# ALIZE-Speaker-Recognition/LIA_RAL

Measured on AMD Instinct MI355X. Metric: Gframe-Gaussian evals/s (UBM EM pass: LLK + full-posterior statistics), higher is better.
Workload: dtype f64; 1 GPU; TrainWorld EM: 2048-Gaussian diag UBM, 60-dim float32 frames, 10000000 frames per GPU resident in HBM, 1 EM iteration per step; gaussians=2048, dim=60, frames_per_gpu=10000000, partitioning=frames sharded per rank, one RCCL all-reduce of 247810 doubles per step

## Files before the change

### lia_ral_amd/csrc/capi_ctx.hip

```cpp
#include <stdarg.h>
#include <stdlib.h>

#include "ctx.h"
#include "gmm_kernels.h"

static thread_local char g_err[512] = "";

static thread_local gmmiv_kopts g_kopts_val;
static thread_local const gmmiv_kopts *g_kopts_src = nullptr;
const gmmiv_kopts &gmmiv_kopts_cur() { return g_kopts_val; }
void gmmiv_kopts_bind(const gmmiv_kopts *ko) { g_kopts_val = ko ? *ko : gmmiv_kopts(); g_kopts_src = ko; }

void gmmiv_set_error(const char *fmt, ...)
{
    va_list ap;
    va_start(ap, fmt);
    vsnprintf(g_err, sizeof(g_err), fmt, ap);
    va_end(ap);
}

bool gmmiv_is_device_ptr(const void *p)
{
    if (!p) return false;
    hipPointerAttribute_t at;
    hipError_t e = hipPointerGetAttributes(&at, p);
    if (e != hipSuccess) {
        (void)hipGetLastError();
        return false;
    }
    return at.type == hipMemoryTypeDevice || at.type == hipMemoryTypeManaged;
}

extern "C" {

const char *gmmiv_last_error(void) { return g_err; }
const char *gmmiv_version(void) { return "gmmiv 0.1 (gfx950)"; }

int gmmiv_ctx_create(int device, void *stream, gmmiv_ctx **out)
{
    if (!out) { gmmiv_set_error("ctx_create: out == NULL"); return GMMIV_ERR_ARG; }
    int ndev = 0;
    hipError_t e = hipGetDeviceCount(&ndev);
    if (e != hipSuccess || ndev <= 0) {
        (void)hipGetLastError();
        gmmiv_set_error("ctx_create: no HIP device available (%s)", e == hipSuccess ? "count = 0" : hipGetErrorString(e));
        return GMMIV_ERR_HIP;
    }
    if (device < 0 || device >= ndev) { gmmiv_set_error("ctx_create: device %d out of range [0,%d)", device, ndev); return GMMIV_ERR_ARG; }
    GCHK(hipSetDevice(device));
    gmmiv_ctx *c = new gmmiv_ctx();
    c->device = device;
    if (stream == GMMIV_STREAM_DEFAULT || stream == (void *)hipStreamLegacy) { c->stream = nullptr; c->own_stream = false; }
    else if (stream) { c->stream = (hipStream_t)stream; c->own_stream = false; }
    else { GCHK(hipStreamCreateWithFlags(&c->stream, hipStreamNonBlocking)); c->own_stream = true; }
    hipDeviceProp_t prop;
    if (hipGetDeviceProperties(&prop, device) == hipSuccess) { c->n_cu = prop.multiProcessorCount; c->total_mem = prop.totalGlobalMem; }
    if (hipMalloc((void **)&c->d_zero_llk, 2 * sizeof(unsigned long long)) != hipSuccess || hipMemset(c->d_zero_llk, 0, 2 * sizeof(unsigned long long)) != hipSuccess) {
        (void)hipGetLastError();
        if (c->own_stream) (void)hipStreamDestroy(c->stream);
        delete c;
        gmmiv_set_error("ctx_create: hipMalloc of the context's device counters failed");
        return GMMIV_ERR_HIP;
    }
    c->d_screened = c->d_zero_llk + 1;
    *out = c;
    return GMMIV_OK;
}

void gmmiv_ctx_destroy(gmmiv_ctx *c)
{
    if (!c) return;
    (void)hipSetDevice(c->device);
    (void)hipStreamSynchronize(c->stream);
    for (gmmiv_comm *cm : std::vector<gmmiv_comm *>(c->comms)) gmmiv_comm_orphan(cm);
    for (int i = 0; i < WS_COUNT; ++i)
        if (c->ws[i]) (void)hipFree(c->ws[i]);
    for (int i = 0; i < gmmiv_ctx::NSLOT; ++i) {
        for (hipEvent_t e : c->ev0[i]) (void)hipEventDestroy(e);
        for (hipEvent_t e : c->ev1[i]) (void)hipEventDestroy(e);
    }
    if (c->d_zero_llk) (void)hipFree(c->d_zero_llk);
    if (c->own_stream) (void)hipStreamDestroy(c->stream);
    if (g_kopts_src == &c->ko) gmmiv_kopts_bind(nullptr);
    delete c;
}

int gmmiv_ctx_sync(gmmiv_ctx *c)
{
    if (!c) return GMMIV_ERR_ARG;
    GCHK(hipStreamSynchronize(c->stream));
    return GMMIV_OK;
}

void *gmmiv_ctx_stream(gmmiv_ctx *c) { return c ? (void *)c->stream : nullptr; }

long gmmiv_ctx_set_option(gmmiv_ctx *c, const char *key, long value)
{
    if (!c || !key) return -1;
    long *slot = nullptr;
    if (!strcmp(key, "glds")) slot = &c->use_glds;
    else if (!strcmp(key, "em_chunks")) slot = &c->em_chunks;
    else if (!strcmp(key, "timing")) slot = &c->timing;
    else if (!strcmp(key, "wg_waves")) slot = &c->wg_waves;
    else if (!strcmp(key, "dbg")) slot = &c->dbg;
    else if (!strcmp(key, "prune_log2")) slot = &c->prune_log2;
    else if (!strcmp(key, "stats_z")) slot = &c->stats_z;
    else if (!strcmp(key, "z_scratch_mb")) slot = &c->z_scratch_mb;
    else if (!strcmp(key, "models_scratch_mb")) slot = &c->models_scratch_mb;
    else if (!strcmp(key, "trials_scratch_mb")) slot = &c->trials_scratch_mb;
    else if (!strcmp(key, "trials_piece")) slot = &c->trials_piece;
    else if (!strcmp(key, "iv_trials_anchor")) slot = &c->iv_trials_anchor;
    else if (!strcmp(key, "iv_trials_piece")) slot = &c->iv_trials_piece;
    else if (!strcmp(key, "tv_batch")) slot = &c->tv_batch;
    else if (!strcmp(key, "tv_tett_direct")) slot = &c->tv_tett_direct;
    else if (!strcmp(key, "tv_stats_split")) slot = &c->tv_stats_split;
    else if (!strcmp(key, "topc_z")) slot = &c->topc_z;
    else if (!strcmp(key, "tv_mstep_solve")) slot = &c->tv_mstep_solve;
    else if (!strcmp(key, "tv_md_device")) slot = &c->tv_md_device;
    else if (!strcmp(key, "tv_acc_mb")) slot = &c->tv_acc_mb;
    else if (!strcmp(key, "topc_fused")) slot = &c->topc_fused;
    else if (!strcmp(key, "topc_fallbacks")) slot = &c->topc_fallbacks;
    else if (!strcmp(key, "topc_rank_direct")) slot = &c->topc_rank_direct;
    else if (!strcmp(key, "topc_rank2")) slot = &c->topc_rank2;
    else if (!strcmp(key, "topc_use_lanes")) slot = &c->topc_use_lanes;
    else if (!strcmp(key, "assume_finite")) slot = &c->assume_finite;
    int *ks = nullptr;
    if (!strcmp(key, "z_waves")) { const long prev = c->ko.z_waves; c->ko.z_waves = (value == 4 || value == 16) ? (int)value : 8; return prev; }
    if (!strcmp(key, "z_depth_em")) { const long prev = c->ko.z_depth_em; if (value == 2 || value == 4) c->ko.z_depth_em = (int)value; return prev; }
    if (!strcmp(key, "z_depth_tv")) { const long prev = c->ko.z_depth_tv; if (value == 2 || value == 4) c->ko.z_depth_tv = (int)value; return prev; }
    if (!strcmp(key, "z_tv4")) ks = &c->ko.z_tv4;
    else if (!strcmp(key, "gemm_remap")) ks = &c->ko.gemm_remap;
    else if (!strcmp(key, "gemm_clamp")) ks = &c->ko.gemm_clamp;
    else if (!strcmp(key, "gemm_narrow")) ks = &c->ko.gemm_narrow;
    else if (!strcmp(key, "gemm_nt80")) ks = &c->ko.gemm_nt80;
    else if (!strcmp(key, "chol_lds")) ks = &c->ko.chol_lds;
    else if (!strcmp(key, "chol_gemm")) ks = &c->ko.chol_gemm;
    else if (!strcmp(key, "chol_waves")) ks = &c->ko.chol_waves;
    else if (!strcmp(key, "short_calls")) ks = &c->ko.short_calls;
    else if (!strcmp(key, "chol_flow")) ks = &c->ko.chol_flow;
    if (ks) { const long prev = *ks; *ks = (int)value; return prev; }
    if (!strcmp(key, "zero_llk_frames") || !strcmp(key, "screened_frames")) {
        unsigned long long *ctr = key[0] == 'z' ? c->d_zero_llk : c->d_screened;
        unsigned long long prev = 0, nv = value > 0 ? (unsigned long long)value : 0;
        if (hipSetDevice(c->device) != hipSuccess || hipStreamSynchronize(c->stream) != hipSuccess ||
            hipMemcpy(&prev, ctr, sizeof prev, hipMemcpyDeviceToHost) != hipSuccess ||
            hipMemcpy(ctr, &nv, sizeof nv, hipMemcpyHostToDevice) != hipSuccess) { (void)hipGetLastError(); return -1; }
        return (long)prev;
    }
    if (!strcmp(key, "kopts_bound")) return g_kopts_src == &c->ko ? 1 : 0;
    if (!slot) return -1;
    long prev = *slot;
    *slot = value;
    return prev;
}

int gmmiv_ctx_set_hook(gmmiv_ctx *c, const char *point, gmmiv_hook_fn fn, void *user)
{
    if (!c || !point) return -1;
    gmmiv_ctx::Hook *h = !strcmp(point, "tv_a_ready") ? &c->hook_tv_a_ready : (!strcmp(point, "md_factored") ? &c->hook_md_factored : nullptr);
    if (!h) return -1;
    h->fn = fn;
    h->user = fn ? user : nullptr;
    return 0;
}
// ... 103 lines not shown
```

### lia_ral_amd/csrc/capi_feat.hip

```cpp
#include <math.h>
#include <stdlib.h>

#include <algorithm>

#include "ctx.h"
#include "gmm_kernels.h"
#include "tv_kernels.h"
#include "capi_gmm_util.h"

extern "C" {

int gmmiv_frame_moments(gmmiv_ctx *c, const void *x, int dt, int64_t T, int64_t ldx, int D, double *acc)
{
    if (!c || !acc || T < 0 || D <= 0) { gmmiv_set_error("frame_moments: bad argument"); return GMMIV_ERR_ARG; }
    GBIND(c);
    XView xv;
    int rc = xv.init(c, x, dt, T, ldx, D);
    if (rc) return rc;
    DevOut<double> o;
    if ((rc = o.init(c, WS_T0, acc, 2 * D + 1, true))) return rc;
    const int maxb = 2048;
    void *part;
    if ((rc = c->scratch(WS_PART, (size_t)maxb * 2 * D * sizeof(double), &part))) return rc;
    c->t_begin("k_frame_moments");
// ... 63 lines not shown
    c->t_end();
    if (!gmmiv_is_device_ptr(runs)) GCHK(hipStreamSynchronize(c->stream));
    return GMMIV_OK;
}

int gmmiv_segment_means(gmmiv_ctx *c, const double *v, int64_t ld, int nrows, const int64_t *seg_begin, int64_t nseg, double *out)
{
    if (!c || !v || !seg_begin || !out || nrows < 0 || nseg < 0 || ld < 0) { gmmiv_set_error("segment_means: bad argument"); return GMMIV_ERR_ARG; }
    if (!gmmiv_is_device_ptr(v)) { gmmiv_set_error("segment_means: v must be a device array"); return GMMIV_ERR_ARG; }
    if (gmmiv_is_device_ptr(seg_begin)) { gmmiv_set_error("segment_means: seg_begin must be a host array"); return GMMIV_ERR_ARG; }
    for (int64_t s = 0; s < nseg; ++s)
        if (seg_begin[s] < 0 || seg_begin[s + 1] < seg_begin[s]) { gmmiv_set_error("segment_means: seg_begin must be non-negative and non-decreasing"); return GMMIV_ERR_ARG; }
    if (nseg > 0 && nrows > 1 && seg_begin[nseg] > ld) { gmmiv_set_error("segment_means: the last segment ends after the row stride"); return GMMIV_ERR_ARG; }
    const int64_t npair = (int64_t)nrows * nseg;
    if (npair == 0) return GMMIV_OK;
    GBIND(c);
    const int64_t PIECE = 8192;
    std::vector<long> tab;
    std::vector<long> off(npair + 1, 0), len(npair, 0);
    for (int r = 0; r < nrows; ++r)
        for (int64_t s = 0; s < nseg; ++s) {
            const int64_t p = (int64_t)r * nseg + s;
            len[p] = (long)(seg_begin[s + 1] - seg_begin[s]);
            for (int64_t b = seg_begin[s]; b < seg_begin[s + 1]; b += PIECE) {
                tab.push_back(r); tab.push_back((long)b); tab.push_back((long)(b + PIECE < seg_begin[s + 1] ? b + PIECE : seg_begin[s + 1]));
            }
            off[p + 1] = (long)(tab.size() / 3);
        }
    const size_t nitem = tab.size() / 3;
    tab.insert(tab.end(), off.begin(), off.end());
    tab.insert(tab.end(), len.begin(), len.end());
    void *dtab, *part;
    int rc;
    if ((rc = c->scratch(WS_T8, tab.size() * sizeof(long), &dtab))) return rc;
    if ((rc = c->scratch(WS_T9, (nitem ? nitem : 1) * sizeof(double), &part))) return rc;
    DevOut<double> o;
    if ((rc = o.init(c, WS_T7, out, (size_t)npair, false))) return rc;
    GCHK(hipMemcpyAsync(dtab, tab.data(), tab.size() * sizeof(long), hipMemcpyHostToDevice, c->stream));
    const long *di = (const long *)dtab;
    GCHK(gmmk_segment_means(c->stream, v, (long)ld, di, (long)nitem, (double *)part, di + 3 * nitem, di + 3 * nitem + npair + 1, (long)npair, o.d));
    GCHK(hipStreamSynchronize(c->stream));
    return o.finish();
}

static int feat_check_dtype(const char *who, int xdt, int odt)
{
    if ((xdt != GMMIV_F32 && xdt != GMMIV_F64) || (odt != GMMIV_F32 && odt != GMMIV_F64)) { gmmiv_set_error("%s: x_dtype / out_dtype must be GMMIV_F32 or GMMIV_F64", who); return GMMIV_ERR_ARG; }
    return GMMIV_OK;
}
static int feat_check(const char *who, const void *x, int xdt, int64_t T, int64_t ldx, const void *out, int odt, int64_t ldo, int D)
{
    if (T < 0 || ldx < D || ldo < D) { gmmiv_set_error("%s: T < 0 or a row stride below vectSize %d", who, D); return GMMIV_ERR_ARG; }
    if (T == 0) return GMMIV_OK;
    if (!x || !out) { gmmiv_set_error("%s: x or out == NULL", who); return GMMIV_ERR_ARG; }
    const uintptr_t xb = (uintptr_t)x, xe = xb + ((size_t)(T - 1) * ldx + D) * gmmiv_esize(xdt);
    const uintptr_t ob = (uintptr_t)out, oe = ob + ((size_t)(T - 1) * ldo + D) * gmmiv_esize(odt);
    const bool in_place = x == out && xdt == odt && ldx == ldo;
    if (!in_place && xb < oe && ob < xe) { gmmiv_set_error("%s: out overlaps x (only out == x with the same dtype and stride is allowed)", who); return GMMIV_ERR_ARG; }
    return GMMIV_OK;
}

int gmmiv_feat_check_args(const char *who, const void *x, int xdt, int64_t T, int64_t ldx, const void *out, int odt, int64_t ldo, int D)
{
    const int rc = feat_check_dtype(who, xdt, odt);
    return rc ? rc : feat_check(who, x, xdt, T, ldx, out, odt, ldo, D);
}

int gmmiv_feat_compensate(gmmiv_ctx *c, const gmmiv_gmm *g, const void *x, int dt, int64_t T, int64_t ldx, const double *offset,
                          void *out, int odt, int64_t ldo)
{
    int rc = feat_check_dtype("feat_compensate", dt, odt);
    if (rc) return rc;
    if (!c || !g) { gmmiv_set_error("feat_compensate: NULL context or model"); return GMMIV_ERR_ARG; }
    if ((rc = check_model(c, g))) return rc;
    if (!offset) { gmmiv_set_error("feat_compensate: offset == NULL"); return GMMIV_ERR_ARG; }
    if ((rc = feat_check("feat_compensate", x, dt, T, ldx, out, odt, ldo, g->D))) return rc;
    if (T == 0) return GMMIV_OK;
    XView xv;
    if ((rc = xv.init(c, x, dt, T, ldx, g->D))) return rc;
    FeatOut o;
    if ((rc = o.init(c, out, odt, 0, T, ldo, g->D))) return rc;
    DevIn<double> i_off;
    if ((rc = i_off.init(c, WS_FEAT_M0, offset, (size_t)g->C * g->D))) return rc;
    if ((rc = count_unusable(c, xv, dt, T, g->D))) return rc;
    const int64_t Tcz = g->D <= 64 ? z_chunk_frames(c, g) : 0;
    if (Tcz > 0) {
        gmmk_zview z;
        double *lz;
        void *offp;
        if ((rc = gmmiv_z_reserve(c, g->nct, T < Tcz ? T : Tcz, true, &z, &lz))) return rc;
        if ((rc = c->scratch(WS_FEAT_OFF, gmmk_feat_offset_doubles(g->nct, g->D) * sizeof(double), &offp))) return rc;
        GCHK(gmmk_feat_pack_offset(c->stream, i_off.d, g->C, g->D, g->nct, (double *)offp));
        for (int64_t c0 = 0; c0 < T; c0 += Tcz) {
            const int64_t n = (T - c0) < Tcz ? (T - c0) : Tcz;
            if ((rc = llk_z_run(c, g, xv, dt, c0, n, lz, z, c0 == 0))) return rc;
            GCHK(count_dead(c, lz, n));
            c->t_begin("k_feat_comp", c0 == 0);
            GCHK(gmmk_feat_comp(c->stream, dt == GMMIV_F64, odt == GMMIV_F64, gmmiv_x_at(xv, dt, c0), xv.ldx, n, g->D, g->nct, z, (const double *)offp,
                                o.at(c0), o.ld));
            c->t_end();
        }
        return o.finish();
    }
    double *lse;
    if ((rc = run_lse(c, g, xv, dt, T, &lse))) return rc;
    int64_t per = (int64_t)(((size_t)512 << 20) / ((size_t)g->C * sizeof(double))) / 2 * 2;
    if (per < 64) per = 64;
    const int64_t firstg = T < per ? T : per;
    void *gam, *pm;
    if ((rc = c->scratch(WS_Z, (size_t)firstg * g->C * sizeof(double), &gam))) return rc;
    if ((rc = c->scratch(WS_INV, (size_t)firstg * g->D * sizeof(double), &pm))) return rc;
    for (int64_t b = 0; b < T; b += per) {
        const int64_t m = T - b < per ? T - b : per;
        c->t_begin("k_posteriors", b == 0);
        GCHK(gmmk_posteriors(c->stream, dt == GMMIV_F64, gmmiv_x_at(xv, dt, b), (long)m, xv.ldx, g->D, g->C, g->Cp64, g->meanT, g->ivT, g->lwc, lse + b,
                             (double *)gam));
        c->t_end();
        GCHK(tvk_dgemm(c->stream, false, false, (int)m, g->D, g->C, 1.0, (const double *)gam, g->C, 0, i_off.d, g->D, 0, 0.0, (double *)pm, g->D, 0, 1));
        c->t_begin("k_feat_sub", b == 0);
        GCHK(gmmk_feat_sub(c->stream, dt == GMMIV_F64, odt == GMMIV_F64, gmmiv_x_at(xv, dt, b), xv.ldx, (long)m, g->D, (const double *)pm, lse + b, o.at(b), o.ld));
        c->t_end();
    }
    return o.finish();
}

int gmmiv_feat_map(gmmiv_ctx *c, const gmmiv_gmm *cd, const double *cd_mean, const double *cd_cov, const double *ci_mean,
                   const double *ci_cov, const void *x, int dt, int64_t T, int64_t ldx, void *out, int odt, int64_t ldo, int32_t *best)
{
    int rc = feat_check_dtype("feat_map", dt, odt);
    if (rc) return rc;
    if (!c || !cd) { gmmiv_set_error("feat_map: NULL context or model"); return GMMIV_ERR_ARG; }
    if ((rc = check_model(c, cd))) return rc;
    if (!cd_mean || !cd_cov || !ci_mean || !ci_cov) { gmmiv_set_error("feat_map: a model table is NULL"); return GMMIV_ERR_ARG; }
    if ((rc = feat_check("feat_map", x, dt, T, ldx, out, odt, ldo, cd->D))) return rc;
    if (T == 0) return GMMIV_OK;
    XView xv;
    if ((rc = xv.init(c, x, dt, T, ldx, cd->D))) return rc;
    FeatOut o;
    if ((rc = o.init(c, out, odt, 0, T, ldo, cd->D))) return rc;
    const size_t CD = (size_t)cd->C * cd->D;
    DevIn<double> m0, v0, m1, v1;
    if ((rc = m0.init(c, WS_FEAT_M0, cd_mean, CD)) || (rc = v0.init(c, WS_FEAT_M1, cd_cov, CD)) || (rc = m1.init(c, WS_FEAT_M2, ci_mean, CD)) ||
        (rc = v1.init(c, WS_FEAT_M3, ci_cov, CD))) return rc;
    int32_t *bd = best;
    if (!gmmiv_is_device_ptr(best)) {
        void *p;
        if ((rc = c->scratch(WS_FEAT_IDX, (size_t)T * sizeof(int32_t), &p))) return rc;
        bd = (int32_t *)p;
    }
    GCHK(hipMemsetAsync(bd, 0, (size_t)T * sizeof(int32_t), c->stream));
    if ((rc = gmmiv_llk_determine_top(c, cd, xv.d, dt, T, xv.ldx, 1, GMMIV_TOP_COMPLETE, -INFINITY, INFINITY, bd, nullptr, nullptr, nullptr, nullptr,
                                      nullptr))) return rc;
    c->t_begin("k_feat_map");
    GCHK(gmmk_feat_map(c->stream, dt == GMMIV_F64, odt == GMMIV_F64, xv.d, xv.ldx, T, cd->D, cd->C, bd, m0.d, v0.d, m1.d, v1.d, o.d, o.ld));
    c->t_end();
    if (best && bd != best) GCHK(hipMemcpyAsync(best, bd, (size_t)T * sizeof(int32_t), hipMemcpyDeviceToHost, c->stream));
    if ((rc = o.finish())) return rc;
    if (best && bd != best) GCHK(hipStreamSynchronize(c->stream));
    return GMMIV_OK;
}

int gmmiv_scatter_runs(gmmiv_ctx *c, void *x, int dt, int64_t ldx, int D, const int64_t *runs, int64_t nrun, const void *in)
{
    if (!c || !x || !in || (!runs && nrun > 0) || nrun < 0 || D <= 0 || ldx < D) { gmmiv_set_error("scatter_runs: bad argument"); return GMMIV_ERR_ARG; }
    if (dt != GMMIV_F32 && dt != GMMIV_F64) { gmmiv_set_error("scatter_runs: feature dtype must be GMMIV_F32 or GMMIV_F64"); return GMMIV_ERR_ARG; }
    if (!gmmiv_is_device_ptr(x) || !gmmiv_is_device_ptr(in)) { gmmiv_set_error("scatter_runs: x and in must be device arrays"); return GMMIV_ERR_ARG; }
    if (nrun == 0) return GMMIV_OK;
    GBIND(c);
    DevIn<int64_t> i_runs;
    int rc = i_runs.init(c, WS_T0, runs, (size_t)nrun * 3);
    if (rc) return rc;
    c->t_begin("k_scatter_runs");
    GCHK(gmmk_scatter_runs(c->stream, dt == GMMIV_F64, x, ldx, D, (const long *)i_runs.d, nrun, in));
    c->t_end();
    if (!gmmiv_is_device_ptr(runs)) GCHK(hipStreamSynchronize(c->stream));
    return GMMIV_OK;
}

static int norm_check_runs(const char *who, const int64_t *runs, int64_t nrun, int64_t ngroups, int64_t *lo, int64_t *hi)
{
    int64_t prev = 0, a = INT64_MAX, b = 0;
    for (int64_t r = 0; r < nrun; ++r) {
        const int64_t first = runs[3 * r], len = runs[3 * r + 1], g = runs[3 * r + 2];
        if (first < 0 || len < 0) { gmmiv_set_error("%s: run %ld has a negative first frame or length", who, (long)r); return GMMIV_ERR_ARG; }
        if (g < prev || g >= ngroups) { gmmiv_set_error("%s: run %ld: group %ld is below its predecessor's or outside [0, %ld) (group ids must be non-decreasing)", who, (long)r, (long)g, (long)ngroups); return GMMIV_ERR_ARG; }
        prev = g;
        if (len > 0) { if (first < a) a = first; if (first + len > b) b = first + len; }
    }
// ... 216 lines not shown
```

### lia_ral_amd/csrc/capi_gmm.hip

```cpp
#include <math.h>
#include <stdlib.h>

#include "ctx.h"
#include "gmm_kernels.h"
#include "tv_kernels.h"
#include "capi_gmm_util.h"

namespace {
struct TopOut {
    int *idx;
    double *lk, *nlk, *nllk, *nw, *llk;
    int ctop;
    template <typename V> static V *from(V *p, size_t off) { return p ? p + off : nullptr; }
    TopOut at(int64_t c0) const { return TopOut{from(idx, (size_t)c0 * ctop), from(lk, (size_t)c0 * ctop), from(nlk, c0), from(nllk, c0), from(nw, c0), from(llk, c0), ctop}; }
};
}

int count_unusable(gmmiv_ctx *c, const XView &xv, int dt, int64_t T, int D)
{
    if (c->assume_finite || T <= 0) return GMMIV_OK;
    void *p;
    int rc;
    const size_t fbytes = ((size_t)T + 15) / 16 * 16;
    if ((rc = c->scratch(WS_GFLAG, fbytes + 16, &p))) return rc;
    unsigned char *flag = (unsigned char *)p;
    GCHK(hipMemsetAsync(flag, 0, fbytes + 16, c->stream));
    GCHK(gmmk_flag_frames(c->stream, dt == GMMIV_F64, xv.d, T, xv.ldx, D, flag, (int *)(flag + fbytes)));
    GCHK(gmmk_count_flags(c->stream, flag, (long)T, c->d_screened));
    return GMMIV_OK;
}

static int topc_big(gmmiv_ctx *c, const gmmiv_gmm *g, const XView &xv, int dt, int64_t T, int complete, double lo, double hi, const TopOut &o)
{
    const int ctop = o.ctop;
    if (T <= 0) return GMMIV_OK;
    int64_t per = (int64_t)(((size_t)1 << 30) / ((size_t)g->Cp64 * sizeof(double))) / 4 * 4;
    if (per < 4) per = 4;
    if (per > T) per = (T + 3) / 4 * 4;
    void *zs;
    int rc = c->scratch(WS_Z, gmmk_topc_big_scratch_doubles((long)per, g->Cp64) * sizeof(double), &zs);
    if (rc) return rc;
    for (int64_t c0 = 0; c0 < T; c0 += per) {
        const int64_t n = T - c0 < per ? T - c0 : per;
        c->t_begin("k_topc_determine", c0 == 0);
        const TopOut oc = o.at(c0);
        int krc = gmmk_topc_determine_big(c->stream, dt == GMMIV_F64, gmmiv_x_at(xv, dt, c0), (long)n, xv.ldx, g->D, g->C, g->Cp64, g->meanT, g->ivT, g->lwc,
                                          g->w, ctop, complete, lo, hi, oc.idx, oc.lk, oc.nlk, oc.nllk, oc.nw, oc.llk, (double *)zs);
        c->t_end();
        if (krc == -1) { gmmiv_set_error("vectSize %d exceeds the generic kernels' bound", g->D); return GMMIV_ERR_UNSUPPORTED; }
        if (krc == -2) { gmmiv_set_error("topDistribsCount %d outside 1 .. mixtureDistribCount %d", ctop, g->C); return GMMIV_ERR_ARG; }
        GCHK(krc);
    }
    return GMMIV_OK;
}

int run_lse(gmmiv_ctx *c, const gmmiv_gmm *g, const XView &xv, int dt, int64_t T, double **lse_out)
{
    void *lse;
    int rc = c->scratch(WS_LSE, (size_t)(T > 0 ? T : 1) * sizeof(double), &lse);
    if (rc) return rc;
    if (g->KS == GMMK_KS_GENERIC) {
        if ((rc = topc_big(c, g, xv, dt, T, 1, -INFINITY, INFINITY, TopOut{nullptr, nullptr, nullptr, nullptr, nullptr, (double *)lse, 1}))) return rc;
        GCHK(count_dead(c, (const double *)lse, T));
        *lse_out = (double *)lse;
        return GMMIV_OK;
    }
    c->t_begin("k_llk_mfma");
    GCHK(gmmk_llk(c->stream, g->KS, dt == GMMIV_F64, xv.d, T, xv.ldx, g->D, g->Pt, g->nct, (double *)lse, (int)(c->use_glds | (c->dbg << 8)), (int)c->wg_waves));
    c->t_end();
    GCHK(count_dead(c, (const double *)lse, T));
    *lse_out = (double *)lse;
    return GMMIV_OK;
}

int generic_gamma_gemm(gmmiv_ctx *c, const gmmiv_gmm *g, const XView &xv, int dt, int64_t t0, int64_t n, const double *lse, bool sq, int NC,
                       double *S)
{
    int rc;
    int64_t per = (int64_t)(((size_t)512 << 20) / ((size_t)g->C * sizeof(double)));
    if (per < 64) per = 64;
    per = per / 2 * 2;
    void *gam, *xa;
    const int64_t first = n < per ? n : per;
    if ((rc = c->scratch(WS_Z, (size_t)(first > 0 ? first : 1) * g->C * sizeof(double), &gam))) return rc;
    if ((rc = c->scratch(WS_INV, (size_t)(first > 0 ? first : 1) * NC * sizeof(double), &xa))) return rc;
    if (n <= 0) { GCHK(hipMemsetAsync(S, 0, (size_t)g->C * NC * sizeof(double), c->stream)); return GMMIV_OK; }
    for (int64_t b = 0; b < n; b += per) {
        const int64_t m = n - b < per ? n - b : per;
        c->t_begin("k_posteriors", b == 0);
        GCHK(gmmk_posteriors(c->stream, dt == GMMIV_F64, gmmiv_x_at(xv, dt, t0 + b), (long)m, xv.ldx, g->D, g->C, g->Cp64, g->meanT, g->ivT, g->lwc, lse + t0 + b,
                             (double *)gam));
        c->t_end();
        GCHK(gmmk_build_xa(c->stream, dt == GMMIV_F64, gmmiv_x_at(xv, dt, t0 + b), xv.ldx, g->D, (long)m, sq ? 1 : 0, NC, (double *)xa));
        GCHK(tvk_dgemm(c->stream, true, false, g->C, NC, (int)m, 1.0, (const double *)gam, g->C, 0, (const double *)xa, NC, 0, b == 0 ? 0.0 : 1.0, S, NC, 0, 1));
    }
    return GMMIV_OK;
}

static size_t fused_frame_bytes() { return (size_t)gmmk_topc_cap() * 16; }

static int64_t fused_chunk_frames(const gmmiv_ctx *c)
{
    size_t budget = (size_t)(c->z_scratch_mb > 0 ? c->z_scratch_mb : 0) << 20;
    if (c->total_mem && budget > c->total_mem / 4) budget = c->total_mem / 4;
    const int64_t Tf = (int64_t)(budget / fused_frame_bytes() / 1.2) / 256 * 256;
    return Tf >= 256 ? Tf : 0;
}

static int top_fused(gmmiv_ctx *c, const gmmiv_gmm *g, const XView &xv, int dt, int64_t T, int complete, double min_llk, double max_llk,
                     const TopOut &o, int64_t Tf, bool *done)
{
    int rc;
    const int ctop = o.ctop;
    const int64_t nalloc = T < Tf ? (T + 255) / 256 * 256 : Tf;
    const int stats = getenv("GMMIV_TOPC_STATS") != nullptr;
    void *cand, *cnt, *th, *sl, *flg, *redo;
    if ((rc = c->scratch(WS_Z, (size_t)nalloc * fused_frame_bytes(), &cand))) return rc;
    if ((rc = c->scratch(WS_EIT, (size_t)nalloc * sizeof(int), &cnt))) return rc;
    if ((rc = c->scratch(WS_INV, (size_t)nalloc * (sizeof(double) + sizeof(int)), &sl))) return rc;
    if ((rc = c->scratch(WS_LSE, (size_t)nalloc * sizeof(double), &th))) return rc;
    if ((rc = c->scratch(WS_FLAGS, 64, &flg))) return rc;
    int *efin = (int *)((double *)sl + nalloc);
    if ((rc = c->scratch(WS_SEG, (size_t)nalloc * 2 * sizeof(long), &redo))) return rc;
    int krc = 0;
    bool whole = false;
    for (int64_t c0 = 0; c0 < T; c0 += Tf) {
        const int64_t n = (T - c0) < Tf ? (T - c0) : Tf;
        const TopOut oc = o.at(c0);
        GCHK(hipMemsetAsync(flg, 0, 64, c->stream));
        c->t_begin("k_llk_mfma", c0 == 0);
        krc = gmmk_llk_topc(c->stream, g->KS, dt == GMMIV_F64, gmmiv_x_at(xv, dt, c0), n, xv.ldx, g->D, g->Pt, g->nct, (int)c->use_glds,
                            ctop, (double *)cand, (int *)cnt, (double *)th, (double *)sl, efin);
        c->t_end();
        if (krc) break;
        c->t_begin("k_topc_rank", c0 == 0);
        krc = gmmk_topc_rank(c->stream, dt == GMMIV_F64, gmmiv_x_at(xv, dt, c0), n, xv.ldx, g->D, g->C, (const double *)cand, (const int *)cnt,
                             (const double *)th, (const double *)sl, efin, g->mean, g->iv, g->lwc, g->w, ctop, complete,
                             min_llk, max_llk, oc.idx, oc.lk, oc.nlk, oc.nllk, oc.nw, oc.llk, (int *)flg, (long *)redo,
                             stats | (c->topc_rank_direct ? 2 : 0) | (c->topc_rank2 ? 0 : 4), (long *)redo + nalloc);
        c->t_end();
        if (krc) break;
        int hf[16] = {0};
        GCHK(hipMemcpyAsync(hf, flg, 64, hipMemcpyDeviceToHost, c->stream));
        GCHK(hipStreamSynchronize(c->stream));
        if (stats)
            fprintf(stderr, "topc fused: %ld frames, redone %d | overflow %d, survivors > 64: %d, < ctop: %d, margin %d | list max %d mean %.1f | survivors max %d mean %.1f\n",
                    (long)n, hf[0], hf[1], hf[2], hf[3], hf[4], hf[5], (double)*(unsigned long long *)&hf[6] / (double)n, hf[8],
                    (double)*(unsigned long long *)&hf[10] / (double)n);
        const int64_t nr = hf[0];
        c->topc_fallbacks += nr;
        if (nr == 0) continue;
        if (nr > n / 8 + 64) { whole = true; break; }
        void *gx, *t_idx, *t_d;
        if ((rc = c->scratch(WS_PART, (size_t)nr * g->D * gmmiv_esize(dt), &gx))) return rc;
        if ((rc = c->scratch(WS_T6, (size_t)nr * ctop * sizeof(int), &t_idx))) return rc;
        if ((rc = c->scratch(WS_T7, (size_t)nr * (ctop + 4) * sizeof(double), &t_d))) return rc;
        double *t_lk = (double *)t_d, *t_nlk = t_lk + (size_t)nr * ctop, *t_nllk = t_nlk + nr, *t_nw = t_nllk + nr, *t_llk = t_nw + nr;
        GCHK(gmmk_gather_frames(c->stream, dt == GMMIV_F64, gmmiv_x_at(xv, dt, c0), xv.ldx, g->D, (const long *)redo, nr, gx));
        c->t_begin("k_topc_determine", c0 == 0);
        GCHK(gmmk_topc_determine(c->stream, dt == GMMIV_F64, gx, nr, g->D, g->D, g->C, g->Cp64, g->meanT, g->ivT, g->lwc, g->w, ctop,
                                 complete, min_llk, max_llk, (int *)t_idx, t_lk, t_nlk, t_nllk, t_nw, t_llk));
        c->t_end();
        GCHK(gmmk_topc_scatter(c->stream, nr, ctop, (const long *)redo, (const int *)t_idx, t_lk, t_nlk, t_nllk, t_nw, t_llk, oc.idx, oc.lk, oc.nlk,
                               oc.nllk, oc.nw, oc.llk));
    }
    if (krc > 0) GCHK(krc);
    *done = krc == 0 && !whole;
    return GMMIV_OK;
}

static int top_from_z(gmmiv_ctx *c, const gmmiv_gmm *g, const XView &xv, int dt, int64_t T, int complete, double min_llk, double max_llk,
                      const TopOut &o, int64_t Tc, bool *done)
{
    int rc;
    gmmk_zview z;
    double *lse;
    void *flg;
    if ((rc = gmmiv_z_reserve(c, g->nct, T < Tc ? T : Tc, true, &z, &lse))) return rc;
    if ((rc = c->scratch(WS_FLAGS, 64, &flg))) return rc;
    GCHK(hipMemsetAsync(flg, 0, sizeof(int), c->stream));
    for (int64_t c0 = 0; c0 < T; c0 += Tc) {
        const int64_t n = (T - c0) < Tc ? (T - c0) : Tc;
        const TopOut oc = o.at(c0);
        if ((rc = llk_z_run(c, g, xv, dt, c0, n, lse, z, c0 == 0))) return rc;
        c->t_begin("k_topc_from_z", c0 == 0);
        GCHK(gmmk_topc_from_z(c->stream, dt == GMMIV_F64, gmmiv_x_at(xv, dt, c0), n, xv.ldx, g->D, g->C, g->nct, z, g->mean, g->iv, g->lwc, g->w,
                              o.ctop, complete, min_llk, max_llk, oc.idx, oc.lk, oc.nlk, oc.nllk, oc.nw, oc.llk, (int *)flg));
        c->t_end();
    }
    int hflag = 0;
    GCHK(hipMemcpyAsync(&hflag, flg, sizeof(int), hipMemcpyDeviceToHost, c->stream));
    GCHK(hipStreamSynchronize(c->stream));
    *done = hflag == 0;
    return GMMIV_OK;
}

static int top_direct(gmmiv_ctx *c, const gmmiv_gmm *g, const XView &xv, int dt, int64_t T, int complete, double min_llk, double max_llk,
                      const TopOut &o)
{
    if (o.ctop > 64 || !gmmk_topc_frames_per_block(g->Cp64, g->D)) return topc_big(c, g, xv, dt, T, complete, min_llk, max_llk, o);
    c->t_begin("k_topc_determine");
    GCHK(gmmk_topc_determine(c->stream, dt == GMMIV_F64, xv.d, T, xv.ldx, g->D, g->C, g->Cp64, g->meanT, g->ivT, g->lwc,
                             g->w, o.ctop, complete, min_llk, max_llk, o.idx, o.lk, o.nlk, o.nllk, o.nw, o.llk));
    c->t_end();
    return GMMIV_OK;
}

extern "C" {

int gmmiv_llk(gmmiv_ctx *c, const gmmiv_gmm *g, const void *x, int dt, int64_t T, int64_t ldx, double min_llk,
              double max_llk, double *llk_out, double *sums)
{
    int rc = check_model(c, g);
    if (rc) return rc;
    if (T < 0) { gmmiv_set_error("llk: T < 0"); return GMMIV_ERR_ARG; }
    XView xv;
    if ((rc = xv.init(c, x, dt, T, ldx, g->D))) return rc;
    if ((rc = count_unusable(c, xv, dt, T, g->D))) return rc;
    double *lse;
    if ((rc = run_lse(c, g, xv, dt, T, &lse))) return rc;
    DevOut<double> o_llk, o_sum;
    if ((rc = o_llk.init(c, WS_T0, llk_out, (size_t)T, false))) return rc;
    if ((rc = o_sum.init(c, WS_T1, sums, 2, true))) return rc;
    void *part;
    if ((rc = c->scratch(WS_SMALL, 3 * 256 * sizeof(double), &part))) return rc;
    GCHK(gmmk_llk_finalize(c->stream, lse, T, min_llk, max_llk, o_llk.d, (double *)part, 1.0, 0.0,
                           sums ? o_sum.d : nullptr, nullptr));
    if (sums) GCHK(gmmk_add_scalar(c->stream, o_sum.d + 1, (double)T));
    if ((rc = o_llk.finish())) return rc;
    return o_sum.finish();
}

int gmmiv_llk_determine_top(gmmiv_ctx *c, const gmmiv_gmm *g, const void *x, int dt, int64_t T, int64_t ldx, int ctop,
                            int mode, double min_llk, double max_llk, int32_t *idx, double *lk, double *nontop_lk,
                            double *nontop_llk, double *nontop_w, double *llk_out)
{
    int rc = check_model(c, g);
    if (rc) return rc;
    if (T < 0 || !idx || ctop <= 0) { gmmiv_set_error("determine_top: bad argument"); return GMMIV_ERR_ARG; }
    if (ctop > g->C) { gmmiv_set_error("determine_top: topDistribsCount %d exceeds mixtureDistribCount %d (clamp it at the call site)", ctop, g->C); return GMMIV_ERR_ARG; }
    XView xv;
    if ((rc = xv.init(c, x, dt, T, ldx, g->D))) return rc;
    if ((rc = count_unusable(c, xv, dt, T, g->D))) return rc;
    DevOut<int32_t> o_idx;
    DevOut<double> o_lk, o_nlk, o_nllk, o_nw, o_llk;
    if ((rc = o_idx.init(c, WS_T0, idx, (size_t)T * ctop, false))) return rc;
    if ((rc = o_lk.init(c, WS_T1, lk, (size_t)T * ctop, false))) return rc;
    if ((rc = o_nlk.init(c, WS_T2, nontop_lk, (size_t)T, false))) return rc;
    if ((rc = o_nllk.init(c, WS_T3, nontop_llk, (size_t)T, false))) return rc;
    if ((rc = o_nw.init(c, WS_T4, nontop_w, (size_t)T, false))) return rc;
    if ((rc = o_llk.init(c, WS_T5, llk_out, (size_t)T, false))) return rc;
    const TopOut o{o_idx.d, o_lk.d, o_nlk.d, o_nllk.d, o_nw.d, o_llk.d, ctop};
    const int complete = mode == GMMIV_TOP_COMPLETE;
    bool done = false;
    const int64_t Tf = (c->topc_fused && T > 0 && ctop <= 16 && g->C <= 2048 && g->D <= 64 && g->KS <= 15 && c->wg_waves == 8) ? fused_chunk_frames(c) : 0;
    if (Tf > 0 && (rc = top_fused(c, g, xv, dt, T, complete, min_llk, max_llk, o, Tf, &done))) return rc;
    const int64_t Tc = (!done && c->topc_z) ? z_chunk_frames(c, g) : 0;
    if (Tc > 0 && T > 0 && ctop + 4 <= 64 && gmmk_topc_z_lds(g->nct, g->D) && (rc = top_from_z(c, g, xv, dt, T, complete, min_llk, max_llk, o, Tc, &done))) return rc;
    if (!done && (rc = top_direct(c, g, xv, dt, T, complete, min_llk, max_llk, o))) return rc;
    if ((rc = o_idx.finish())) return rc;
    if ((rc = o_lk.finish())) return rc;
    if ((rc = o_nlk.finish())) return rc;
    if ((rc = o_nllk.finish())) return rc;
    if ((rc = o_nw.finish())) return rc;
    return o_llk.finish();
}

int gmmiv_topgauss_compute(gmmiv_ctx *c, const gmmiv_gmm *g, const void *x, int dt, int64_t T, int64_t ldx, int cap, double top_gauss,
                           int mode, double min_llk, double max_llk, int32_t *idx, int32_t *count, double *snsw, double *snsl,
                           double *llk_out, int64_t *n_capped)
{
    int rc = check_model(c, g);
    if (rc) return rc;
    if (T < 0 || !idx || !count || !snsw || !snsl || cap <= 0 || !(top_gauss > 0.0)) { gmmiv_set_error("topgauss_compute: bad argument"); return GMMIV_ERR_ARG; }
    if (n_capped && gmmiv_is_device_ptr(n_capped)) { gmmiv_set_error("topgauss_compute: n_capped must be a host variable"); return GMMIV_ERR_ARG; }
    const int fixed = top_gauss >= 1.0 ? (int)top_gauss : 0;
    if (fixed > cap) { gmmiv_set_error("topgauss_compute: topGauss %d exceeds the list length %d", fixed, cap); return GMMIV_ERR_ARG; }
    if (n_capped) *n_capped = 0;
    if (T == 0) return GMMIV_OK;
    void *p;
    const bool idx_dev = gmmiv_is_device_ptr(idx);
    int32_t *d_idx = idx;
    if (!idx_dev) { if ((rc = c->scratch(WS_LP, (size_t)T * cap * sizeof(int32_t), &p))) return rc; d_idx = (int32_t *)p; }
    if ((rc = c->scratch(WS_AUX, (size_t)T * cap * sizeof(double), &p))) return rc;
    double *d_lk = (double *)p;
    const bool llk_dev = llk_out && gmmiv_is_device_ptr(llk_out);
    double *d_llk = llk_out;
    if (!llk_dev) { if ((rc = c->scratch(WS_SLAB, (size_t)T * sizeof(double), &p))) return rc; d_llk = (double *)p; }
    if ((rc = gmmiv_llk_determine_top(c, g, x, dt, T, ldx, cap, mode, min_llk, max_llk, d_idx, d_lk, nullptr, nullptr, nullptr, d_llk))) return rc;
    DevOut<int32_t> o_cnt;
    DevOut<double> o_w, o_l;
    if ((rc = o_cnt.init(c, WS_T0, count, (size_t)T, false))) return rc;
    if ((rc = o_w.init(c, WS_T1, snsw, (size_t)T, false))) return rc;
    if ((rc = o_l.init(c, WS_T2, snsl, (size_t)T, false))) return rc;
    if ((rc = c->scratch(WS_SMALL, 3 * 256 * sizeof(double), &p))) return rc;
    unsigned long long *d_cap = (unsigned long long *)p;
    GCHK(hipMemsetAsync(d_cap, 0, sizeof(unsigned long long), c->stream));
    GCHK(gmmk_topgauss_select(c->stream, T, cap, top_gauss, fixed, g->w, d_idx, d_lk, d_llk, o_cnt.d, o_w.d, o_l.d, d_cap));
    if (!idx_dev) GCHK(hipMemcpyAsync(idx, d_idx, (size_t)T * cap * sizeof(int32_t), hipMemcpyDeviceToHost, c->stream));
    if (llk_out && !llk_dev) GCHK(hipMemcpyAsync(llk_out, d_llk, (size_t)T * sizeof(double), hipMemcpyDeviceToHost, c->stream));
    if (n_capped) {
        unsigned long long h = 0;
        GCHK(hipMemcpyAsync(&h, d_cap, sizeof(h), hipMemcpyDeviceToHost, c->stream));
// ... 25 lines not shown
    if ((rc = o_llk.init(c, WS_T2, llk_out, (size_t)T, false))) return rc;
    if ((rc = count_unusable(c, xv, dt, T, g->D))) return rc;
    c->t_begin("k_topc_use");
    int krc = ctop > 64 ? gmmk_topc_use_big(c->stream, dt == GMMIV_F64, xv.d, T, xv.ldx, g->D, g->mean, g->iv, g->lwc, g->C, ctop, i_idx.d, i_n.d,
                                            mode == GMMIV_TOP_COMPLETE, min_llk, max_llk, o_llk.d)
              : c->topc_z ? gmmk_topc_use16(c->stream, dt == GMMIV_F64, xv.d, T, xv.ldx, g->D, g->mean, g->iv, g->lwc, g->C, ctop, i_idx.d, i_n.d,
                                          mode == GMMIV_TOP_COMPLETE, min_llk, max_llk, o_llk.d, (int)c->topc_use_lanes)
                        : -1;
    if (krc == -1 && ctop <= 64)
        krc = gmmk_topc_use(c->stream, dt == GMMIV_F64, xv.d, T, xv.ldx, g->D, g->mean, g->iv, g->lwc, g->C, ctop, i_idx.d, i_n.d,
                            mode == GMMIV_TOP_COMPLETE, min_llk, max_llk, o_llk.d);
    GCHK(krc);
    c->t_end();
    return o_llk.finish();
}

int gmmiv_llk_use_top_multi(gmmiv_ctx *c, int n_clients, const gmmiv_gmm *const *clients, const void *x, int dt, int64_t T, int64_t ldx,
                            int ctop, const int32_t *idx, const double *nontop_llk, int mode, double min_llk, double max_llk,
                            double *llk_out)
{
    if (!c) { gmmiv_set_error("use_top_multi: null context"); return GMMIV_ERR_ARG; }
    if (n_clients < 0 || (n_clients > 0 && !clients)) { gmmiv_set_error("use_top_multi: bad client list"); return GMMIV_ERR_ARG; }
    if (n_clients == 0) return GMMIV_OK;
    int rc;
    for (int i = 0; i < n_clients; ++i) {
        if ((rc = check_model(c, clients[i]))) return rc;
        if (clients[i]->D != clients[0]->D) { gmmiv_set_error("use_top_multi: client %d has %d dimensions, client 0 has %d", i, clients[i]->D, clients[0]->D); return GMMIV_ERR_ARG; }
        if (ctop > clients[i]->C) { gmmiv_set_error("use_top_multi: topDistribsCount %d exceeds mixtureDistribCount %d of client %d", ctop, clients[i]->C, i); return GMMIV_ERR_ARG; }
    }
    if (T < 0 || !idx || !llk_out || ctop <= 0) { gmmiv_set_error("use_top_multi: bad argument"); return GMMIV_ERR_ARG; }
    if (mode == GMMIV_TOP_COMPLETE && !nontop_llk) { gmmiv_set_error("use_top_multi: COMPLETE mode needs nontop_llk"); return GMMIV_ERR_ARG; }
    const gmmiv_gmm *g0 = clients[0];
    {
        const size_t cap = (size_t)1 << 30, row = (size_t)(T > 0 ? T : 1) * sizeof(double);
        if (n_clients > 1 && !gmmiv_is_device_ptr(llk_out) && (size_t)n_clients * row > cap) {
            const int per = (int)(cap / row > 0 ? cap / row : 1);
            for (int i0 = 0; i0 < n_clients; i0 += per) {
                const int n = n_clients - i0 < per ? n_clients - i0 : per;
                if ((rc = gmmiv_llk_use_top_multi(c, n, clients + i0, x, dt, T, ldx, ctop, idx, nontop_llk, mode, min_llk, max_llk, llk_out + (size_t)i0 * T))) return rc;
            }
            return GMMIV_OK;
        }
    }
    const bool batched = c->topc_z && c->topc_use_lanes == 4 && ctop <= 16 && g0->D % 2 == 0 && n_clients <= 65535 && T > 0;
    if (!batched) {
        for (int i = 0; i < n_clients; ++i)
            if ((rc = gmmiv_llk_use_top(c, clients[i], x, dt, T, ldx, ctop, idx, nontop_llk, mode, min_llk, max_llk, llk_out + (size_t)i * T))) return rc;
        return GMMIV_OK;
    }
    GBIND(c);
    XView xv;
    if ((rc = xv.init(c, x, dt, T, ldx, g0->D))) return rc;
    if ((rc = count_unusable(c, xv, dt, T, g0->D))) return rc;
    DevIn<int32_t> i_idx;
    DevIn<double> i_n;
    DevOut<double> o_llk;
    if ((rc = i_idx.init(c, WS_T0, idx, (size_t)T * ctop))) return rc;
    if ((rc = i_n.init(c, WS_T1, nontop_llk, (size_t)T))) return rc;
    if ((rc = o_llk.init(c, WS_T2, llk_out, (size_t)T * n_clients, false))) return rc;
    struct Rec { const double *mean, *iv, *lwc; long C; };
    std::vector<Rec> recs((size_t)n_clients);
    for (int i = 0; i < n_clients; ++i) recs[i] = Rec{clients[i]->mean, clients[i]->iv, clients[i]->lwc, (long)clients[i]->C};
    void *drec;
    if ((rc = c->scratch(WS_T3, recs.size() * sizeof(Rec), &drec))) return rc;
    GCHK(hipMemcpyAsync(drec, recs.data(), recs.size() * sizeof(Rec), hipMemcpyHostToDevice, c->stream));
    GCHK(hipStreamSynchronize(c->stream));
    c->t_begin("k_topc_use");
    GCHK(gmmk_topc_use4_multi(c->stream, dt == GMMIV_F64, xv.d, T, xv.ldx, g0->D, drec, n_clients, ctop, i_idx.d, i_n.d, mode == GMMIV_TOP_COMPLETE,
                              min_llk, max_llk, o_llk.d));
    c->t_end();
    return o_llk.finish();
}

int gmmiv_occ(gmmiv_ctx *c, const gmmiv_gmm *g, const void *x, int dt, int64_t T, int64_t ldx, double *gamma)
{
    int rc = check_model(c, g);
    if (rc) return rc;
    if (T < 0 || !gamma) { gmmiv_set_error("occ: bad argument"); return GMMIV_ERR_ARG; }
    if (T > 0x7fffffff) { gmmiv_set_error("occ: too many frames in one call"); return GMMIV_ERR_UNSUPPORTED; }
    XView xv;
    if ((rc = xv.init(c, x, dt, T, ldx, g->D))) return rc;
    DevOut<double> o;
    if ((rc = o.init(c, WS_T0, gamma, (size_t)T * g->C, false))) return rc;
    if ((rc = count_unusable(c, xv, dt, T, g->D))) return rc;
    const int64_t Tcz = c->topc_z ? z_chunk_frames(c, g) : 0;
    if (Tcz > 0 && T > 0) {
        gmmk_zview z;
        double *lz;
        if ((rc = gmmiv_z_reserve(c, g->nct, T < Tcz ? T : Tcz, true, &z, &lz))) return rc;
        for (int64_t c0 = 0; c0 < T; c0 += Tcz) {
            const int64_t n = (T - c0) < Tcz ? (T - c0) : Tcz;
            if ((rc = llk_z_run(c, g, xv, dt, c0, n, lz, z, c0 == 0))) return rc;
            GCHK(count_dead(c, lz, n));
            c->t_begin("k_post_from_z", c0 == 0);
            GCHK(gmmk_post_from_z(c->stream, n, g->C, g->nct, z, o.d + (size_t)c0 * g->C));
            c->t_end();
        }
        return o.finish();
    }
    double *lse;
    if ((rc = run_lse(c, g, xv, dt, T, &lse))) return rc;
    c->t_begin("k_posteriors");
    GCHK(gmmk_posteriors(c->stream, dt == GMMIV_F64, xv.d, T, xv.ldx, g->D, g->C, g->Cp64, g->meanT, g->ivT, g->lwc, lse, o.d));
    c->t_end();
    return o.finish();
}

size_t gmmiv_em_acc_len(int C, int D) { return (size_t)C * (1 + 2 * (size_t)D) + 2; }

static int make_chunks(gmmiv_ctx *c, int64_t T, int nseg, long **dev)
{
    const int64_t per = ((T + nseg - 1) / nseg + 63) / 64 * 64;
    void *buf;
    int rc = c->scratch(WS_SEG, (nseg + 1) * sizeof(long), &buf);
    if (rc) return rc;
    GCHK(gmmk_fill_chunks(c->stream, (long *)buf, nseg, (long)per, (long)T));
    *dev = (long *)buf;
    return GMMIV_OK;
}

static int em_stats_z(gmmiv_ctx *c, const gmmiv_gmm *g, const XView &xv, int dt, int64_t T, int64_t Tc, double weight,
                      double *lse, int *nseg_out, void **part_out)
{
    int rc;
    const int ngrp = gmmk_stats_z_groups(g->nct);
    int nseg = c->em_chunks > 0 ? (int)c->em_chunks : (c->n_cu * gmmk_stats_z_wg_per_cu() + ngrp - 1) / ngrp;
    nseg = (nseg + 7) / 8 * 8;
    const int64_t first = T < Tc ? T : Tc;
    const int64_t cap = (first + 255) / 256;
    if (nseg > cap) nseg = (int)((cap + 7) / 8 * 8);
    const int64_t nchunk = (T + Tc - 1) / Tc;
    const int64_t lastn = T - (nchunk - 1) * Tc;
    void *seg, *part;
    if ((rc = c->scratch(WS_SEG, 2 * (size_t)(nseg + 1) * sizeof(long), &seg))) return rc;
    auto fill = [&](long *dst, int64_t n) {
        const int64_t per = ((n + nseg - 1) / nseg + 63) / 64 * 64;
        return gmmk_fill_chunks(c->stream, dst, nseg, (long)per, (long)n);
    };
    GCHK(fill((long *)seg, first));
    GCHK(fill((long *)seg + nseg + 1, lastn));
    gmmk_zview z;
    if ((rc = gmmiv_z_reserve(c, g->nct, first, !(c->dbg & 64), &z, nullptr))) return rc;
    const int RL = gmmk_rl_for_ks(g->KS);
    const size_t Cp = (size_t)g->nct * 16;
    if ((rc = c->scratch(WS_PART, (size_t)nseg * Cp * 2 * RL * sizeof(double), &part))) return rc;
    for (int64_t k = 0; k < nchunk; ++k) {
        const int64_t c0 = k * Tc, n = (k == nchunk - 1) ? lastn : Tc;
        if ((rc = llk_z_run(c, g, xv, dt, c0, n, lse + c0, z, k == 0))) return rc;
        GCHK(count_dead(c, lse + c0, n));
        c->t_begin("k_stats_z", k == 0);
        GCHK(gmmk_stats_z(c->stream, g->KS, 1, dt == GMMIV_F64, gmmiv_x_at(xv, dt, c0), xv.ldx, g->D, g->C, g->nct, z, weight,
                          (const long *)seg + (k == nchunk - 1 ? nseg + 1 : 0), nseg, (double *)part, nullptr, 0, k > 0, c->prune_thr()));
        c->t_end();
    }
    *nseg_out = nseg;
    *part_out = part;
    return GMMIV_OK;
}

int gmmiv_em_accumulate(gmmiv_ctx *c, const gmmiv_gmm *g, const void *x, int dt, int64_t T, int64_t ldx, double weight,
                        double *acc)
{
    int rc = check_model(c, g);
    if (rc) return rc;
    if (T < 0 || !acc || !(weight > 0.0)) { gmmiv_set_error("em_accumulate: bad argument (T >= 0, weight > 0, acc != NULL)"); return GMMIV_ERR_ARG; }
    const size_t nacc = gmmiv_em_acc_len(g->C, g->D);
    DevOut<double> o;
    if ((rc = o.init(c, WS_T0, acc, nacc, true))) return rc;
    if (T == 0) return o.finish();
    XView xv;
    if ((rc = xv.init(c, x, dt, T, ldx, g->D))) return rc;
    if ((rc = count_unusable(c, xv, dt, T, g->D))) return rc;
    const int64_t Tc = z_chunk_frames(c, g);
    if (Tc > 0) {
        void *lsew, *small, *part;
        int nseg = 0;
        if ((rc = c->scratch(WS_LSE, (size_t)T * sizeof(double), &lsew))) return rc;
        if ((rc = c->scratch(WS_SMALL, 3 * 256 * sizeof(double), &small))) return rc;
        if ((rc = em_stats_z(c, g, xv, dt, T, Tc, weight, (double *)lsew, &nseg, &part))) return rc;
        GCHK(gmmk_llk_finalize(c->stream, (const double *)lsew, T, -INFINITY, INFINITY, nullptr, (double *)small, 0.0, weight, nullptr,
                               o.d + nacc - 2, weight, o.d + nacc - 1));
        GCHK(gmmk_em_reduce(c->stream, (const double *)part, nseg, g->C, g->nct * 16, g->D, g->KS, o.d));
        return o.finish();
    }
    double *lse;
    if ((rc = run_lse(c, g, xv, dt, T, &lse))) return rc;
    void *small;
    if ((rc = c->scratch(WS_SMALL, 3 * 256 * sizeof(double), &small))) return rc;
    GCHK(gmmk_llk_finalize(c->stream, lse, T, -INFINITY, INFINITY, nullptr, (double *)small, 0.0, weight, nullptr,
                           o.d + nacc - 2, weight, o.d + nacc - 1));
    if (g->KS == GMMK_KS_GENERIC) {
        const int NC = 2 * g->D + 2;
        void *S;
        if ((rc = c->scratch(WS_PART, (size_t)g->C * NC * sizeof(double), &S))) return rc;
        if ((rc = generic_gamma_gemm(c, g, xv, dt, 0, T, lse, true, NC, (double *)S))) return rc;
        GCHK(gmmk_scatter_em(c->stream, g->C, g->D, NC, (const double *)S, weight, o.d));
        return o.finish();
    }
    const int nw = c->wg_waves == 8 ? 8 : 4;
    const int ngrp = (g->nct + nw - 1) / nw;
    int nseg = c->em_chunks > 0 ? (int)c->em_chunks : ((nw == 8 ? 2 : 4) * c->n_cu + ngrp - 1) / ngrp;
    nseg = (nseg + 7) / 8 * 8;
    const int64_t cap = (T + 4095) / 4096;
    if (nseg > cap) nseg = (int)cap;
    if (nseg < 1) nseg = 1;
    long *seg;
    if ((rc = make_chunks(c, T, nseg, &seg))) return rc;
    const int RL = gmmk_rl_for_ks(g->KS);
    const size_t Cp = (size_t)g->nct * 16;
    void *part;
    if ((rc = c->scratch(WS_PART, (size_t)nseg * Cp * 2 * RL * sizeof(double), &part))) return rc;
    c->t_begin("k_stats_mfma");
    GCHK(gmmk_stats(c->stream, g->KS, 1, dt == GMMIV_F64, xv.d, xv.ldx, g->D, g->C, g->Pt, g->nct, lse, -log(weight), seg,
                    nseg, (double *)part, nullptr, 0, (int)c->wg_waves, c->prune_arg()));
    c->t_end();
    GCHK(gmmk_em_reduce(c->stream, (const double *)part, nseg, g->C, (int)Cp, g->D, g->KS, o.d));
    return o.finish();
}

int gmmiv_em_get(gmmiv_ctx *c, int C, int D, const double *acc, const double *prev_mean, const double *prev_cov,
                 double *w, double *mean, double *cov)
{
    if (!c || !acc || !prev_mean || !prev_cov || !w || !mean || !cov || C <= 0 || D <= 0) { gmmiv_set_error("em_get: bad argument"); return GMMIV_ERR_ARG; }
    GBIND(c);
    const size_t CD = (size_t)C * D;
    DevIn<double> i_acc, i_pm, i_pc;
    DevOut<double> o_w, o_m, o_c;
    int rc;
    if ((rc = i_acc.init(c, WS_T0, acc, gmmiv_em_acc_len(C, D)))) return rc;
    if ((rc = i_pm.init(c, WS_T1, prev_mean, CD))) return rc;
    if ((rc = i_pc.init(c, WS_T2, prev_cov, CD))) return rc;
    if ((rc = o_w.init(c, WS_T3, w, C, false))) return rc;
    if ((rc = o_m.init(c, WS_T4, mean, CD, false))) return rc;
    if ((rc = o_c.init(c, WS_T5, cov, CD, false))) return rc;
    GCHK(gmmk_em_get(c->stream, C, D, i_acc.d, i_pm.d, i_pc.d, o_w.d, o_m.d, o_c.d));
    if ((rc = o_w.finish())) return rc;
    if ((rc = o_m.finish())) return rc;
    return o_c.finish();
}

int gmmiv_variance_control(gmmiv_ctx *c, int C, int D, double *cov, double flooring, double ceiling,
                           const double *cov_signal, int64_t *counts)
{
    if (!c || C <= 0 || D <= 0 || !cov || !cov_signal) { gmmiv_set_error("variance_control: bad argument"); return GMMIV_ERR_ARG; }
    if (counts && gmmiv_is_device_ptr(counts)) { gmmiv_set_error("variance_control: counts must be a host array"); return GMMIV_ERR_ARG; }
    GBIND(c);
    DevOut<double> o;
    DevIn<double> i_cs;
    int rc;
    if ((rc = o.init(c, WS_T0, cov, (size_t)C * D, true))) return rc;
    if ((rc = i_cs.init(c, WS_T1, cov_signal, D))) return rc;
    unsigned long long *dc = nullptr;
    if (counts) {
        void *p;
        if ((rc = c->scratch(WS_SMALL, 3 * 256 * sizeof(double), &p))) return rc;
        dc = (unsigned long long *)p;
        GCHK(hipMemsetAsync(dc, 0, 2 * sizeof(unsigned long long), c->stream));
    }
    GCHK(gmmk_variance_control(c->stream, C, D, o.d, flooring, ceiling, i_cs.d, dc));
    if (counts) {
        unsigned long long h[2];
        GCHK(hipMemcpyAsync(h, dc, sizeof(h), hipMemcpyDeviceToHost, c->stream));
        GCHK(hipStreamSynchronize(c->stream));
        counts[0] = (int64_t)h[0];
        counts[1] = (int64_t)h[1];
    }
    return o.finish();
}

static bool plan_utt_chunks(const int64_t *utt_begin, int64_t U, int64_t Tcz, std::vector<int64_t> &cu, std::vector<long> &rel, int64_t *maxn)
{
    cu.assign(1, 0);
    const int64_t Ttot = utt_begin[U] - utt_begin[0], nch = (Ttot + Tcz - 1) / Tcz;
    const int64_t target = nch > 0 ? (Ttot + nch - 1) / nch : Tcz;
    for (int64_t u = 0; u < U;) {
        int64_t v = u;
        while (v < U && utt_begin[v + 1] - utt_begin[u] <= Tcz && (v == u || utt_begin[v] - utt_begin[u] < target)) ++v;
        if (v < U && v - u > 64) v = u + (v - u) / 64 * 64;
        if (v == u) return false;
        if (utt_begin[v] - utt_begin[u] > *maxn) *maxn = utt_begin[v] - utt_begin[u];
        cu.push_back(v);
        u = v;
    }
    for (size_t k = 0; k + 1 < cu.size(); ++k)
        for (int64_t u = cu[k]; u <= cu[k + 1]; ++u) rel.push_back((long)(utt_begin[u] - utt_begin[cu[k]]));
    return true;
}

static bool plan_utt_pieces(const int64_t *utt_begin, int64_t U, std::vector<long> &pb, std::vector<int> &rbh)
{
    rbh.assign((size_t)U + 1, 0);
    const int64_t per_utt = 32 / U > 1 ? 32 / U : 1;
    for (int64_t u = 0; u < U; ++u) {
        const int64_t b = utt_begin[u] - utt_begin[0], e = utt_begin[u + 1] - utt_begin[0], len = e - b;
        int64_t S = (len + 255) / 256;
        S = S < 1 ? 1 : (S > per_utt ? per_utt : S);
        const int64_t per = ((len + S - 1) / S + 63) / 64 * 64;
        int64_t pos = b;
        int cntp = 0;
        do { pb.push_back((long)pos); pos = per > 0 && pos + per < e ? pos + per : e; ++cntp; } while (pos < e);
        rbh[u + 1] = rbh[u] + cntp;
    }
    pb.push_back((long)(utt_begin[U] - utt_begin[0]));
    return rbh[U] > U;
}

int gmmiv_tv_stats(gmmiv_ctx *c, const gmmiv_gmm *g, const void *x, int dt, int64_t T, int64_t ldx,
                   const int64_t *utt_begin, int64_t U, double *N, double *F)
{
    int rc = check_model(c, g);
    if (rc) return rc;
    if (T < 0 || U < 0 || !utt_begin || !N || !F) { gmmiv_set_error("tv_stats: bad argument"); return GMMIV_ERR_ARG; }
    if (gmmiv_is_device_ptr(utt_begin)) { gmmiv_set_error("tv_stats: utt_begin must be a host array"); return GMMIV_ERR_ARG; }
    if (U == 0) return GMMIV_OK;
    if (utt_begin[0] < 0 || utt_begin[U] > T) { gmmiv_set_error("tv_stats: utt_begin out of range"); return GMMIV_ERR_ARG; }
    for (int64_t u = 0; u < U; ++u)
        if (utt_begin[u + 1] < utt_begin[u]) { gmmiv_set_error("tv_stats: utt_begin must be non-decreasing"); return GMMIV_ERR_ARG; }
    if (U > 0x7fffffff / 64) { gmmiv_set_error("tv_stats: too many utterances in one call"); return GMMIV_ERR_UNSUPPORTED; }
    XView xv;
    if ((rc = xv.init(c, x, dt, T, ldx, g->D))) return rc;
    if ((rc = count_unusable(c, xv, dt, T, g->D))) return rc;
    std::vector<long> h(utt_begin, utt_begin + U + 1);
    void *seg;
    if ((rc = c->scratch(WS_SEG, (U + 1) * sizeof(long), &seg))) return rc;
    GCHK(hipMemcpyAsync(seg, h.data(), (U + 1) * sizeof(long), hipMemcpyHostToDevice, c->stream));
    GCHK(hipStreamSynchronize(c->stream));
    const size_t SV = (size_t)g->C * g->D;
    DevOut<double> o_n, o_f;
    if ((rc = o_n.init(c, WS_T0, N, (size_t)U * g->C, false))) return rc;
    if ((rc = o_f.init(c, WS_T1, F, (size_t)U * SV, false))) return rc;
    const int64_t Tcz = z_chunk_frames(c, g);
    std::vector<int64_t> cu;
    std::vector<long> rel;
    int64_t maxn = 0;
    if (Tcz > 0 && plan_utt_chunks(utt_begin, U, Tcz, cu, rel, &maxn)) {
        if ((rc = c->scratch(WS_SEG, rel.size() * sizeof(long), &seg))) return rc;
        GCHK(hipMemcpyAsync(seg, rel.data(), rel.size() * sizeof(long), hipMemcpyHostToDevice, c->stream));
        GCHK(hipStreamSynchronize(c->stream));
        gmmk_zview z;
        double *lsew;
        if ((rc = gmmiv_z_reserve(c, g->nct, maxn, true, &z, &lsew))) return rc;
        std::vector<long> pb;
        std::vector<int> rbh;
        const bool split = cu.size() == 2 && U <= 16 && c->tv_stats_split && plan_utt_pieces(utt_begin, U, pb, rbh);
        const int np = split ? rbh[U] : 0;
        void *pseg = nullptr, *prb = nullptr, *tn = o_n.d, *tf = o_f.d;
        if (split) {
            if ((rc = c->scratch(WS_SEG, pb.size() * sizeof(long), &pseg))) return rc;
            if ((rc = c->scratch(WS_SMALL, rbh.size() * sizeof(int) + 64, &prb))) return rc;
            if ((rc = c->scratch(WS_T2, (size_t)np * g->C * sizeof(double), &tn))) return rc;
            if ((rc = c->scratch(WS_T3, (size_t)np * SV * sizeof(double), &tf))) return rc;
            GCHK(hipMemcpyAsync(pseg, pb.data(), pb.size() * sizeof(long), hipMemcpyHostToDevice, c->stream));
            GCHK(hipMemcpyAsync(prb, rbh.data(), rbh.size() * sizeof(int), hipMemcpyHostToDevice, c->stream));
            GCHK(hipStreamSynchronize(c->stream));
        }
        for (size_t k = 0; k + 1 < cu.size(); ++k) {
            const int64_t u0 = cu[k], u1 = cu[k + 1], c0 = utt_begin[u0], n = utt_begin[u1] - c0;
            if ((rc = llk_z_run(c, g, xv, dt, c0, n, lsew, z, k == 0))) return rc;
            GCHK(count_dead(c, lsew, n));
            c->t_begin("k_stats_z", k == 0);
            GCHK(gmmk_stats_z(c->stream, g->KS, 0, dt == GMMIV_F64, gmmiv_x_at(xv, dt, c0), xv.ldx, g->D, g->C, g->nct, z, 1.0,
                              split ? (const long *)pseg : (const long *)seg + u0 + k, split ? np : (int)(u1 - u0), (double *)tn + (size_t)u0 * g->C,
                              (double *)tf + (size_t)u0 * SV, 1, 0, c->prune_thr()));
            if (split) {
                GCHK(gmmk_rows_sum_groups(c->stream, g->C, (int)U, (const int *)prb, (const double *)tn, o_n.d));
                GCHK(gmmk_rows_sum_groups(c->stream, (long)SV, (int)U, (const int *)prb, (const double *)tf, o_f.d));
            }
            c->t_end();
        }
        if ((rc = o_n.finish())) return rc;
        return o_f.finish();
    }
    double *lse;
    if ((rc = run_lse(c, g, xv, dt, T, &lse))) return rc;
    if (g->KS == GMMK_KS_GENERIC) {
        const int NC = g->D + 2 - (g->D & 1);
        void *S;
        if ((rc = c->scratch(WS_PART, (size_t)g->C * NC * sizeof(double), &S))) return rc;
        for (int64_t u = 0; u < U; ++u) {
            if ((rc = generic_gamma_gemm(c, g, xv, dt, utt_begin[u], utt_begin[u + 1] - utt_begin[u], lse, false, NC, (double *)S))) return rc;
            GCHK(gmmk_scatter_nf(c->stream, g->C, g->D, NC, (const double *)S, o_n.d + (size_t)u * g->C, o_f.d + (size_t)u * SV));
        }
        if ((rc = o_n.finish())) return rc;
        return o_f.finish();
    }
    c->t_begin("k_stats_mfma");
    GCHK(gmmk_stats(c->stream, g->KS, 0, dt == GMMIV_F64, xv.d, xv.ldx, g->D, g->C, g->Pt, g->nct, lse, 0.0,
                    (const long *)seg, (int)U, o_n.d, o_f.d, 1, (int)c->wg_waves, c->prune_arg()));
    c->t_end();
    if ((rc = o_n.finish())) return rc;
    return o_f.finish();
}

int gmmiv_tv_stats_lines(gmmiv_ctx *c, const gmmiv_gmm *g, const void *x, int dt, int64_t T, int64_t ldx, const int64_t *file_begin,
                         int64_t nfiles, int64_t nlines, const int64_t *line_off, const int64_t *line_files, double *N, double *F)
{
    int rc = check_model(c, g);
    if (rc) return rc;
    if (nfiles < 0 || nlines < 0 || !file_begin || !line_off || (!line_files && nlines && line_off[nlines]) || !N || !F) { gmmiv_set_error("tv_stats_lines: bad argument"); return GMMIV_ERR_ARG; }
    if (gmmiv_is_device_ptr(line_off) || gmmiv_is_device_ptr(line_files)) { gmmiv_set_error("tv_stats_lines: the line map must be host arrays"); return GMMIV_ERR_ARG; }
    if (nlines == 0) return GMMIV_OK;
    if (line_off[0] != 0) { gmmiv_set_error("tv_stats_lines: line_off must start at 0"); return GMMIV_ERR_ARG; }
    for (int64_t l = 0; l < nlines; ++l)
        if (line_off[l + 1] < line_off[l]) { gmmiv_set_error("tv_stats_lines: line_off must be non-decreasing"); return GMMIV_ERR_ARG; }
    const int64_t npairs = line_off[nlines];
    for (int64_t p = 0; p < npairs; ++p)
        if (line_files[p] < 0 || line_files[p] >= nfiles) { gmmiv_set_error("tv_stats_lines: file index %lld out of range", (long long)line_files[p]); return GMMIV_ERR_ARG; }
    const size_t SV = (size_t)g->C * g->D;
    void *pn, *pf, *pm;
    if ((rc = c->scratch(WS_T6, (size_t)(nfiles ? nfiles : 1) * g->C * sizeof(double), &pn))) return rc;
    if ((rc = c->scratch(WS_T7, (size_t)(nfiles ? nfiles : 1) * SV * sizeof(double), &pf))) return rc;
    if ((rc = gmmiv_tv_stats(c, g, x, dt, T, ldx, file_begin, nfiles, (double *)pn, (double *)pf))) return rc;
    if ((rc = c->scratch(WS_T8, (size_t)(nlines + 1 + npairs + 1) * sizeof(long), &pm))) return rc;
    std::vector<long> h((size_t)nlines + 1 + npairs);
    for (int64_t l = 0; l <= nlines; ++l) h[l] = (long)line_off[l];
    for (int64_t p = 0; p < npairs; ++p) h[nlines + 1 + p] = (long)line_files[p];
    GCHK(hipMemcpyAsync(pm, h.data(), h.size() * sizeof(long), hipMemcpyHostToDevice, c->stream));
    DevOut<double> o_n, o_f;
    if ((rc = o_n.init(c, WS_T4, N, (size_t)nlines * g->C, false))) return rc;
    if ((rc = o_f.init(c, WS_T5, F, (size_t)nlines * SV, false))) return rc;
    const long *off = (const long *)pm, *rows = off + nlines + 1;
    GCHK(tvk_merge_rows(c->stream, (long)nlines, g->C, off, rows, (const double *)pn, o_n.d));
    GCHK(tvk_merge_rows(c->stream, (long)nlines, (long)SV, off, rows, (const double *)pf, o_f.d));
    GCHK(hipStreamSynchronize(c->stream));
    if ((rc = o_n.finish())) return rc;
    return o_f.finish();
}

}
```

### lia_ral_amd/csrc/capi_gmm_util.h

```cpp
#pragma once
#include "ctx.h"
#include "gmm_kernels.h"

static inline int check_model(gmmiv_ctx *c, const gmmiv_gmm *g)
{
    if (!c || !g) { gmmiv_set_error("NULL context or model"); return GMMIV_ERR_ARG; }
    if (g->ctx != c) { gmmiv_set_error("model belongs to a different context"); return GMMIV_ERR_ARG; }
    GBIND(c);
    return GMMIV_OK;
}

static inline size_t gmmiv_esize(int dt) { return dt == GMMIV_F64 ? 8 : 4; }

struct XView {
    const void *d = nullptr;
    int64_t ldx = 0;
    int init(gmmiv_ctx *c, const void *x, int dt, int64_t T, int64_t ld, int D)
    {
        if (dt != GMMIV_F32 && dt != GMMIV_F64) { gmmiv_set_error("feature dtype must be GMMIV_F32 or GMMIV_F64"); return GMMIV_ERR_ARG; }
        if (ld < D) { gmmiv_set_error("ldx (%ld) < D (%d)", (long)ld, D); return GMMIV_ERR_ARG; }
        if (T == 0) { d = x; ldx = ld; return GMMIV_OK; }
        if (!x) { gmmiv_set_error("x == NULL"); return GMMIV_ERR_ARG; }
        if (gmmiv_is_device_ptr(x)) { d = x; ldx = ld; return GMMIV_OK; }
        void *buf;
        int rc = c->scratch(WS_X, (size_t)T * D * gmmiv_esize(dt), &buf);
        if (rc) return rc;
        GCHK(hipMemcpy2DAsync(buf, D * gmmiv_esize(dt), x, ld * gmmiv_esize(dt), D * gmmiv_esize(dt), T, hipMemcpyHostToDevice, c->stream));
        d = buf; ldx = D;
        return GMMIV_OK;
    }
};

static inline const void *gmmiv_x_at(const XView &xv, int dt, int64_t frame) { return (const char *)xv.d + (size_t)frame * xv.ldx * gmmiv_esize(dt); }

struct FeatOut {
    void *d = nullptr, *host = nullptr;
    int64_t ld = 0, hld = 0, F0 = 0, F1 = 0;
    int D = 0, dt = 0;
    gmmiv_ctx *c = nullptr;
    int init(gmmiv_ctx *ctx, void *out, int odt, int64_t F0_, int64_t F1_, int64_t ldo, int D_)
    {
        c = ctx; F0 = F0_; F1 = F1_; D = D_; dt = odt;
        if (F1 == F0 || gmmiv_is_device_ptr(out)) { d = out; ld = ldo; return GMMIV_OK; }
        void *stage;
        int rc = c->scratch(WS_FEAT_OUT, (size_t)(F1 - F0) * D * gmmiv_esize(odt), &stage);
        if (rc) return rc;
        host = out; hld = ldo; ld = D;
        d = (char *)stage - (ptrdiff_t)F0 * ld * (ptrdiff_t)gmmiv_esize(dt);
        return GMMIV_OK;
    }
    void *at(int64_t frame) const { return (char *)d + (ptrdiff_t)frame * ld * (ptrdiff_t)gmmiv_esize(dt); }
    int finish()
    {
        if (host) {
            GCHK(hipMemcpy2DAsync((char *)host + (size_t)F0 * hld * gmmiv_esize(dt), hld * gmmiv_esize(dt), at(F0), D * gmmiv_esize(dt), D * gmmiv_esize(dt),
                                  (size_t)(F1 - F0), hipMemcpyDeviceToHost, c->stream));
            GCHK(hipStreamSynchronize(c->stream));
        }
        return GMMIV_OK;
    }
};

static inline long gmmiv_z_tile_blocks(int64_t n, bool pad)
{
    long nfb = 16 * ((n + 255) / 256);
    if (pad && (nfb / 2) % 2 == 0) nfb += 2;
    return nfb;
}

static inline int gmmiv_z_reserve(gmmiv_ctx *c, int nct, int64_t frames, bool pad, gmmk_zview *z, double **lse)
{
    const size_t n = (size_t)(frames > 0 ? frames : 1);
    void *zb, *eit, *inv, *l;
    int rc;
    z->nfb = gmmiv_z_tile_blocks(frames, pad);
    if ((rc = c->scratch(WS_Z, (size_t)nct * z->nfb * 2048, &zb))) return rc;
    if ((rc = c->scratch(WS_EIT, (size_t)(nct / 2) * z->nfb * 16 * sizeof(int), &eit))) return rc;
    if ((rc = c->scratch(WS_INV, n * (sizeof(double) + sizeof(int)), &inv))) return rc;
    if (lse && (rc = c->scratch(WS_LSE, n * sizeof(double), &l))) return rc;
    z->zbuf = (double *)zb; z->eit = (int *)eit; z->inv = (double *)inv;
    z->efin = (int *)(z->inv + n);
    if (lse) *lse = (double *)l;
    return GMMIV_OK;
}

static inline int64_t gmmiv_z_budget_frames(const gmmiv_ctx *c, int nct, size_t extra)
{
    size_t budget = (size_t)(c->z_scratch_mb > 0 ? c->z_scratch_mb : 0) << 20;
    if (c->total_mem && budget > c->total_mem / 4) budget = c->total_mem / 4;
    const size_t per_frame = (size_t)nct * 16 * sizeof(double) + (size_t)nct * 2 + extra;
    return (int64_t)(budget / per_frame / 1.2);
}

static inline int64_t z_chunk_frames(gmmiv_ctx *c, const gmmiv_gmm *g)
{
    if (!c->stats_z || g->KS > 15 || c->wg_waves != 8) return 0;
    int64_t tc = gmmiv_z_budget_frames(c, g->nct, 16);
    const int64_t round = (int64_t)c->n_cu * 2 * 256;
    tc = tc >= round ? tc / round * round : tc / 64 * 64;
    return tc >= 4096 ? tc : 0;
}

static inline int llk_z_run(gmmiv_ctx *c, const gmmiv_gmm *g, const XView &xv, int dt, int64_t c0, int64_t n, double *lse, const gmmk_zview &z, bool first)
{
    c->t_begin("k_llk_mfma", first);
    GCHK(gmmk_llk_z(c->stream, g->KS, dt == GMMIV_F64, gmmiv_x_at(xv, dt, c0), n, xv.ldx, g->D, g->Pt, g->nct, lse,
                    (int)(c->use_glds | ((c->dbg & 15) << 8)), z));
    c->t_end();
    return GMMIV_OK;
}

static inline int count_dead(gmmiv_ctx *c, const double *lse, int64_t n) { return gmmk_count_dead(c->stream, lse, (long)n, c->d_zero_llk); }

#pragma GCC visibility push(hidden)
int count_unusable(gmmiv_ctx *c, const XView &xv, int dt, int64_t T, int D);
int run_lse(gmmiv_ctx *c, const gmmiv_gmm *g, const XView &xv, int dt, int64_t T, double **lse_out);
int generic_gamma_gemm(gmmiv_ctx *c, const gmmiv_gmm *g, const XView &xv, int dt, int64_t t0, int64_t n, const double *lse, bool sq, int NC,
                       double *S);
extern "C" int gmmiv_feat_check_args(const char *who, const void *x, int xdt, int64_t T, int64_t ldx, const void *out, int odt, int64_t ldo, int D);
#pragma GCC visibility pop
```

### lia_ral_amd/csrc/capi_models.hip

```cpp
#include <math.h>
#include <stdlib.h>

#include <vector>

#include "capi_gmm_util.h"
#include "gmm_kernels.h"

#define MODEL_TILE_FRAMES 256

extern "C" {

int64_t gmmiv_plan_model_tiles(const int64_t *seg_begin, const int32_t *seg_model, int64_t nseg, int tile_frames, gmmiv_model_tile *tiles,
                               int64_t cap)
{
    if (!seg_begin || !seg_model || nseg < 0 || tile_frames <= 0 || tile_frames % 32 || seg_begin[0] < 0) return -1;
    int64_t first_ne = -1, last_ne = -1;
    for (int64_t s = 0; s < nseg; ++s) {
        if (seg_begin[s + 1] < seg_begin[s]) return -1;
        if (seg_begin[s + 1] > seg_begin[s]) { if (first_ne < 0) first_ne = s; last_ne = s; }
    }
    int64_t n = 0;
    for (int64_t s = 0; s < nseg; ++s) {
        const int64_t b = seg_begin[s], e = seg_begin[s + 1];
        if (e <= b) continue;
// ... 236 lines not shown
            const int64_t nf = gmmiv_plan_feat_tiles(seg_begin + s0, seg_model + s0, s1 - s0, p.feat_blocks, nullptr, 0);
            p.ftiles.resize(ck.ftile_off + (size_t)nf);
            gmmiv_plan_feat_tiles(seg_begin + s0, seg_model + s0, s1 - s0, p.feat_blocks, p.ftiles.data() + ck.ftile_off, nf);
            for (size_t i = ck.ftile_off; i < p.ftiles.size(); ++i) {
                gmmiv_feat_tile &t = p.ftiles[i];
                t.block -= ck.base / 16; t.lo -= ck.base; t.hi -= ck.base;
                t.model = slot[t.model];
            }
            ck.nftiles = (size_t)nf;
        }
        for (size_t i = ck.id_off; i < p.ids.size(); ++i) slot[p.ids[i]] = -1;
        const int64_t span = seg_begin[s1] - ck.base;
        if (span > p.max_span) p.max_span = span;
        if ((int)ck.nids > p.max_models) p.max_models = (int)ck.nids;
        p.chunks.push_back(ck);
        s0 = s1;
    }
    return true;
}

static int upload_plan(gmmiv_ctx *c, ModelPlan &p)
{
    void *dt, *di, *ds;
    int rc;
    if ((rc = c->scratch(WS_MB_TILES, p.tiles.size() * sizeof(gmmiv_model_tile), &dt))) return rc;
    if ((rc = c->scratch(WS_MB_IDS, p.ids.size() * sizeof(int), &di))) return rc;
    if ((rc = c->scratch(WS_MB_SEG, p.segrel.size() * sizeof(long), &ds))) return rc;
    if (!p.tiles.empty()) GCHK(hipMemcpyAsync(dt, p.tiles.data(), p.tiles.size() * sizeof(gmmiv_model_tile), hipMemcpyHostToDevice, c->stream));
    if (!p.ids.empty()) GCHK(hipMemcpyAsync(di, p.ids.data(), p.ids.size() * sizeof(int), hipMemcpyHostToDevice, c->stream));
    GCHK(hipMemcpyAsync(ds, p.segrel.data(), p.segrel.size() * sizeof(long), hipMemcpyHostToDevice, c->stream));
    if (!p.ftiles.empty()) {
        void *df;
        if ((rc = c->scratch(WS_MB_FTILES, p.ftiles.size() * sizeof(gmmiv_feat_tile), &df))) return rc;
        GCHK(hipMemcpyAsync(df, p.ftiles.data(), p.ftiles.size() * sizeof(gmmiv_feat_tile), hipMemcpyHostToDevice, c->stream));
        p.d_ftiles = (const gmmiv_feat_tile *)df;
    }
    GCHK(hipStreamSynchronize(c->stream));
    p.d_tiles = (const gmmiv_model_tile *)dt; p.d_ids = (const int *)di; p.d_seg = (const long *)ds;
    return GMMIV_OK;
}

static int models_per_chunk(const gmmiv_ctx *c, const gmmiv_gmm_batch *b)
{
    const size_t budget = (size_t)(c->models_scratch_mb > 0 ? c->models_scratch_mb : 0) << 20;
    const size_t n = budget / (b->packed_doubles() * sizeof(double));
    return n < 1 ? 1 : (n > 0x7fff ? 0x7fff : (int)n);
}

static int64_t models_chunk_frames(const gmmiv_ctx *c, const gmmiv_gmm_batch *b)
{
    if (!c->stats_z || b->KS > 15) return 0;
    return gmmiv_z_budget_frames(c, b->nct, 24) / 256 * 256;
}

static int pack_chunk(gmmiv_ctx *c, const gmmiv_gmm_batch *b, const ModelPlan &p, const ModelChunk &ck, double *pt, bool first)
{
    c->t_begin("k_gmm_pack", first);
    GCHK(gmmk_pack_models(c->stream, (int)ck.nids, p.d_ids + ck.id_off, b->C, b->Cpa, b->D, b->KS, b->nct, b->mean, b->sm, b->iv, b->si, b->a, pt));
    c->t_end();
    return GMMIV_OK;
}

static int reserve_packed(gmmiv_ctx *c, const gmmiv_gmm_batch *b, const ModelPlan &p, double **pt)
{
    void *q;
    const int rc = c->scratch(WS_MB_PT, (size_t)(p.max_models ? p.max_models : 1) * b->packed_doubles() * sizeof(double), &q);
    *pt = (double *)q;
    return rc;
}

static int llk_chunk(gmmiv_ctx *c, const gmmiv_gmm_batch *b, const XView &xv, int dt, const int64_t *seg_begin, const ModelPlan &p, const ModelChunk &ck,
                     double *pt, double *lse, const gmmk_zview *z, bool first)
{
    const int64_t f0 = seg_begin[ck.s0], n = seg_begin[ck.s1] - f0;
    int rc;
    XView sub;
    sub.d = gmmiv_x_at(xv, dt, f0); sub.ldx = xv.ldx;
    if ((rc = count_unusable(c, sub, dt, n, b->D))) return rc;
    if ((rc = pack_chunk(c, b, p, ck, pt, first))) return rc;
    const void *xb = gmmiv_x_at(xv, dt, ck.base);
    c->t_begin("k_llk_mfma", first);
    if (z)
        GCHK(gmmk_llk_z_models(c->stream, b->KS, dt == GMMIV_F64, xb, xv.ldx, b->D, pt, (long)b->packed_doubles(), b->nct, p.d_tiles + ck.tile_off,
                               (long)ck.ntiles, lse, (int)(c->use_glds & 1), *z));
    else
        GCHK(gmmk_llk_models(c->stream, b->KS, dt == GMMIV_F64, xb, xv.ldx, b->D, pt, (long)b->packed_doubles(), b->nct, p.d_tiles + ck.tile_off,
                             (long)ck.ntiles, lse, (int)(c->use_glds & 1)));
    c->t_end();
    GCHK(gmmk_count_dead(c->stream, lse + (f0 - ck.base), (long)n, c->d_zero_llk));
    return GMMIV_OK;
}

struct OneModel {
    gmmiv_gmm *g = nullptr;
    int cur = -1;
    ~OneModel() { if (g) gmmiv_gmm_destroy(g); }
    int set(gmmiv_ctx *c, const gmmiv_gmm_batch *b, int m)
    {
        if (m == cur) return GMMIV_OK;
        const double *w = b->w + (size_t)m * b->sw, *mean = b->mean + (size_t)m * b->sm, *iv = b->iv + (size_t)m * b->si;
        const int rc = g ? gmmiv_gmm_set(g, w, mean, iv) : gmmiv_gmm_create(c, b->C, b->D, w, mean, iv, &g);
        if (!rc) cur = m;
        return rc;
    }
};

static int walk_segment(gmmiv_ctx *c, const gmmiv_gmm_batch *b, OneModel &om, int m, const XView &xv, int dt, int64_t f0, int64_t n, XView *sub,
                        double **lse, long **sb)
{
    int rc;
    if ((rc = om.set(c, b, m))) return rc;
    sub->d = gmmiv_x_at(xv, dt, f0); sub->ldx = xv.ldx;
    if ((rc = count_unusable(c, *sub, dt, n, b->D))) return rc;
    if ((rc = run_lse(c, om.g, *sub, dt, n, lse))) return rc;
    void *p;
    if ((rc = c->scratch(WS_MB_SEG, 2 * sizeof(long), &p))) return rc;
    GCHK(gmmk_fill_chunks(c->stream, (long *)p, 1, (long)n, (long)n));
    *sb = (long *)p;
    return GMMIV_OK;
}

int gmmiv_llk_models(gmmiv_ctx *c, const gmmiv_gmm_batch *b, const void *x, int dt, int64_t T, int64_t ldx, const int64_t *seg_begin,
                     const int32_t *seg_model, int64_t nseg, double min_llk, double max_llk, double *llk, double *seg_sum)
{
    int rc = check_batch(c, b, "llk_models");
    if (rc) return rc;
    if ((rc = check_segments(b, "llk_models", T, seg_begin, seg_model, nseg))) return rc;
    if (nseg == 0) return GMMIV_OK;
    XView xv;
    if ((rc = xv.init(c, x, dt, T, ldx, b->D))) return rc;
    DevOut<double> o_llk, o_sum;
    if ((rc = o_llk.init(c, WS_T0, llk, (size_t)T, true))) return rc;
    if ((rc = o_sum.init(c, WS_T1, seg_sum, (size_t)nseg, false))) return rc;
    ModelPlan p;
    if (b->KS <= 15 && plan_chunks(b, seg_begin, seg_model, nseg, (int64_t)1 << 24, models_per_chunk(c, b), p)) {
        if ((rc = upload_plan(c, p))) return rc;
        double *pt;
        void *lse;
        if ((rc = reserve_packed(c, b, p, &pt))) return rc;
        if ((rc = c->scratch(WS_LSE, (size_t)(p.max_span > 0 ? p.max_span : 1) * sizeof(double), &lse))) return rc;
        bool first = true;
        for (size_t k = 0; k < p.chunks.size(); ++k) {
            const ModelChunk &ck = p.chunks[k];
            if (seg_begin[ck.s1] > seg_begin[ck.s0]) {
                if ((rc = llk_chunk(c, b, xv, dt, seg_begin, p, ck, pt, (double *)lse, nullptr, first))) return rc;
                first = false;
            }
            GCHK(gmmk_llk_seg_finalize(c->stream, (const double *)lse, p.d_seg + ck.seg_off, (long)(ck.s1 - ck.s0), min_llk, max_llk,
                                       llk ? o_llk.d + ck.base : nullptr, seg_sum ? o_sum.d + ck.s0 : nullptr, nullptr));
        }
        if ((rc = o_llk.finish())) return rc;
        return o_sum.finish();
    }
    OneModel om;
    if (seg_sum) GCHK(hipMemsetAsync(o_sum.d, 0, (size_t)nseg * sizeof(double), c->stream));
    for (int64_t s = 0; s < nseg; ++s) {
        const int64_t f0 = seg_begin[s], n = seg_begin[s + 1] - f0;
        if (n <= 0) continue;
        XView sub;
        double *lse;
        long *sb;
        if ((rc = walk_segment(c, b, om, seg_model[s], xv, dt, f0, n, &sub, &lse, &sb))) return rc;
        GCHK(gmmk_llk_seg_finalize(c->stream, lse, sb, 1, min_llk, max_llk, llk ? o_llk.d + f0 : nullptr, seg_sum ? o_sum.d + s : nullptr, nullptr));
    }
    if ((rc = o_llk.finish())) return rc;
    return o_sum.finish();
}

static int stats_models(gmmiv_ctx *c, const gmmiv_gmm_batch *b, const void *x, int dt, int64_t T, int64_t ldx, const int64_t *seg_begin,
                        const int32_t *seg_model, int64_t nseg, double *N, double *F, double *S, double *seg_llk, bool second, const char *who)
{
    int rc = check_batch(c, b, who);
    if (rc) return rc;
    if ((rc = check_segments(b, who, T, seg_begin, seg_model, nseg))) return rc;
    if (!N || !F || (second && !S)) { gmmiv_set_error("%s: %s are required", who, second ? "N, F and S" : "N and F"); return GMMIV_ERR_ARG; }
    if (nseg == 0) return GMMIV_OK;
    XView xv;
    if ((rc = xv.init(c, x, dt, T, ldx, b->D))) return rc;
    const size_t SV = (size_t)b->C * b->D;
    DevOut<double> o_n, o_f, o_s, o_l;
    if ((rc = o_n.init(c, WS_T0, N, (size_t)nseg * b->C, false))) return rc;
    if ((rc = o_f.init(c, WS_T1, F, (size_t)nseg * SV, false))) return rc;
    if (second && (rc = o_s.init(c, WS_T5, S, (size_t)nseg * SV, false))) return rc;
    if ((rc = o_l.init(c, WS_T4, seg_llk, 2 * (size_t)nseg, false))) return rc;
    auto finish = [&]() { int r = o_n.finish(); if (!r) r = o_f.finish(); if (!r && second) r = o_s.finish(); if (!r) r = o_l.finish(); return r; };
    ModelPlan p;
    const int64_t Tc = models_chunk_frames(c, b);
    if (Tc > 0 && plan_chunks(b, seg_begin, seg_model, nseg, Tc, models_per_chunk(c, b), p)) {
        if ((rc = upload_plan(c, p))) return rc;
        gmmk_zview z;
        double *pt, *lse;
        if ((rc = reserve_packed(c, b, p, &pt))) return rc;
        if ((rc = gmmiv_z_reserve(c, b->nct, p.max_span, true, &z, &lse))) return rc;
        bool first = true;
        for (size_t k = 0; k < p.chunks.size(); ++k) {
            const ModelChunk &ck = p.chunks[k];
            const void *xb = gmmiv_x_at(xv, dt, ck.base);
// ... 237 lines not shown
```

### lia_ral_amd/csrc/ctx.h

```cpp
#pragma once
#include <hip/hip_runtime.h>
#include <stdint.h>
#include <stdio.h>
#include <string.h>
#include <stdlib.h>
#include <time.h>

#include <map>
#include <string>
#include <vector>

#include "../../include/gmmiv.h"

void gmmiv_set_error(const char *fmt, ...);

#include "kopts.h"

#define GBIND(c)                                                                                    \
    do {                                                                                            \
        GCHK(hipSetDevice((c)->device));                                                            \
        gmmiv_kopts_bind(&(c)->ko);                                                                 \
    } while (0)

#define GCHK(expr)                                                                                  \
    do {                                                                                            \
        hipError_t _e = (hipError_t)(expr);                                                         \
        if (_e != hipSuccess) {                                                                     \
            gmmiv_set_error("%s:%d: %s -> %s", __FILE__, __LINE__, #expr, hipGetErrorString(_e));   \
            return GMMIV_ERR_HIP;                                                                   \
        }                                                                                           \
    } while (0)

enum { WS_X = 0, WS_LSE, WS_PART, WS_SEG, WS_SMALL, WS_T0, WS_T1, WS_T2, WS_T3, WS_T4, WS_T5, WS_T6, WS_T7, WS_T8,
       WS_T9, WS_TIV, WS_LP, WS_AUX, WS_SLAB, WS_SLOTS, WS_FLAGS, WS_Z, WS_EIT, WS_INV,
       WS_GFLAG, WS_NORM, WS_FEAT_OFF, WS_FEAT_OUT, WS_FEAT_IDX, WS_FEAT_M0, WS_FEAT_M1, WS_FEAT_M2, WS_FEAT_M3,
       WS_NORM_OFF, WS_NORM_STATE, WS_NORM_DECAY,
       WS_MB_PT, WS_MB_TILES, WS_MB_IDS, WS_MB_SEG, WS_MB_OFF, WS_MB_FTILES, WS_MB_OFFSRC,
       WS_TR_IDX, WS_TR_NLLK, WS_TR_LLKW, WS_TR_TILES, WS_TR_TAB, WS_TR_PART, WS_TR_ROW,
       WS_IVT_M, WS_IVT_S, WS_IVT_OUT, WS_IVT_A, WS_IVT_B, WS_IVT_Y, WS_IVT_Q, WS_IVT_MAT, WS_IVT_TAB,
       WS_COUNT };

struct gmmiv_ctx {
    int device = 0;
    hipStream_t stream = nullptr;
    bool own_stream = false;
    void *ws[WS_COUNT] = {};
    size_t ws_size[WS_COUNT] = {};
    long use_glds = 1;
    long em_chunks = 0;
    long timing = 0;
    long dbg = 0;
    long prune_log2 = 0;
    double prune_arg() const { return prune_log2 > 0 ? -(double)prune_log2 * 0.6931471805599453 : -__builtin_inf(); }
    double prune_thr() const { return prune_log2 > 0 ? __builtin_ldexp(1.0, -(int)prune_log2) : 0.0; }
    long wg_waves = 8;
    long stats_z = 1;
    long topc_use_lanes = 4;
    long topc_rank2 = 1;
    long topc_rank_direct = 0;
    long topc_fused = 1;
    long assume_finite = 0;
    unsigned long long *d_zero_llk = nullptr, *d_screened = nullptr;
    long topc_fallbacks = 0;
    long topc_z = 1;
    long tv_acc_mb = 8192;
    long tv_md_device = 1;
    long tv_mstep_solve = 1;
    long tv_stats_split = 1;
    long tv_tett_direct = 1;
    long tv_batch = 1024;
    gmmiv_kopts ko;
    struct Hook { gmmiv_hook_fn fn = nullptr; void *user = nullptr; void call() const { if (fn) fn(user); } };
    Hook hook_tv_a_ready, hook_md_factored;
    long z_scratch_mb = 16384;
    long models_scratch_mb = 2048;
    long trials_scratch_mb = 2048;
    long trials_piece = 0;
    long iv_trials_anchor = 0;
    long iv_trials_piece = 0;
    int n_cu = 256;
    std::vector<double> plda_ftjf;
    struct PldaK { std::vector<double> K; double alpha; };
    std::map<long, PldaK> plda_k;
    std::vector<struct gmmiv_comm *> comms;
    size_t total_mem = 0;
    enum { NSLOT = 6 };
    std::vector<hipEvent_t> ev0[NSLOT], ev1[NSLOT];
    const char *ev_name[NSLOT] = {};
    int ev_used[NSLOT] = {};
    int ev_cur = -1, ev_last = -1;

    int scratch(int slot, size_t bytes, void **out)
    {
        if (bytes == 0) bytes = 8;
        if (ws_size[slot] < bytes) {
            if (ws[slot]) {
                GCHK(hipStreamSynchronize(stream));
                GCHK(hipFree(ws[slot]));
                ws[slot] = nullptr;
                ws_size[slot] = 0;
            }
            size_t want = bytes + bytes / 8;
            static const bool trace = [] { const char *e = getenv("GMMIV_TRACE_ALLOC"); return e && *e && *e != '0'; }();
            timespec t0, t1;
            if (trace) clock_gettime(CLOCK_MONOTONIC, &t0);
            hipError_t me = hipMalloc(&ws[slot], want);
            if (trace) {
                clock_gettime(CLOCK_MONOTONIC, &t1);
                fprintf(stderr, "[gmmiv] workspace %d: hipMalloc of %.1f MiB took %.2f ms\n", slot, want / 1048576.0,
                        (t1.tv_sec - t0.tv_sec) * 1e3 + (t1.tv_nsec - t0.tv_nsec) * 1e-6);
            }
            if (me != hipSuccess) {
                (void)hipGetLastError();
                ws[slot] = nullptr;
                gmmiv_set_error("device workspace %d: hipMalloc of %zu MiB failed (%s); lower the \"z_scratch_mb\" / \"tv_batch\" options or free device memory",
                                slot, want >> 20, hipGetErrorString(me));
                return GMMIV_ERR_HIP;
            }
            ws_size[slot] = want;
        }
        *out = ws[slot];
        return GMMIV_OK;
    }
    void t_begin(const char *name, bool first = true)
    {
        if (!timing) return;
        int s = -1;
        for (int i = 0; i < NSLOT; ++i)
            if (ev_name[i] && !strcmp(ev_name[i], name)) { s = i; break; }
        if (s < 0)
            for (int i = 0; i < NSLOT; ++i)
                if (!ev_name[i]) { s = i; break; }
        if (s < 0) s = NSLOT - 1;
        if (ev_name[s] == nullptr || strcmp(ev_name[s], name) != 0 || first) ev_used[s] = 0;
        ev_name[s] = name;
        if ((int)ev0[s].size() <= ev_used[s]) {
            hipEvent_t a = nullptr, b = nullptr;
            (void)hipEventCreate(&a); (void)hipEventCreate(&b);
            ev0[s].push_back(a); ev1[s].push_back(b);
        }
        ev_cur = s;
        (void)hipEventRecord(ev0[s][ev_used[s]], stream);
    }
    void t_end()
    {
// ... 85 lines not shown
```

### lia_ral_amd/csrc/devutil.h

```cpp
#pragma once
#include <hip/hip_runtime.h>
#include <stdint.h>

typedef double d4 __attribute__((ext_vector_type(4)));

#define MFMA_F64(a, b, c) __builtin_amdgcn_mfma_f64_16x16x4f64((a), (b), (c), 0, 0, 0)

#define GMMIV_NEG_BIG (-1.0e300)
#define GMMIV_ZERO_LLK (-745.1332191019412)
#define GMMIV_PAD_LOGIT (-1.0e9)

__device__ __forceinline__ double gexp(double x)
{
    x = fmax(x, -750.0);
    const double n = __builtin_rint(x * 1.4426950408889634074);
    double r = __builtin_fma(n, -6.93147180369123816490e-01, x);
    r = __builtin_fma(n, -1.90821492927058770002e-10, r);
    double p = 1.6059043836821613e-10;
    p = __builtin_fma(p, r, 2.08767569878681e-09);
    p = __builtin_fma(p, r, 2.505210838544172e-08);
    p = __builtin_fma(p, r, 2.755731922398589e-07);
    p = __builtin_fma(p, r, 2.7557319223985893e-06);
    p = __builtin_fma(p, r, 2.48015873015873e-05);
    p = __builtin_fma(p, r, 1.984126984126984e-04);
    p = __builtin_fma(p, r, 1.388888888888889e-03);
    p = __builtin_fma(p, r, 8.333333333333333e-03);
    p = __builtin_fma(p, r, 4.1666666666666664e-02);
    p = __builtin_fma(p, r, 1.6666666666666666e-01);
    p = __builtin_fma(p, r, 0.5);
    p = __builtin_fma(p, r, 1.0);
    p = __builtin_fma(p, r, 1.0);
    return __builtin_ldexp(p, (int)n);
}

__device__ __forceinline__ void gexp_table_init(double *tab, int tid)
{
    if (tid < 32) tab[tid] = exp2((double)tid * 0.03125);
}
__device__ __forceinline__ double gexp_t(double x, const double *tab)
{
    x = fmax(x, -750.0);
    const double k = __builtin_rint(x * 46.16624130844683);
    double r = __builtin_fma(k, -0.021660849219188094, x);
    r = __builtin_fma(k, -1.733101967801894e-10, r);
    const int ki = (int)k;
    const double tj = tab[ki & 31];
    double p = 1.984126984126984e-04;
    p = __builtin_fma(p, r, 1.388888888888889e-03);
    p = __builtin_fma(p, r, 8.333333333333333e-03);
    p = __builtin_fma(p, r, 4.1666666666666664e-02);
    p = __builtin_fma(p, r, 1.6666666666666666e-01);
    p = __builtin_fma(p, r, 0.5);
    p = __builtin_fma(p, r, 1.0);
    p = p * r;
    return __builtin_ldexp(__builtin_fma(tj, p, tj), ki >> 5);
}

__device__ __forceinline__ double gexp_scaled(double x, int E, const double *tab)
{
    x = fmax(x, -4.0e7);
    const double k = __builtin_rint(x * 46.16624130844683);
    double r = __builtin_fma(k, -0.021660849219188094, x);
    r = __builtin_fma(k, -1.733101967801894e-10, r);
    const int ki = (int)k;
    const double tj = tab[ki & 31];
    double p = 1.984126984126984e-04;
    p = __builtin_fma(p, r, 1.388888888888889e-03);
    p = __builtin_fma(p, r, 8.333333333333333e-03);
    p = __builtin_fma(p, r, 4.1666666666666664e-02);
    p = __builtin_fma(p, r, 1.6666666666666666e-01);
    p = __builtin_fma(p, r, 0.5);
    p = __builtin_fma(p, r, 1.0);
    p = p * r;
    int n = (ki >> 5) - E;
    n = n < -2000 ? -2000 : n;
    return __builtin_ldexp(__builtin_fma(tj, p, tj), n);
}
#ifndef GEXP_TAB_BITS
#define GEXP_TAB_BITS 11
#endif
#define GEXP_TAB_N (1 << GEXP_TAB_BITS)
#if GEXP_TAB_BITS == 11
#define GEXP_TAB_SCALE 2954.639443740597
#define GEXP_TAB_HI 0.00033845076904981397
#define GEXP_TAB_LO 2.7079718246904592e-12
#define GEXP_TAB_LN2N 0.00033845077175778578
#elif GEXP_TAB_BITS == 6
#define GEXP_TAB_SCALE 92.33248261689366
#define GEXP_TAB_HI 0.010830424609594047
#define GEXP_TAB_LO 8.66550983900947e-11
#define GEXP_TAB_LN2N 0.010830424696249145
#else
#error "GEXP_TAB_BITS must be 6 or 11"
#endif
__device__ __forceinline__ void gexp_tab_init(double *tab, int tid, int nthreads)
{
    for (int j = tid; j < GEXP_TAB_N; j += nthreads) tab[j] = exp2((double)j * (1.0 / GEXP_TAB_N));
}
__device__ __forceinline__ double gexp_tab_poly(double r)
{
#if GEXP_TAB_BITS == 11
    double p = 1.6666666666666666e-01;
#else
    double p = 8.333333333333333e-03;
    p = __builtin_fma(p, r, 4.1666666666666664e-02);
    p = __builtin_fma(p, r, 1.6666666666666666e-01);
#endif
    p = __builtin_fma(p, r, 0.5);
    p = __builtin_fma(p, r, 1.0);
    return p * r;
}
__device__ __forceinline__ void gexp_tab_reduce(double x, int &ki, double &r)
{
    const double k = __builtin_rint(x * GEXP_TAB_SCALE);
#ifdef GEXP_TAB_TWO_STEP
    r = __builtin_fma(k, -GEXP_TAB_HI, x);
    r = __builtin_fma(k, -GEXP_TAB_LO, r);
#else
    r = __builtin_fma(k, -GEXP_TAB_LN2N, x);
#endif
    ki = (int)k;
}
__device__ __forceinline__ double gexp_tab_finish(int ki, double r, int E, const double *tab)
{
    const double tj = tab[ki & (GEXP_TAB_N - 1)];
    return __builtin_ldexp(__builtin_fma(tj, gexp_tab_poly(r), tj), (ki >> GEXP_TAB_BITS) - E);
}
__device__ __forceinline__ double gexp_tab_scaled(double x, int E, const double *tab)
{
    int ki;
    double r;
    gexp_tab_reduce(x, ki, r);
    return gexp_tab_finish(ki, r, E, tab);
}
__device__ __forceinline__ int gexp_tab_exponent(double x)
{
    return ((int)__builtin_rint(x * GEXP_TAB_SCALE)) >> GEXP_TAB_BITS;
}
__device__ __forceinline__ int gexp_exponent(double x)
{
    x = fmax(x, -4.0e7);
    return ((int)__builtin_rint(x * 46.16624130844683)) >> 5;
}

template <int CTRL> __device__ __forceinline__ int dpp_i32(int v) { return __builtin_amdgcn_update_dpp(0, v, CTRL, 0xf, 0xf, false); }
__device__ __forceinline__ int row_max_i32(int v)
{
    int o;
    o = dpp_i32<0x128>(v); v = o > v ? o : v;
    o = dpp_i32<0x124>(v); v = o > v ? o : v;
    o = dpp_i32<0x122>(v); v = o > v ? o : v;
    o = dpp_i32<0x121>(v); v = o > v ? o : v;
    return v;
}

__device__ __forceinline__ int row_min_i32(int v)
{
    int o;
    o = dpp_i32<0x128>(v); v = o < v ? o : v;
    o = dpp_i32<0x124>(v); v = o < v ? o : v;
    o = dpp_i32<0x122>(v); v = o < v ? o : v;
    o = dpp_i32<0x121>(v); v = o < v ? o : v;
    return v;
}

__device__ __forceinline__ void wave_argmax_f64(double &v, int &c)
{
#define GMMIV_ARGMAX_STEP(CTRL)                                                                    \
    {                                                                                              \
        const int ohi = dpp_i32<CTRL>(__double2hiint(v)), olo = dpp_i32<CTRL>(__double2loint(v)); \
        const int oc = dpp_i32<CTRL>(c);                                                           \
        const double ov = __hiloint2double(ohi, olo);                                              \
        if (ov > v || (ov == v && oc < c)) { v = ov; c = oc; }                                     \
    }
    GMMIV_ARGMAX_STEP(0x128)
    GMMIV_ARGMAX_STEP(0x124)
    GMMIV_ARGMAX_STEP(0x122)
    GMMIV_ARGMAX_STEP(0x121)
#undef GMMIV_ARGMAX_STEP
    const double v0 = __hiloint2double(__builtin_amdgcn_readlane(__double2hiint(v), 0), __builtin_amdgcn_readlane(__double2loint(v), 0));
// ... 11 lines not shown
}

__device__ __forceinline__ double dpp_f64_0x128(double v) { return __hiloint2double(dpp_i32<0x128>(__double2hiint(v)), dpp_i32<0x128>(__double2loint(v))); }
__device__ __forceinline__ double dpp_f64_0x124(double v) { return __hiloint2double(dpp_i32<0x124>(__double2hiint(v)), dpp_i32<0x124>(__double2loint(v))); }
__device__ __forceinline__ double dpp_f64_0x122(double v) { return __hiloint2double(dpp_i32<0x122>(__double2hiint(v)), dpp_i32<0x122>(__double2loint(v))); }
__device__ __forceinline__ double dpp_f64_0x121(double v) { return __hiloint2double(dpp_i32<0x121>(__double2hiint(v)), dpp_i32<0x121>(__double2loint(v))); }
__device__ __forceinline__ double readlane_f64u(double v, int l)
{
    return __hiloint2double(__builtin_amdgcn_readlane(__double2hiint(v), l), __builtin_amdgcn_readlane(__double2loint(v), l));
}
__device__ __forceinline__ double wave_sum_f64_dpp(double v)
{
    v += dpp_f64_0x128(v); v += dpp_f64_0x124(v); v += dpp_f64_0x122(v); v += dpp_f64_0x121(v);
    return (readlane_f64u(v, 0) + readlane_f64u(v, 16)) + (readlane_f64u(v, 32) + readlane_f64u(v, 48));
}
__device__ __forceinline__ double half_sum_f64_dpp(double v, bool hi)
{
    v += dpp_f64_0x128(v); v += dpp_f64_0x124(v); v += dpp_f64_0x122(v); v += dpp_f64_0x121(v);
    const double a = readlane_f64u(v, 0) + readlane_f64u(v, 16), b = readlane_f64u(v, 32) + readlane_f64u(v, 48);
    return hi ? b : a;
}
__device__ __forceinline__ double half_max_f64_dpp(double v, bool hi)
{
    v = fmax(v, dpp_f64_0x128(v)); v = fmax(v, dpp_f64_0x124(v)); v = fmax(v, dpp_f64_0x122(v)); v = fmax(v, dpp_f64_0x121(v));
    const double a = fmax(readlane_f64u(v, 0), readlane_f64u(v, 16)), b = fmax(readlane_f64u(v, 32), readlane_f64u(v, 48));
    return hi ? b : a;
}
__device__ __forceinline__ double half_min_f64_dpp(double v, bool hi)
{
    v = fmin(v, dpp_f64_0x128(v)); v = fmin(v, dpp_f64_0x124(v)); v = fmin(v, dpp_f64_0x122(v)); v = fmin(v, dpp_f64_0x121(v));
    const double a = fmin(readlane_f64u(v, 0), readlane_f64u(v, 16)), b = fmin(readlane_f64u(v, 32), readlane_f64u(v, 48));
    return hi ? b : a;
}
__device__ __forceinline__ double wave_max_f64_dpp(double v)
{
    v = fmax(v, dpp_f64_0x128(v)); v = fmax(v, dpp_f64_0x124(v)); v = fmax(v, dpp_f64_0x122(v)); v = fmax(v, dpp_f64_0x121(v));
    return fmax(fmax(readlane_f64u(v, 0), readlane_f64u(v, 16)), fmax(readlane_f64u(v, 32), readlane_f64u(v, 48)));
}
__device__ __forceinline__ double wave_min_f64_dpp(double v)
{
    v = fmin(v, dpp_f64_0x128(v)); v = fmin(v, dpp_f64_0x124(v)); v = fmin(v, dpp_f64_0x122(v)); v = fmin(v, dpp_f64_0x121(v));
    return fmin(fmin(readlane_f64u(v, 0), readlane_f64u(v, 16)), fmin(readlane_f64u(v, 32), readlane_f64u(v, 48)));
}

__device__ __forceinline__ double shfl_xor_f64(double v, int mask)
{
    int lo = __double2loint(v), hi = __double2hiint(v);
    lo = __shfl_xor(lo, mask, 64);
    hi = __shfl_xor(hi, mask, 64);
    return __hiloint2double(hi, lo);
}

__device__ __forceinline__ double wave_sum_f64(double v)
{
#pragma unroll
    for (int o = 32; o > 0; o >>= 1) v += shfl_xor_f64(v, o);
    return v;
}
__device__ __forceinline__ double wave_max_f64(double v)
{
#pragma unroll
    for (int o = 32; o > 0; o >>= 1) v = fmax(v, shfl_xor_f64(v, o));
    return v;
}

__device__ __forceinline__ int xswz(int t) { return ((t << 1) ^ ((t & 1) << 4)) & 31; }

__device__ __forceinline__ int xrot(int t) { return ((t & 1) << 4) + (((t >> 1) & 7) << 1); }

__device__ __forceinline__ int eit_slot(int t) { return (t & ~15) | ((t & 3) << 2) | ((t >> 2) & 3); }

__device__ __forceinline__ int div_by_magic(unsigned e, unsigned magic) { return magic ? (int)__umulhi(e, magic) : (int)e; }
static inline unsigned gmmiv_div_magic(int D) { return D == 1 ? 0u : (unsigned)((1ULL << 32) / (unsigned)D + 1); }

#define GMMIV_UNUSABLE_BOUND 1e18
#define GMMIV_UNUSABLE_READ_AS 1e10
#ifndef GMMIV_FEAT_SANE_OFF
__device__ __forceinline__ float feat_sane(float v) { return __builtin_fabsf(v) <= (float)GMMIV_UNUSABLE_BOUND ? v : (float)GMMIV_UNUSABLE_READ_AS; }
__device__ __forceinline__ double feat_sane(double v) { return __builtin_fabs(v) <= GMMIV_UNUSABLE_BOUND ? v : GMMIV_UNUSABLE_READ_AS; }
#else
__device__ __forceinline__ float feat_sane(float v) { return v; }
__device__ __forceinline__ double feat_sane(double v) { return v; }
#endif
template <typename T> struct feat_load;
template <> struct feat_load<float> {
    static __device__ __forceinline__ double get(const void *p, long i) { return (double)feat_sane(((const float *)p)[i]); }
    static __device__ __forceinline__ double raw(const void *p, long i) { return (double)((const float *)p)[i]; }
};
template <> struct feat_load<double> {
    static __device__ __forceinline__ double get(const void *p, long i) { return feat_sane(((const double *)p)[i]); }
    static __device__ __forceinline__ double raw(const void *p, long i) { return ((const double *)p)[i]; }
};
```

### lia_ral_amd/csrc/gmm_kernels.h

```cpp
#pragma once
#include <hip/hip_runtime.h>

#include "kopts.h"
#include "../../include/gmmiv.h"

#define GMMK_KS_GENERIC 99
#define GMMK_MAX_DIM 4096
int gmmk_ks_for_dim(int D);
int gmmk_rl_for_ks(int KS);
int gmmk_pack_model(hipStream_t st, int C, int D, int KS, int nct, int Cp64, const double *w, const double *mean,
                    const double *iv, double *a, double *lwc, double *Pt, double *meanT, double *ivT);
int gmmk_llk(hipStream_t st, int KS, int x_f64, const void *x, long T, long ldx, int D, const double *Pt, int nct,
             double *lse, int use_glds, int wg_waves);
int gmmk_llk_finalize(hipStream_t st, const double *lse, long T, double lo, double hi, double *llk_out,
                      double *partial , double scale_c, double scale_r, double *dst_clamped,
                      double *dst_raw, double scale_n = 0.0, double *dst_count = nullptr);
int gmmk_add_scalar(hipStream_t st, double *dst, double v);
int gmmk_count_dead(hipStream_t st, const double *lse, long T, unsigned long long *cnt);
int gmmk_rows_sum_groups(hipStream_t st, long n, int ngroups, const int *rb, const double *src, double *dst);
int gmmk_stats(hipStream_t st, int KS, int sq, int x_f64, const void *x, long ldx, int D, int C, const double *Pt,
               int nct, const double *lse, double lse_shift, const long *seg_begin, int nseg, double *out0,
               double *out1, int mode, int wg_waves, double prune_arg);
int gmmk_em_reduce(hipStream_t st, const double *part, int nseg, int C, int Cp, int D, int KS, double *acc);
int gmmk_em_get(hipStream_t st, int C, int D, const double *acc, const double *prev_mean, const double *prev_cov,
                double *w, double *mean, double *cov);
int gmmk_topc_frames_per_block(int Cp64, int D);
int gmmk_topc_determine(hipStream_t st, int x_f64, const void *x, long T, long ldx, int D, int C, int Cp,
                        const double *meanT, const double *ivT, const double *lwc, const double *w, int ctop,
                        int complete, double lo, double hi, int *idx, double *lk, double *nlk, double *nllk,
                        double *nw, double *llk);
int gmmk_build_xa(hipStream_t st, int x_f64, const void *x, long ldx, int D, long n, int sq, int NC, double *Xa);
int gmmk_scatter_em(hipStream_t st, int C, int D, int NC, const double *S, double scale, double *acc);
int gmmk_scatter_nf(hipStream_t st, int C, int D, int NC, const double *S, double *Nrow, double *Frow);
size_t gmmk_topc_big_scratch_doubles(long T, int Cp);
int gmmk_topc_determine_big(hipStream_t st, int x_f64, const void *x, long T, long ldx, int D, int C, int Cp,
                            const double *meanT, const double *ivT, const double *lwc, const double *w, int ctop,
                            int complete, double lo, double hi, int *idx, double *lk, double *nlk, double *nllk,
                            double *nw, double *llk, double *zs);
int gmmk_topc_use_big(hipStream_t st, int x_f64, const void *x, long T, long ldx, int D, const double *mean,
                      const double *iv, const double *lwc, int C, int ctop, const int *idx, const double *nllk, int complete,
                      double lo, double hi, double *llk);
int gmmk_topc_use(hipStream_t st, int x_f64, const void *x, long T, long ldx, int D, const double *mean,
                  const double *iv, const double *lwc, int C, int ctop, const int *idx, const double *nllk, int complete,
                  double lo, double hi, double *llk);
int gmmk_frame_moments(hipStream_t st, int x_f64, const void *x, long T, long ldx, int D, double *partial,
                       int max_blocks, double *acc);
int gmmk_variance_control(hipStream_t st, int C, int D, double *cov, double flooring, double ceiling,
                          const double *cov_signal, unsigned long long *counts);
int gmmk_reciprocal(hipStream_t st, long n, const double *in, double *out);
int gmmk_gather_frames(hipStream_t st, int x_f64, const void *x, long ldx, int D, const long *idx, long n, void *out);
int gmmk_segment_means(hipStream_t st, const double *v, long ld, const long *item, long nitem, double *part, const long *pair_off,
                       const long *pair_len, long npair, double *out);
int gmmk_topgauss_select(hipStream_t st, long T, int cap, double mass, int fixed_count, const double *w, int *idx, const double *lk,
                         const double *llk, int *count, double *snsw, double *snsl, unsigned long long *capped);
int gmmk_flag_frames(hipStream_t st, int x_f64, const void *x, long T, long ldx, int D, unsigned char *flag, int *any);
int gmmk_fill_chunks(hipStream_t st, long *dst, int nseg, long per, long n);
int gmmk_count_flags(hipStream_t st, const unsigned char *flag, long T, unsigned long long *cnt);
int gmmk_gather_runs(hipStream_t st, int x_f64, const void *x, long ldx, int D, const long *runs, long nrun, void *out);

struct gmmk_zview {
    double *zbuf;
    long nfb;
    int *eit;
    double *inv;
    int *efin;
};
int gmmk_llk_z(hipStream_t st, int KS, int x_f64, const void *x, long T, long ldx, int D, const double *Pt, int nct,
               double *lse, int use_glds, const gmmk_zview &z);
int gmmk_llk_models(hipStream_t st, int KS, int x_f64, const void *x, long ldx, int D, const double *Pt, long pt_stride, int nct,
                    const gmmiv_model_tile *tiles, long ntiles, double *lse, int use_glds);
int gmmk_llk_z_models(hipStream_t st, int KS, int x_f64, const void *x, long ldx, int D, const double *Pt, long pt_stride, int nct,
                      const gmmiv_model_tile *tiles, long ntiles, double *lse, int use_glds, const gmmk_zview &z);
int gmmk_const_models(hipStream_t st, int G, int C, int Cp, int D, const double *w, long sw, const double *mean, long sm, const double *iv,
                      long si, double *a, double *lwc);
int gmmk_pack_models(hipStream_t st, int n, const int *ids, int C, int Cp, int D, int KS, int nct, const double *mean, long sm,
                     const double *iv, long si, const double *a, double *Pt);
int gmmk_llk_seg_finalize(hipStream_t st, const double *lse, const long *sb, long nseg, double lo, double hi, double *llk_out, double *seg_sum,
                          double *seg_llk);
int gmmk_map_adapt_models(hipStream_t st, int G, int C, int D, const double *N, const double *F, const double *count, long count_stride,
                          const double *w0, const double *mean0, const double *cur, long cur_stride, int method, int mean_adapt,
                          int weight_adapt, double mean_reg, double weight_reg, double mean_alpha, double *mean_out, double *w_out);
int gmmk_map_adapt_models_full(hipStream_t st, int G, int C, int D, const double *N, const double *F, const double *S, const double *count,
                               long count_stride, const double *w0, const double *mean0, const double *cov0, const double *cur_mean,
                               long cur_mean_stride, const double *cur_cov, long cur_cov_stride, int method, int mean_adapt, int var_adapt,
                               int weight_adapt, double mean_reg, double var_reg, double weight_reg, double mean_alpha, double *mean_out,
                               double *cov_out, double *w_out, int *status);
int gmmk_normalize_models(hipStream_t st, int G, int C, int D, const double *w, long w_stride, double *mean, double *cov, int nb_it,
                          int mean_only);
int gmmk_acc_to_rows(hipStream_t st, int C, int D, const double *acc, double *Nrow, double *Frow, double *Srow);
int gmmk_topc_cap(void);
int gmmk_llk_topc(hipStream_t st, int KS, int x_f64, const void *x, long T, long ldx, int D, const double *Pt, int nct, int use_glds,
                  int ctop, double *cand, int *cnt, double *theta, double *slow, int *efin);
int gmmk_topc_rank(hipStream_t st, int x_f64, const void *x, long n, long ldx, int D, int C, const double *cand, const int *cnt,
                   const double *theta, const double *slow, const int *efin, const double *mean, const double *iv, const double *lwc,
                   const double *w, int ctop, int complete, double lo, double hi, int *idx, double *lk, double *nlk, double *nllk,
                   double *nw, double *llk, int *flag, long *redo, int stats, long *wide);
int gmmk_topc_scatter(hipStream_t st, long n, int ctop, const long *redo, const int *sidx, const double *slk, const double *snlk,
                      const double *snllk, const double *snw, const double *sllk, int *idx, double *lk, double *nlk, double *nllk, double *nw,
                      double *llk);
int gmmk_posteriors(hipStream_t st, int x_f64, const void *x, long T, long ldx, int D, int C, int Cp, const double *meanT,
                    const double *ivT, const double *lwc, const double *lse, double *gamma);
int gmmk_stats_z_groups(int nct);
int gmmk_stats_z_wg_per_cu(void);
int gmmk_stats_z(hipStream_t st, int KS, int sq, int x_f64, const void *x, long ldx, int D, int C, int nct, const gmmk_zview &z,
                 double scale, const long *seg_begin, int nseg, double *out0, double *out1, int mode, int accum, double prune_thr);
int gmmk_stats_z_rows(hipStream_t st, int KS, int x_f64, const void *x, long ldx, int D, int C, int nct, const gmmk_zview &z,
                      const long *seg_begin, int nseg, double *N, double *F, double *X2, double prune_thr);
size_t gmmk_topc_z_lds(int nct, int D);
int gmmk_topc_from_z(hipStream_t st, int x_f64, const void *x, long n, long ldx, int D, int C, int nct, const gmmk_zview &z,
                     const double *mean, const double *iv, const double *lwc, const double *w, int ctop, int complete, double lo, double hi,
                     int *idx, double *lk, double *nlk, double *nllk, double *nw, double *llk, int *flag);
int gmmk_topc_use16(hipStream_t st, int x_f64, const void *x, long T, long ldx, int D, const double *mean, const double *iv,
                    const double *lwc, int C, int ctop, const int *idx, const double *nllk, int complete, double lo, double hi, double *llk, int four);
int gmmk_topc_use4_multi(hipStream_t st, int x_f64, const void *x, long T, long ldx, int D, const void *clients, int n_clients, int ctop,
                         const int *idx, const double *nllk, int complete, double lo, double hi, double *llk);
int gmmk_post_from_z(hipStream_t st, long n, int C, int nct, const gmmk_zview &z, double *gamma);

size_t gmmk_feat_offset_doubles(int nct, int D);
int gmmk_feat_pack_offset(hipStream_t st, const double *off, int C, int D, int nct, double *offP);
int gmmk_feat_comp(hipStream_t st, int x_f64, int o_f64, const void *x, long ldx, long n, int D, int nct, const gmmk_zview &z,
                   const double *offP, void *out, long ldo);
int gmmk_feat_pack_offsets(hipStream_t st, int n, const int *ids, const double *off, long stride, int C, int D, int nct, double *offP);
int gmmk_feat_blocks_per_tile(void);
int gmmk_feat_comp_models(hipStream_t st, int x_f64, int o_f64, const void *x, long ldx, long n, int D, int nct, const gmmk_zview &z,
                          const double *offP, long off_stride, const gmmiv_feat_tile *tiles, long ntiles, void *out, long ldo);
int gmmk_feat_sub(hipStream_t st, int x_f64, int o_f64, const void *x, long ldx, long n, int D, const double *P, const double *lse, void *out,
                  long ldo);
int gmmk_feat_map(hipStream_t st, int x_f64, int o_f64, const void *x, long ldx, long T, int D, int C, const int *best, const double *cd_mean,
                  const double *cd_cov, const double *ci_mean, const double *ci_cov, void *out, long ldo);
int gmmk_scatter_runs(hipStream_t st, int x_f64, void *x, long ldx, int D, const long *runs, long nrun, const void *in);

int gmmk_moments_groups(hipStream_t st, int x_f64, const void *x, long ldx, int D, const long *runs, long nrun, long ngroups, double *partial,
                        double *acc);
int gmmk_moments_stats(hipStream_t st, long ngroups, int D, const double *acc, double *mean, double *sd);
int gmmk_feat_norm_apply(hipStream_t st, int x_f64, int o_f64, const void *x, long ldx, int D, const long *runs, long nrun, long ngroups,
                         const double *mean, const double *sd, void *out, long ldo);
size_t gmmk_online_units(long nfiles, long frames);
long gmmk_online_chunk(void);
int gmmk_feat_norm_online(hipStream_t st, int n_cu, int x_f64, int o_f64, const void *x, long ldx, int D, const long *file_begin, long nfiles,
                          long W, long L, long max_units, long *chunk_off, double *state, double *decay, void *out, long ldo);
long gmmk_energy_stage_frames(int x_f64);
int gmmk_energy_em(hipStream_t st, int x_f64, const void *x, long ldx, const long *runs, long nrun, long nfiles, const long *order, long max_frames,
                   int C, int nb_it, double flooring, double ceiling, double alpha, double *model, double *threshold, int *status);
int gmmk_energy_select(hipStream_t st, int x_f64, const void *x, long ldx, const long *runs, long nrun, long nfiles, const double *threshold,
                       long *n_above, long *seg_count, const long *seg_off, long *seg_begin, long *seg_len);
```

### lia_ral_amd/csrc/gmm_kernels.hip

```cpp
#include <atomic>
#include "devutil.h"
#include "lds_attr.h"
#include "gmm_kernels.h"

typedef double d2v __attribute__((ext_vector_type(2)));

__device__ __forceinline__ void gmm_const_one(int c, int C, int D, const double *__restrict__ w, const double *__restrict__ mean,
                                              const double *__restrict__ iv, double *__restrict__ a, double *__restrict__ logwcst)
{
    if (c >= C) { a[c] = GMMIV_NEG_BIG; logwcst[c] = GMMIV_NEG_BIG; return; }
    double sl = 0.0, sm = 0.0;
    for (int d = 0; d < D; ++d) {
        double v = iv[(size_t)c * D + d], m = mean[(size_t)c * D + d];
        sl += log(v);
        sm += m * m * v;
    }
    double lw = (w[c] > 0.0) ? log(w[c]) : GMMIV_NEG_BIG;
    double lc = lw - 0.5 * D * 1.8378770664093454836 + 0.5 * sl;
    lc = fmax(lc, GMMIV_NEG_BIG);
    logwcst[c] = lc;
    a[c] = fmax(lc - 0.5 * sm, GMMIV_NEG_BIG);
}
__global__ void k_gmm_const(int C, int Cp, int D, const double *__restrict__ w,
                            const double *__restrict__ mean, const double *__restrict__ iv,
                            double *__restrict__ a, double *__restrict__ logwcst)
{
    int c = blockIdx.x * blockDim.x + threadIdx.x;
    if (c >= Cp) return;
    gmm_const_one(c, C, D, w, mean, iv, a, logwcst);
}
__global__ void k_gmm_const_batch(int C, int Cp, int D, const double *__restrict__ w, long sw, const double *__restrict__ mean, long sm,
                                  const double *__restrict__ iv, long si, double *__restrict__ a, double *__restrict__ logwcst)
{
    const int c = blockIdx.x * blockDim.x + threadIdx.x;
    const size_t g = blockIdx.y;
    if (c >= Cp) return;
    gmm_const_one(c, C, D, w + g * sw, mean + g * sm, iv + g * si, a + g * Cp, logwcst + g * Cp);
}

__device__ __forceinline__ double gmm_pack_one(long e, int C, int D, int KS, const double *__restrict__ mean,
                                               const double *__restrict__ iv, const double *__restrict__ a)
{
    const int NR = 2 * KS + 2;
    int lane = e & 63;
    int row = (e >> 6) % NR;
    int ct = (e >> 6) / NR;
    int j = lane & 15, q = lane >> 4;
    int c = ct * 16 + j;
    double v = 0.0;
    if (row < 2 * KS) {
        int s = row < KS ? row : row - KS;
        int k = 4 * s + q;
        if (c < C && k < D) {
            double ivv = iv[(size_t)c * D + k];
            v = row < KS ? mean[(size_t)c * D + k] * ivv : -0.5 * ivv;
        }
    } else if (row == 2 * KS) {
        v = c < C ? fmax(a[c], GMMIV_PAD_LOGIT) : GMMIV_PAD_LOGIT;
    } else {
        v = q == 0 ? (c < C ? fmax(a[c], GMMIV_PAD_LOGIT) : GMMIV_PAD_LOGIT) : (q == 1 ? -1.0 : 0.0);
    }
    return v;
}
__global__ void k_gmm_pack(int C, int D, int KS, int nct, const double *__restrict__ mean,
                           const double *__restrict__ iv, const double *__restrict__ a,
                           double *__restrict__ Pt)
{
    long e = (long)blockIdx.x * blockDim.x + threadIdx.x;
    long total = (long)nct * (2 * KS + 2) * 64;
    if (e >= total) return;
    Pt[e] = gmm_pack_one(e, C, D, KS, mean, iv, a);
}
__global__ void k_gmm_pack_batch(int C, int Cp, int D, int KS, int nct, const int *__restrict__ ids, const double *__restrict__ mean, long sm,
                                 const double *__restrict__ iv, long si, const double *__restrict__ a, double *__restrict__ Pt)
{
    long e = (long)blockIdx.x * blockDim.x + threadIdx.x;
    long total = (long)nct * (2 * KS + 2) * 64;
    if (e >= total) return;
    const size_t g = (size_t)ids[blockIdx.y];
    Pt[(size_t)blockIdx.y * total + e] = gmm_pack_one(e, C, D, KS, mean + g * sm, iv + g * si, a + g * Cp);
}

__global__ void k_gmm_transpose(int C, int Cp, int D, const double *__restrict__ mean,
                                const double *__restrict__ iv, double *__restrict__ meanT,
                                double *__restrict__ ivT)
{
    long e = (long)blockIdx.x * blockDim.x + threadIdx.x;
    if (e >= (long)D * Cp) return;
    int c = e % Cp, d = e / Cp;
    meanT[e] = c < C ? mean[(size_t)c * D + d] : 0.0;
    ivT[e] = c < C ? iv[(size_t)c * D + d] : 0.0;
}

#define TOPC_CAP 256
#define GMMIV_MIN_FRAME_EXP (-1076)
#ifndef K1_ABL
#define K1_ABL 0
#endif
#ifndef K1_PLAIN_SHARED
#define K1_PLAIN_SHARED 1
#endif
template <int KS, typename XT, int NW, int MODE, bool MM = false>
__global__ __launch_bounds__(NW * 64, 2) void k_llk_mfma(const void *__restrict__ x, long T, long ldx, int D,
                                                  const double *__restrict__ Pt, int nct,
                                                  double *__restrict__ lse_out, int use_glds, int dbg,
                                                  double *__restrict__ zbuf, long nfb, int *__restrict__ eit,
                                                  double *__restrict__ inv_out, int *__restrict__ efin_out,
                                                  const gmmiv_model_tile *__restrict__ tiles, long pt_stride)
{
    constexpr bool WZ = MODE == 1, TC = MODE == 2;
    static_assert(!MM || (MODE != 2 && NW == 8), "a model per segment: plain and stored-likelihood modes, 8 waves");
    constexpr int NR = 2 * KS + 2;
    constexpr int GT = 2;
    constexpr int TILE_D = GT * NR * 64;
    constexpr int PIECES = TILE_D * 8 / 1024;
    extern __shared__ __attribute__((aligned(16))) char smem[];
    double *buf0 = (double *)smem;
    double *buf1 = buf0 + TILE_D;
    double *etab = buf1 + TILE_D;
    int *ccnt = (int *)(etab + GEXP_TAB_N);

    const int tid = threadIdx.x, lane = tid & 63, wave = tid >> 6;
    const int i16 = lane & 15, q = lane >> 4;
    long tb0 = (long)blockIdx.x * (NW * 32);
    long wlo = 0, whi = 0, olo = 0, ohi = 0;
    if constexpr (MM) {
        const gmmiv_model_tile me = tiles[blockIdx.x];
        tb0 = me.first; wlo = me.lo; whi = me.hi; olo = me.lo - me.pad_lo; ohi = me.hi + me.pad_hi;
        Pt += (size_t)me.model * pt_stride;
    }
    const long tb = tb0 + wave * 32;
    gexp_tab_init(etab, tid, NW * 64);
    if (TC) ccnt[tid >> 1] = 0;

    constexpr int NA = TC ? KS : 2 * KS;
    double A[2][NA];
#pragma unroll
    for (int h = 0; h < 2; ++h) {
        const long t = tb + h * 16 + i16;
#pragma unroll
        for (int s = 0; s < KS; ++s) {
            const int k = 4 * s + q;
            double v = 0.0;
            if ((MM ? (t >= wlo && t < whi) : t < T) && k < D) v = feat_load<XT>::get(x, t * ldx + k);
            A[h][s] = v;
            if (!TC) A[h][NA - KS + s] = v * v;
        }
    }

    const int ntiles = nct / GT;
    auto stage = [&](double *dst, int tile) {
        const char *src = (const char *)(Pt + (size_t)tile * TILE_D);
        if (use_glds) {
            if (PIECES % NW == 0) {
#pragma unroll
                for (int j = 0; j < PIECES / NW; ++j) {
                    const int p = wave + NW * j;
                    __builtin_amdgcn_global_load_lds(
                        (const __attribute__((address_space(1))) void *)(src + p * 1024 + lane * 16),
                        (__attribute__((address_space(3))) void *)((char *)dst + p * 1024), 16, 0, 0);
                }
            } else {
                for (int p = wave; p < PIECES; p += NW)
                    __builtin_amdgcn_global_load_lds(
                        (const __attribute__((address_space(1))) void *)(src + p * 1024 + lane * 16),
                        (__attribute__((address_space(3))) void *)((char *)dst + p * 1024), 16, 0, 0);
            }
        } else {
            for (int p = wave; p < PIECES; p += NW) {
                uint4 v = *(const uint4 *)(src + p * 1024 + lane * 16);
                *(uint4 *)((char *)dst + p * 1024 + lane * 16) = v;
            }
        }
    };

    double sacc[2][4];
    int E[2][4], nref[2][4];
#pragma unroll
    for (int h = 0; h < 2; ++h)
#pragma unroll
        for (int r = 0; r < 4; ++r) { sacc[h][r] = 0.0; E[h][r] = -(1 << 30); nref[h][r] = -(1 << 30); }

    const bool late = NW == 8 && ((wave >> 1) & 1);
    float thf[2][4], lmaxf[2][4];
#pragma unroll
    for (int h = 0; h < 2; ++h)
#pragma unroll
        for (int r = 0; r < 4; ++r) { thf[h][r] = -__builtin_inff(); lmaxf[h][r] = -__builtin_inff(); }
    d4 acc[GT][2];
    auto mfma_phase = [&](const double *cur) __attribute__((always_inline)) {
    double zv = 0.0;
    if (TC) asm volatile("" : "+v"(zv));
#pragma unroll
    for (int g = 0; g < GT; ++g) {
        const double a = cur[(g * NR + 2 * KS) * 64 + lane];
        acc[g][0] = (d4){a, a, a, a};
        acc[g][1] = acc[g][0];
    }
#pragma unroll
    for (int s = 0; s < 2 * KS; ++s) {
        const double b0 = cur[(0 * NR + s) * 64 + lane];
        const double b1 = cur[(1 * NR + s) * 64 + lane];
        double a0, a1;
        if (TC && s >= KS && !(K1_ABL & 256)) { a0 = __builtin_fma(A[0][s - KS], A[0][s - KS], zv); a1 = __builtin_fma(A[1][s - KS], A[1][s - KS], zv); }
        else if (TC && s >= KS) { a0 = A[0][s - KS]; a1 = A[1][s - KS]; }
        else { a0 = A[0][s < NA ? s : 0]; a1 = A[1][s < NA ? s : 0]; }
        acc[0][0] = MFMA_F64(a0, b0, acc[0][0]);
        acc[1][0] = MFMA_F64(a0, b1, acc[1][0]);
        acc[0][1] = MFMA_F64(a1, b0, acc[0][1]);
        acc[1][1] = MFMA_F64(a1, b1, acc[1][1]);
    }
    };
    auto epi_phase = [&](int te) __attribute__((always_inline)) {
        if (K1_ABL & 1) {
#pragma unroll
            for (int g = 0; g < GT; ++g)
#pragma unroll
                for (int h = 0; h < 2; ++h) asm volatile("" ::"v"(acc[g][h]));
            return;
        }
        if (TC) {
#ifndef TC_SCHED
#define TC_SCHED 1
#endif
            const bool refresh = TC_SCHED == 0 ? (te < 8 || (te < 16 && (te & 1) == 1) || (te < 32 && (te & 3) == 3) || (te & 7) == 7 || te == ntiles - 1)
                                               : ((te & (te + 1)) == 0 || te == ntiles - 1);
            const int kth = dbg > 0 ? dbg : 16;
#pragma unroll
            for (int h = 0; h < 2; ++h) {
                int nm[4], k0[4], k1[4];
                bool hit0[4], hit1[4];
                bool grow = false;
                if (!(K1_ABL & 128))
#pragma unroll
                for (int r = 0; r < 4; ++r)
                    lmaxf[h][r] = fmaxf(lmaxf[h][r], (float)fmax(acc[0][h][r], acc[1][h][r]));
// ... 157 lines not shown
#pragma unroll
                for (int h = 0; h < 2; ++h) __builtin_nontemporal_store(acc[g][h], (d4 *)(zw + ((size_t)g * nfb + h) * 256));
            if (i16 == 0 && !(K1_ABL & 32)) {
                typedef int i4 __attribute__((ext_vector_type(4)));
                int *ew = eit + (size_t)te * (nfb * 16) + tb + 4 * q;
#pragma unroll
                for (int h = 0; h < 2; ++h) *(i4 *)(ew + h * 16) = (i4){E[h][0], E[h][1], E[h][2], E[h][3]};
            }
            return;
        }
        int nm[2][4];
        bool grow = false;
#pragma unroll
        for (int h = 0; h < 2; ++h)
#pragma unroll
            for (int r = 0; r < 4; ++r) {
                nm[h][r] = gexp_tab_exponent(fmax(acc[0][h][r], acc[1][h][r]));
                grow |= nm[h][r] - E[h][r] >= 64;
            }
        if (__builtin_amdgcn_ballot_w64(grow) != 0) {
#pragma unroll
            for (int h = 0; h < 2; ++h)
#pragma unroll
                for (int r = 0; r < 4; ++r)
                    if (nm[h][r] - E[h][r] >= 64) {
                        int sh = E[h][r] - nm[h][r];
                        sh = sh < -2000 ? -2000 : sh;
                        sacc[h][r] = __builtin_ldexp(sacc[h][r], sh);
                        E[h][r] = nm[h][r];
                    }
        }
        unsigned need = 0;
#pragma unroll
        for (int h = 0; h < 2; ++h)
#pragma unroll
            for (int r = 0; r < 4; ++r) {
                nref[h][r] = nm[h][r] > nref[h][r] ? nm[h][r] : nref[h][r];
                need |= (__builtin_amdgcn_ballot_w64(nm[h][r] > nref[h][r] - 57) != 0 ? 1u : 0u) << (h * 4 + r);
            }
        if (__builtin_popcount(need) > 3) {
#pragma unroll
            for (int h = 0; h < 2; ++h)
#pragma unroll
                for (int r = 0; r < 4; ++r)
                    sacc[h][r] += gexp_tab_scaled(acc[0][h][r], E[h][r], etab) + gexp_tab_scaled(acc[1][h][r], E[h][r], etab);
        } else if (need) {
#pragma unroll
            for (int h = 0; h < 2; ++h)
#pragma unroll
                for (int r = 0; r < 4; ++r)
                    if (need & (1u << (h * 4 + r)))
                        sacc[h][r] += gexp_tab_scaled(acc[0][h][r], E[h][r], etab) + gexp_tab_scaled(acc[1][h][r], E[h][r], etab);
        }
    };
    stage(buf0, 0);
    __syncthreads();
    auto step = [&](int tl, bool staged, bool is_late, bool first) __attribute__((always_inline)) {
        double *cur = (tl & 1) ? buf1 : buf0;
        double *nxt = (tl & 1) ? buf0 : buf1;
        if (staged && (TC || dbg < 2) && !(K1_ABL & 16)) stage(nxt, tl + 1);
        if (!is_late) {
            mfma_phase(cur);
            epi_phase(tl);
        } else {
            if (!first) epi_phase(tl - 1);
            mfma_phase(cur);
        }
        if (WZ) {
            if (is_late) asm volatile("s_waitcnt vmcnt(0)" ::: "memory");
            if (!(K1_ABL & 16)) asm volatile("s_waitcnt lgkmcnt(0)\n\ts_barrier" ::: "memory");
        } else {
            __syncthreads();
        }
    };
    if (!late) {
        for (int tl = 0; tl + 1 < ntiles; ++tl) step(tl, true, false, false);
        if (ntiles > 0) step(ntiles - 1, false, false, false);
    } else {
        if (ntiles > 1) step(0, true, true, true);
        for (int tl = 1; tl + 1 < ntiles; ++tl) step(tl, true, true, false);
        if (ntiles > 0) step(ntiles - 1, false, true, ntiles == 1);
    }
    if (late && ntiles > 0) epi_phase(ntiles - 1);
#pragma unroll
    for (int h = 0; h < 2; ++h)
#pragma unroll
        for (int r = 0; r < 4; ++r) {
            int Em = E[h][r];
#pragma unroll
            for (int o = 1; o < 16; o <<= 1) { const int oe = __shfl_xor(Em, o, 64); Em = oe > Em ? oe : Em; }
            int sh = E[h][r] - Em;
            sh = sh < -2000 ? -2000 : sh;
            double sv = __builtin_ldexp(sacc[h][r], sh);
#pragma unroll
            for (int o = 1; o < 16; o <<= 1) sv += shfl_xor_f64(sv, o);
            const long t = tb + h * 16 + q + 4 * r;
            if (TC) {
                if (i16 == 0 && t < T) { lse_out[t] = (double)thf[h][r]; inv_out[t] = sv; efin_out[t] = Em; }
                continue;
            }
            if (i16 == 0 && (MM ? (t >= wlo && t < whi) : t < T)) {
                const bool ok = sv > 0.0 && sv < __builtin_inf() && Em > GMMIV_MIN_FRAME_EXP;
                lse_out[t] = ok ? log(sv) + (double)Em * 0.693147180559945309417 : -__builtin_inf();
                if (WZ) { inv_out[t] = ok ? 1.0 / sv : 0.0; efin_out[t] = ok ? Em : 0; }
            }
        }
    if (TC) {
        __syncthreads();
        const long t = (long)blockIdx.x * (NW * 32) + tid;
        if (tid < NW * 32 && t < T) eit[t] = ccnt[tid];
    }
}

__global__ __launch_bounds__(256) void k_llk_finalize(const double *__restrict__ lse, long T, double lo,
                                                     double hi, double *__restrict__ llk_out,
                                                     double *__restrict__ partial)
{
    __shared__ double red[3][4];
    double sc = 0.0, sr = 0.0, sn = 0.0;
    for (long t = (long)blockIdx.x * blockDim.x + threadIdx.x; t < T; t += (long)gridDim.x * blockDim.x) {
        const double v = lse[t];
        const double c = fmin(fmax(v, lo), hi);
        if (llk_out) llk_out[t] = c;
        sc += c;
        const bool fin = v > -__builtin_inf() && v < __builtin_inf();
        sr += fin ? v : 0.0;
        sn += fin ? 1.0 : 0.0;
    }
    sc = wave_sum_f64(sc);
    sr = wave_sum_f64(sr);
    sn = wave_sum_f64(sn);
    const int lane = threadIdx.x & 63, wave = threadIdx.x >> 6;
    if (lane == 0) { red[0][wave] = sc; red[1][wave] = sr; red[2][wave] = sn; }
    __syncthreads();
    if (threadIdx.x == 0) {
        partial[3 * blockIdx.x] = red[0][0] + red[0][1] + red[0][2] + red[0][3];
        partial[3 * blockIdx.x + 1] = red[1][0] + red[1][1] + red[1][2] + red[1][3];
        partial[3 * blockIdx.x + 2] = red[2][0] + red[2][1] + red[2][2] + red[2][3];
    }
}

__global__ __launch_bounds__(256) void k_count_dead(const double *__restrict__ lse, long T, unsigned long long *__restrict__ cnt)
{
    unsigned n = 0;
    for (long t = (long)blockIdx.x * blockDim.x + threadIdx.x; t < T; t += (long)gridDim.x * blockDim.x) {
        const double v = lse[t];
        n += (v > -__builtin_inf() && v < __builtin_inf()) ? 0u : 1u;
    }
    const unsigned long long b = __ballot(n > 0);
    if (b == 0) return;
    for (int o = 32; o > 0; o >>= 1) n += __shfl_xor(n, o, 64);
    if ((threadIdx.x & 63) == 0) atomicAdd(cnt, (unsigned long long)n);
}
int gmmk_count_dead(hipStream_t st, const double *lse, long T, unsigned long long *cnt)
{
    if (T <= 0 || !cnt) return 0;
    long nb = (T + 1023) / 1024;
    if (nb > 1024) nb = 1024;
    k_count_dead<<<(unsigned)nb, 256, 0, st>>>(lse, T, cnt);
    return (int)hipGetLastError();
}

__global__ void k_reduce_partials(const double *__restrict__ partial, int nb, int n, double s0, double s1, double s2,
                                  double *__restrict__ dst0, double *__restrict__ dst1, double *__restrict__ dst2)
{
    if (threadIdx.x < n) {
        double s = 0.0;
        for (int b = 0; b < nb; ++b) s += partial[(size_t)b * n + threadIdx.x];
        if (threadIdx.x == 0 && dst0) *dst0 += s0 * s;
        if (threadIdx.x == 1 && dst1) *dst1 += s1 * s;
        if (threadIdx.x == 2 && dst2) *dst2 += s2 * s;
    }
}

__global__ void k_add_scalar(double *dst, double v) { *dst += v; }

template <int KS, bool SQ, typename XT, int NW, bool PRUNE>
__global__ __launch_bounds__(NW * 64, 2) void k_stats_mfma(const void *__restrict__ x, long ldx, int D, int C,
                                                    const double *__restrict__ Pt, int nct,
                                                    const double *__restrict__ lse, double lse_shift,
                                                    const long *__restrict__ seg_begin, int nseg, int ngrp,
                                                    double *__restrict__ out0, double *__restrict__ out1,
                                                    int mode, unsigned magicD, double prune_arg)
{
    constexpr int NR = 2 * KS + 2;
    constexpr int Dp = 4 * KS;
    constexpr int RL = ((Dp + 2 + 31) / 32) * 32;
    constexpr int JT = RL / 16;
    constexpr int FT = 64;
// ... 480 lines not shown
    }
    double r = (complete && nontop_llk) ? nontop_llk[t] : -__builtin_inf();
    double M = wave_max_f64(fmax(z, r));
    double s = live ? gexp(z - M) : 0.0;
    s = wave_sum_f64(s);
    if (lane == 0) {
        if (r > -__builtin_inf()) s += gexp(r - M);
        llk_out[t] = fmin(fmax(M + log(s), lo), hi);
    }
}

template <typename XT>
__global__ __launch_bounds__(256) void k_posteriors(const void *__restrict__ x, long ldx, int D, int C, int Cp,
                                                    const double *__restrict__ meanT, const double *__restrict__ ivT,
                                                    const double *__restrict__ lwc, const double *__restrict__ lse,
                                                    double *__restrict__ gamma)
{
    extern __shared__ double xs[];
    const long t = blockIdx.x;
    for (int d = threadIdx.x; d < D; d += 256) xs[d] = feat_load<XT>::get(x, t * ldx + d);
    __syncthreads();
    double l = lse[t];
    if (!(l > -__builtin_inf())) l = __builtin_inf();
    for (int c = threadIdx.x; c < C; c += 256) {
        double acc = 0.0;
        for (int d = 0; d < D; ++d) {
            const double dx = xs[d] - meanT[(size_t)d * Cp + c];
            acc = __builtin_fma(dx * dx, ivT[(size_t)d * Cp + c], acc);
        }
        const double z = __builtin_fma(-0.5, acc, lwc[c]);
        gamma[t * C + c] = z == z ? exp(z - l) : 0.0;
    }
}

template <typename XT>
__global__ __launch_bounds__(256) void k_frame_moments(const void *__restrict__ x, long T, long ldx, int D,
                                                       double *__restrict__ partial)
{
    __shared__ double red[2][4][64];
    const int d = threadIdx.x & 63, rs = threadIdx.x >> 6;
    double s = 0.0, ss = 0.0;
    for (int d0 = 0; d0 < D; d0 += 64) {
        s = 0.0; ss = 0.0;
        const int dd = d0 + d;
        if (dd < D)
            for (long t = (long)blockIdx.x * 4 + rs; t < T; t += (long)gridDim.x * 4) {
                const double v = feat_load<XT>::raw(x, t * ldx + dd);
                s += v;
                ss = __builtin_fma(v, v, ss);
            }
        red[0][rs][d] = s;
        red[1][rs][d] = ss;
        __syncthreads();
        if (rs == 0 && dd < D) {
            partial[(size_t)blockIdx.x * 2 * D + dd] = red[0][0][d] + red[0][1][d] + red[0][2][d] + red[0][3][d];
            partial[(size_t)blockIdx.x * 2 * D + D + dd] = red[1][0][d] + red[1][1][d] + red[1][2][d] + red[1][3][d];
        }
        __syncthreads();
    }
}
__global__ __launch_bounds__(256) void k_moments_reduce(const double *__restrict__ partial, int nb, int n, double *__restrict__ acc)
{
    __shared__ double red[4][64];
    const int lane = threadIdx.x & 63, slot = threadIdx.x >> 6;
    const int e = blockIdx.x * 4 + slot;
    double s = 0.0;
    if (e < n)
        for (int b = lane; b < nb; b += 64) s += partial[(size_t)b * n + e];
    red[slot][lane] = s;
    __syncthreads();
    if (lane == 0 && e < n) {
        double t = 0.0;
        for (int l = 0; l < 64; ++l) t += red[slot][l];
        acc[e] += t;
    }
}

#define HIPCHK(e)                                                         \
    do {                                                                  \
        hipError_t _e = (e);                                              \
        if (_e != hipSuccess) return (int)_e;                             \
    } while (0)

int gmmk_ks_for_dim(int D)
{
    if (D <= 16) return 4;
    if (D <= 32) return 8;
    if (D <= 60) return 15;
    if (D <= 80) return 20;
    return D <= GMMK_MAX_DIM ? GMMK_KS_GENERIC : 0;
}
int gmmk_rl_for_ks(int KS) { return ((4 * KS + 2 + 31) / 32) * 32; }

int gmmk_pack_model(hipStream_t st, int C, int D, int KS, int nct, int Cp64, const double *w, const double *mean,
                    const double *iv, double *a, double *lwc, double *Pt, double *meanT, double *ivT)
{
    const int Cp = Cp64 > nct * 16 ? Cp64 : nct * 16;
    k_gmm_const<<<(Cp + 255) / 256, 256, 0, st>>>(C, Cp, D, w, mean, iv, a, lwc);
    long total = (long)nct * (2 * KS + 2) * 64;
    if (KS != GMMK_KS_GENERIC) k_gmm_pack<<<(unsigned)((total + 255) / 256), 256, 0, st>>>(C, D, KS, nct, mean, iv, a, Pt);
    long tt = (long)D * Cp64;
    k_gmm_transpose<<<(unsigned)((tt + 255) / 256), 256, 0, st>>>(C, Cp64, D, mean, iv, meanT, ivT);
    return (int)hipGetLastError();
}

template <int KS, typename XT, int NW, int MODE>
static int launch_llk(hipStream_t st, const void *x, long T, long ldx, int D, const double *Pt, int nct,
                      double *lse, int use_glds, const gmmk_zview &z = gmmk_zview{})
{
    constexpr int NR = 2 * KS + 2;
    const size_t lds = 2 * 2 * NR * 64 * sizeof(double) + GEXP_TAB_N * sizeof(double) + (MODE == 2 ? NW * 32 * sizeof(int) : 0);
    HIPCHK((gmmiv_lds_attr<k_llk_mfma<KS, XT, NW, MODE>>(lds)));
    const unsigned grid = (unsigned)((T + NW * 32 - 1) / (NW * 32));
    k_llk_mfma<KS, XT, NW, MODE><<<grid, NW * 64, lds, st>>>(x, T, ldx, D, Pt, nct, lse, use_glds & 1, use_glds >> 8, z.zbuf, z.nfb, z.eit, z.inv, z.efin, nullptr, 0);
    return (int)hipGetLastError();
}

template <int KS, typename XT, int MODE>
static int launch_llk_models(hipStream_t st, const void *x, long ldx, int D, const double *Pt, long pt_stride, int nct, const gmmiv_model_tile *tiles,
                             long ntiles, double *lse, int use_glds, const gmmk_zview &z)
{
    constexpr int NR = 2 * KS + 2;
    const size_t lds = 2 * 2 * NR * 64 * sizeof(double) + GEXP_TAB_N * sizeof(double);
    HIPCHK((gmmiv_lds_attr<k_llk_mfma<KS, XT, 8, MODE, true>>(lds)));
    k_llk_mfma<KS, XT, 8, MODE, true><<<(unsigned)ntiles, 8 * 64, lds, st>>>(x, 0, ldx, D, Pt, nct, lse, use_glds & 1, 0, z.zbuf, z.nfb, z.eit, z.inv, z.efin, tiles, pt_stride);
    return (int)hipGetLastError();
}
#define MM_CASE(K, MODE)                                                                                                  \
    case K:                                                                                                               \
        return x_f64 ? launch_llk_models<K, double, MODE>(st, x, ldx, D, Pt, pt_stride, nct, tiles, ntiles, lse, use_glds, z) \
                     : launch_llk_models<K, float, MODE>(st, x, ldx, D, Pt, pt_stride, nct, tiles, ntiles, lse, use_glds, z);
int gmmk_llk_models(hipStream_t st, int KS, int x_f64, const void *x, long ldx, int D, const double *Pt, long pt_stride, int nct,
                    const gmmiv_model_tile *tiles, long ntiles, double *lse, int use_glds)
{
    if (ntiles <= 0) return 0;
    const gmmk_zview z = {};
    switch (KS) {
        MM_CASE(4, 0) MM_CASE(8, 0) MM_CASE(15, 0)
    }
    return -1;
}
int gmmk_llk_z_models(hipStream_t st, int KS, int x_f64, const void *x, long ldx, int D, const double *Pt, long pt_stride, int nct,
                      const gmmiv_model_tile *tiles, long ntiles, double *lse, int use_glds, const gmmk_zview &z)
{
    if (ntiles <= 0) return 0;
    switch (KS) {
        MM_CASE(4, 1) MM_CASE(8, 1) MM_CASE(15, 1)
    }
    return -1;
}
#undef MM_CASE

int gmmk_const_models(hipStream_t st, int G, int C, int Cp, int D, const double *w, long sw, const double *mean, long sm, const double *iv,
                      long si, double *a, double *lwc)
{
    if (G <= 0) return 0;
    k_gmm_const_batch<<<dim3((unsigned)((Cp + 255) / 256), (unsigned)G), 256, 0, st>>>(C, Cp, D, w, sw, mean, sm, iv, si, a, lwc);
    return (int)hipGetLastError();
}
int gmmk_pack_models(hipStream_t st, int n, const int *ids, int C, int Cp, int D, int KS, int nct, const double *mean, long sm,
                     const double *iv, long si, const double *a, double *Pt)
{
    if (n <= 0) return 0;
    const long total = (long)nct * (2 * KS + 2) * 64;
    k_gmm_pack_batch<<<dim3((unsigned)((total + 255) / 256), (unsigned)n), 256, 0, st>>>(C, Cp, D, KS, nct, ids, mean, sm, iv, si, a, Pt);
    return (int)hipGetLastError();
}

__global__ __launch_bounds__(256) void k_llk_seg_finalize(const double *__restrict__ lse, const long *__restrict__ sb, double lo, double hi,
                                                         double *__restrict__ llk_out, double *__restrict__ seg_sum,
                                                         double *__restrict__ seg_llk)
{
    __shared__ double red[3][4];
    const int s = blockIdx.x;
    const long b = sb[s], e = sb[s + 1];
    double sc = 0.0, sr = 0.0, sn = 0.0;
    for (long t = b + threadIdx.x; t < e; t += 256) {
        const double v = lse[t];
        const double c = fmin(fmax(v, lo), hi);
        if (llk_out) llk_out[t] = c;
        sc += c;
        const bool fin = v > -__builtin_inf() && v < __builtin_inf();
        sr += fin ? v : 0.0;
        sn += fin ? 1.0 : 0.0;
    }
    sc = wave_sum_f64(sc);
    sr = wave_sum_f64(sr);
    sn = wave_sum_f64(sn);
    const int lane = threadIdx.x & 63, wave = threadIdx.x >> 6;
    if (lane == 0) { red[0][wave] = sc; red[1][wave] = sr; red[2][wave] = sn; }
    __syncthreads();
    if (threadIdx.x == 0) {
        if (seg_sum) seg_sum[s] = red[0][0] + red[0][1] + red[0][2] + red[0][3];
        if (seg_llk) {
            seg_llk[2 * s] = red[1][0] + red[1][1] + red[1][2] + red[1][3];
            seg_llk[2 * s + 1] = red[2][0] + red[2][1] + red[2][2] + red[2][3];
        }
    }
}
int gmmk_llk_seg_finalize(hipStream_t st, const double *lse, const long *sb, long nseg, double lo, double hi, double *llk_out, double *seg_sum,
                          double *seg_llk)
{
    if (nseg <= 0) return 0;
    k_llk_seg_finalize<<<(unsigned)nseg, 256, 0, st>>>(lse, sb, lo, hi, llk_out, seg_sum, seg_llk);
    return (int)hipGetLastError();
}

__device__ __forceinline__ double map_ml_weight(double n, double count) { return count > 0.0 ? n / count : 0.0; }
__device__ __forceinline__ double map_mean_one(double ml, double m0, double w, double w0c, double cnt, int method, int mean_adapt, double mean_reg,
                                               double mean_alpha)
{
#pragma clang fp contract(off)
    double r = ml;
    if (method != GMMIV_MAP_NONE && !mean_adapt) r = m0;
    else if (method == GMMIV_MAP_OCC_DEP || method == GMMIV_MAP_MODEL_BASED) {
        const double alpha = w * (double)(unsigned long)cnt;
        const double a = alpha / (alpha + mean_reg);
        r = (1 - a) * m0 + a * ml;
    } else if (method == GMMIV_MAP_CONST) {
        r = (mean_alpha * m0) + ((1 - mean_alpha) * ml);
    } else if (method == GMMIV_MAP_CONST2) {
        r = ((mean_alpha * w0c * m0) + ((1 - mean_alpha) * w * ml)) / (w0c * mean_alpha + w * (1 - mean_alpha));
    }
    return r;
}
__global__ __launch_bounds__(256) void k_map_adapt_mean(long total, int C, int D, const double *__restrict__ N, const double *__restrict__ F,
// ... 93 lines not shown
    else if (e < C + 2 * CD) Srow[e - C - CD] = acc[e];
}
__global__ __launch_bounds__(256) void k_map_adapt_weight(int C, const double *__restrict__ N, const double *__restrict__ count, long count_stride,
                                                         const double *__restrict__ w0, int method, int weight_adapt, double weight_reg,
                                                         double *__restrict__ w_out)
{
#pragma clang fp contract(off)
    __shared__ double ssum;
    const size_t g = blockIdx.x;
    const double cnt = count[g * count_stride];
    const bool occ = (method == GMMIV_MAP_OCC_DEP || method == GMMIV_MAP_MODEL_BASED) && weight_adapt;
    for (int c = threadIdx.x; c < C; c += blockDim.x) {
        const double w = map_ml_weight(N[g * C + c], cnt);
        double r = method == GMMIV_MAP_NONE ? w : w0[c];
        if (occ) {
            const double alpha = w * (double)(unsigned long)cnt, a = alpha / (alpha + weight_reg);
            r = a * w + (1 - a) * w0[c];
        }
        w_out[g * C + c] = r;
    }
    if (!occ) return;
    __syncthreads();
    if (threadIdx.x == 0) {
        double s = 0.0;
        for (int c = 0; c < C; ++c) s += w_out[g * C + c];
        ssum = s;
    }
    __syncthreads();
    for (int c = threadIdx.x; c < C; c += blockDim.x) w_out[g * C + c] /= ssum;
}
int gmmk_map_adapt_models(hipStream_t st, int G, int C, int D, const double *N, const double *F, const double *count, long count_stride,
                          const double *w0, const double *mean0, const double *cur, long cur_stride, int method, int mean_adapt,
                          int weight_adapt, double mean_reg, double weight_reg, double mean_alpha, double *mean_out, double *w_out)
{
    if (G <= 0) return 0;
    const long total = (long)G * C * D;
    const unsigned blocks = (unsigned)((total + 255) / 256 > 16384 ? 16384 : (total + 255) / 256);
    k_map_adapt_mean<<<blocks, 256, 0, st>>>(total, C, D, N, F, count, count_stride, w0, mean0, cur, cur_stride, method, mean_adapt, mean_reg,
                                             mean_alpha, mean_out);
    if (w_out) k_map_adapt_weight<<<(unsigned)G, 256, 0, st>>>(C, N, count, count_stride, w0, method, weight_adapt, weight_reg, w_out);
    return (int)hipGetLastError();
}

int gmmk_map_adapt_models_full(hipStream_t st, int G, int C, int D, const double *N, const double *F, const double *S, const double *count,
                               long count_stride, const double *w0, const double *mean0, const double *cov0, const double *cur_mean,
                               long cur_mean_stride, const double *cur_cov, long cur_cov_stride, int method, int mean_adapt, int var_adapt,
                               int weight_adapt, double mean_reg, double var_reg, double weight_reg, double mean_alpha, double *mean_out,
                               double *cov_out, double *w_out, int *status)
{
    if (G <= 0) return 0;
    hipError_t e = hipMemsetAsync(status, 0, (size_t)G * sizeof(int), st);
    if (e != hipSuccess) return (int)e;
    if (mean_out || cov_out) {
        const long CD = (long)C * D;
        const unsigned bx = (unsigned)((CD + 255) / 256 > 1024 ? 1024 : (CD + 255) / 256);
        for (int g0 = 0; g0 < G; g0 += 65535) {
            const int ng = G - g0 < 65535 ? G - g0 : 65535;
            const long o = (long)g0 * CD;
            k_map_adapt_full<<<dim3(bx, (unsigned)ng), 256, 0, st>>>(C, D, N + (long)g0 * C, F + o, S ? S + o : nullptr, count + g0 * count_stride, count_stride,
                                                                     w0, mean0, cov0, cur_mean + g0 * cur_mean_stride, cur_mean_stride,
                                                                     cur_cov ? cur_cov + g0 * cur_cov_stride : nullptr, cur_cov_stride, method, mean_adapt,
                                                                     var_adapt, mean_reg, var_reg, mean_alpha, mean_out ? mean_out + o : nullptr,
                                                                     cov_out ? cov_out + o : nullptr, status + g0);
        }
    }
    if (w_out) k_map_adapt_weight<<<(unsigned)G, 256, 0, st>>>(C, N, count, count_stride, w0, method, weight_adapt, weight_reg, w_out);
    return (int)hipGetLastError();
}
int gmmk_normalize_models(hipStream_t st, int G, int C, int D, const double *w, long w_stride, double *mean, double *cov, int nb_it, int mean_only)
{
    if (G <= 0 || nb_it <= 0) return 0;
    const long n = (long)G * D;
    k_normalize_models<<<(unsigned)((n + 63) / 64), 64, 0, st>>>(G, C, D, w, w_stride, mean, cov, nb_it, mean_only);
    return (int)hipGetLastError();
}
int gmmk_acc_to_rows(hipStream_t st, int C, int D, const double *acc, double *Nrow, double *Frow, double *Srow)
{
    const long n = (long)C * (1 + 2 * D);
    k_acc_to_rows<<<(unsigned)((n + 255) / 256), 256, 0, st>>>(C, D, acc, Nrow, Frow, Srow);
    return (int)hipGetLastError();
}

int gmmk_llk(hipStream_t st, int KS, int x_f64, const void *x, long T, long ldx, int D, const double *Pt, int nct,
             double *lse, int use_glds, int wg_waves)
{
    if (T <= 0) return 0;
    if (T <= 32768 && gmmiv_kopts_cur().short_calls) wg_waves = 4;
#define CASE(K)                                                                                      \
    case K:                                                                                          \
        if (wg_waves == 8)                                                                           \
            return x_f64 ? launch_llk<K, double, 8, 0>(st, x, T, ldx, D, Pt, nct, lse, use_glds) \
                         : launch_llk<K, float, 8, 0>(st, x, T, ldx, D, Pt, nct, lse, use_glds); \
        return x_f64 ? launch_llk<K, double, 4, 0>(st, x, T, ldx, D, Pt, nct, lse, use_glds)     \
                     : launch_llk<K, float, 4, 0>(st, x, T, ldx, D, Pt, nct, lse, use_glds);
    switch (KS) {
        CASE(4) CASE(8) CASE(15) CASE(20)
    }
#undef CASE
    return -1;
}

int gmmk_llk_z(hipStream_t st, int KS, int x_f64, const void *x, long T, long ldx, int D, const double *Pt, int nct,
               double *lse, int use_glds, const gmmk_zview &z)
{
    if (T <= 0) return 0;
    const bool small = T <= 32768 && gmmiv_kopts_cur().short_calls;
#define CASE(K)                                                                                   \
    case K:                                                                                       \
        if (small)                                                                                \
            return x_f64 ? launch_llk<K, double, 4, 1>(st, x, T, ldx, D, Pt, nct, lse, use_glds, z) \
                         : launch_llk<K, float, 4, 1>(st, x, T, ldx, D, Pt, nct, lse, use_glds, z); \
        return x_f64 ? launch_llk<K, double, 8, 1>(st, x, T, ldx, D, Pt, nct, lse, use_glds, z)   \
                     : launch_llk<K, float, 8, 1>(st, x, T, ldx, D, Pt, nct, lse, use_glds, z);
    switch (KS) {
        CASE(4) CASE(8) CASE(15)
    }
#undef CASE
    return -1;
}

int gmmk_topc_cap(void) { return TOPC_CAP; }
int gmmk_llk_topc(hipStream_t st, int KS, int x_f64, const void *x, long T, long ldx, int D, const double *Pt, int nct, int use_glds,
                  int ctop, double *cand, int *cnt, double *theta, double *slow, int *efin)
{
    if (T <= 0) return 0;
    if (ctop < 1 || ctop > 16) return -1;
    use_glds = (use_glds & 1) | (ctop << 8);
    const bool small = T <= 32768 && gmmiv_kopts_cur().short_calls;
    const gmmk_zview tc = {cand, 0, cnt, slow, efin};
#define CASE(K)                                                                                                                    \
    case K:                                                                                                                        \
        if (small)                                                                                                                 \
            return x_f64 ? launch_llk<K, double, 4, 2>(st, x, T, ldx, D, Pt, nct, theta, use_glds, tc)        \
                         : launch_llk<K, float, 4, 2>(st, x, T, ldx, D, Pt, nct, theta, use_glds, tc);        \
        return x_f64 ? launch_llk<K, double, 8, 2>(st, x, T, ldx, D, Pt, nct, theta, use_glds, tc)            \
                     : launch_llk<K, float, 8, 2>(st, x, T, ldx, D, Pt, nct, theta, use_glds, tc);
    switch (KS) {
        CASE(4) CASE(8) CASE(15)
    }
#undef CASE
    return -1;
}

int gmmk_llk_finalize(hipStream_t st, const double *lse, long T, double lo, double hi, double *llk_out,
                      double *partial , double scale_c, double scale_r, double *dst_clamped,
                      double *dst_raw, double scale_n, double *dst_count)
{
    if (T <= 0) return 0;
    int nb = (int)((T + 255) / 256);
    if (nb > 256) nb = 256;
    k_llk_finalize<<<nb, 256, 0, st>>>(lse, T, lo, hi, llk_out, partial);
    k_reduce_partials<<<1, 64, 0, st>>>(partial, nb, 3, scale_c, scale_r, scale_n, dst_clamped, dst_raw, dst_count);
    return (int)hipGetLastError();
}

__global__ void k_rows_sum_groups(long n, const int *__restrict__ rb, const double *__restrict__ src, double *__restrict__ dst)
{
    const int g = blockIdx.y, r0 = rb[g], r1 = rb[g + 1];
    for (size_t e = (size_t)blockIdx.x * blockDim.x + threadIdx.x; e < (size_t)n; e += (size_t)gridDim.x * blockDim.x) {
        double s = 0.0;
        for (int r = r0; r < r1; ++r) s += src[(size_t)r * n + e];
        dst[(size_t)g * n + e] = s;
    }
}
int gmmk_rows_sum_groups(hipStream_t st, long n, int ngroups, const int *rb, const double *src, double *dst)
{
    if (n <= 0 || ngroups <= 0) return 0;
    const unsigned bx = (unsigned)((n + 255) / 256 > 1024 ? 1024 : (n + 255) / 256);
    k_rows_sum_groups<<<dim3(bx, (unsigned)ngroups), 256, 0, st>>>(n, rb, src, dst);
    return (int)hipGetLastError();
}

__global__ __launch_bounds__(256) void k_segment_partials(const double *__restrict__ v, long ld, const long *__restrict__ item,
                                                          double *__restrict__ part)
{
    __shared__ double red[4];
    const long i = blockIdx.x;
    const double *row = v + item[3 * i] * ld;
    double s = 0.0;
    for (long t = item[3 * i + 1] + threadIdx.x; t < item[3 * i + 2]; t += 256) s += row[t];
    s = wave_sum_f64(s);
    if ((threadIdx.x & 63) == 0) red[threadIdx.x >> 6] = s;
    __syncthreads();
    if (threadIdx.x == 0) part[i] = red[0] + red[1] + red[2] + red[3];
}
__global__ void k_segment_finish(const double *__restrict__ part, const long *__restrict__ pair_off, const long *__restrict__ pair_len, long npair,
                                 double *__restrict__ out)
{
    const long p = (long)blockIdx.x * blockDim.x + threadIdx.x;
    if (p >= npair) return;
    double s = 0.0;
    for (long i = pair_off[p]; i < pair_off[p + 1]; ++i) s += part[i];
    out[p] = pair_len[p] > 0 ? s / (double)pair_len[p] : 0.0;
}
int gmmk_segment_means(hipStream_t st, const double *v, long ld, const long *item, long nitem, double *part, const long *pair_off,
                       const long *pair_len, long npair, double *out)
{
    if (npair <= 0) return 0;
    if (nitem > 0) k_segment_partials<<<(unsigned)nitem, 256, 0, st>>>(v, ld, item, part);
    k_segment_finish<<<(unsigned)((npair + 127) / 128), 128, 0, st>>>(part, pair_off, pair_len, npair, out);
    return (int)hipGetLastError();
}

__global__ __launch_bounds__(256) void k_topgauss_select(long T, int cap, double mass, int fixed_count, const double *__restrict__ w,
                                                         int *__restrict__ idx, const double *__restrict__ lk, const double *__restrict__ llk,
                                                         int *__restrict__ count, double *__restrict__ snsw, double *__restrict__ snsl,
                                                         unsigned long long *__restrict__ capped)
{
    const long t = (long)blockIdx.x * blockDim.x + threadIdx.x;
    if (t >= T) return;
    const double lk_tot = exp(llk[t]);
    int *ix = idx + t * cap;
    const double *lv = lk + t * cap;
    int n = 0;
    if (fixed_count > 0) n = fixed_count;
    else {
        double val = 0.0;
        for (int j = 0; j < cap; ++j) {
            if (val > mass * lk_tot) break;
// ... 387 lines not shown
```

Baseline: 128.2 Gframe-Gaussian/s.

## Fuse unusable-frame and dead-LLK counting into the LLK kernel; precompute exp table

Removes the separate count_unusable and count_dead passes over frames and LSE. Those counts are now accumulated inside the MFMA log-likelihood kernel through optional counter pointers. The exp2 lookup table is computed once per context into device memory and copied into LDS rather than rebuilt by every workgroup. It also adds a compile-time use_glds template split. This saves a full read of the frame matrix and the LSE array per EM pass, at the cost of atomics and extra registers in the hot kernel.

```diff
diff --git a/lia_ral_amd/csrc/capi_ctx.hip b/lia_ral_amd/csrc/capi_ctx.hip
--- a/lia_ral_amd/csrc/capi_ctx.hip
+++ b/lia_ral_amd/csrc/capi_ctx.hip
@@ -63,6 +63,13 @@
         return GMMIV_ERR_HIP;
     }
     c->d_screened = c->d_zero_llk + 1;
+    if (hipMalloc((void **)&c->d_exptab, gmmk_exp_table_doubles() * sizeof(double)) != hipSuccess || gmmk_exp_table(c->stream, c->d_exptab) != 0 ||
+        hipStreamSynchronize(c->stream) != hipSuccess) {
+        (void)hipGetLastError();
+        gmmiv_set_error("ctx_create: the exponential table of the log-likelihood kernel could not be set up");
+        gmmiv_ctx_destroy(c);
+        return GMMIV_ERR_HIP;
+    }
     *out = c;
     return GMMIV_OK;
 }
@@ -80,6 +87,7 @@
         for (hipEvent_t e : c->ev1[i]) (void)hipEventDestroy(e);
     }
     if (c->d_zero_llk) (void)hipFree(c->d_zero_llk);
+    if (c->d_exptab) (void)hipFree(c->d_exptab);
     if (c->own_stream) (void)hipStreamDestroy(c->stream);
     if (g_kopts_src == &c->ko) gmmiv_kopts_bind(nullptr);
     delete c;
diff --git a/lia_ral_amd/csrc/capi_feat.hip b/lia_ral_amd/csrc/capi_feat.hip
--- a/lia_ral_amd/csrc/capi_feat.hip
+++ b/lia_ral_amd/csrc/capi_feat.hip
@@ -169,7 +169,6 @@
     if ((rc = o.init(c, out, odt, 0, T, ldo, g->D))) return rc;
     DevIn<double> i_off;
     if ((rc = i_off.init(c, WS_FEAT_M0, offset, (size_t)g->C * g->D))) return rc;
-    if ((rc = count_unusable(c, xv, dt, T, g->D))) return rc;
     const int64_t Tcz = g->D <= 64 ? z_chunk_frames(c, g) : 0;
     if (Tcz > 0) {
         gmmk_zview z;
@@ -180,8 +179,7 @@
         GCHK(gmmk_feat_pack_offset(c->stream, i_off.d, g->C, g->D, g->nct, (double *)offp));
         for (int64_t c0 = 0; c0 < T; c0 += Tcz) {
             const int64_t n = (T - c0) < Tcz ? (T - c0) : Tcz;
-            if ((rc = llk_z_run(c, g, xv, dt, c0, n, lz, z, c0 == 0))) return rc;
-            GCHK(count_dead(c, lz, n));
+            if ((rc = llk_z_run(c, g, xv, dt, c0, n, lz, z, c0 == 0, LLK_COUNT_BOTH))) return rc;
             c->t_begin("k_feat_comp", c0 == 0);
             GCHK(gmmk_feat_comp(c->stream, dt == GMMIV_F64, odt == GMMIV_F64, gmmiv_x_at(xv, dt, c0), xv.ldx, n, g->D, g->nct, z, (const double *)offp,
                                 o.at(c0), o.ld));
@@ -190,7 +188,7 @@
         return o.finish();
     }
     double *lse;
-    if ((rc = run_lse(c, g, xv, dt, T, &lse))) return rc;
+    if ((rc = run_lse(c, g, xv, dt, T, &lse, true))) return rc;
     int64_t per = (int64_t)(((size_t)512 << 20) / ((size_t)g->C * sizeof(double))) / 2 * 2;
     if (per < 64) per = 64;
     const int64_t firstg = T < per ? T : per;
diff --git a/lia_ral_amd/csrc/capi_gmm.hip b/lia_ral_amd/csrc/capi_gmm.hip
--- a/lia_ral_amd/csrc/capi_gmm.hip
+++ b/lia_ral_amd/csrc/capi_gmm.hip
@@ -54,21 +54,22 @@
     return GMMIV_OK;
 }
 
-int run_lse(gmmiv_ctx *c, const gmmiv_gmm *g, const XView &xv, int dt, int64_t T, double **lse_out)
+int run_lse(gmmiv_ctx *c, const gmmiv_gmm *g, const XView &xv, int dt, int64_t T, double **lse_out, bool screen)
 {
     void *lse;
     int rc = c->scratch(WS_LSE, (size_t)(T > 0 ? T : 1) * sizeof(double), &lse);
     if (rc) return rc;
     if (g->KS == GMMK_KS_GENERIC) {
+        if (screen && (rc = count_unusable(c, xv, dt, T, g->D))) return rc;
         if ((rc = topc_big(c, g, xv, dt, T, 1, -INFINITY, INFINITY, TopOut{nullptr, nullptr, nullptr, nullptr, nullptr, (double *)lse, 1}))) return rc;
         GCHK(count_dead(c, (const double *)lse, T));
         *lse_out = (double *)lse;
         return GMMIV_OK;
     }
     c->t_begin("k_llk_mfma");
-    GCHK(gmmk_llk(c->stream, g->KS, dt == GMMIV_F64, xv.d, T, xv.ldx, g->D, g->Pt, g->nct, (double *)lse, (int)(c->use_glds | (c->dbg << 8)), (int)c->wg_waves));
+    GCHK(gmmk_llk(c->stream, g->KS, dt == GMMIV_F64, xv.d, T, xv.ldx, g->D, g->Pt, g->nct, (double *)lse, (int)(c->use_glds | (c->dbg << 8)), c->d_exptab, (int)c->wg_waves,
+                  llk_unusable_counter(c, screen ? LLK_COUNT_UNUSABLE : LLK_COUNT_NONE), c->d_zero_llk));
     c->t_end();
-    GCHK(count_dead(c, (const double *)lse, T));
     *lse_out = (double *)lse;
     return GMMIV_OK;
 }
@@ -130,7 +131,7 @@
         GCHK(hipMemsetAsync(flg, 0, 64, c->stream));
         c->t_begin("k_llk_mfma", c0 == 0);
         krc = gmmk_llk_topc(c->stream, g->KS, dt == GMMIV_F64, gmmiv_x_at(xv, dt, c0), n, xv.ldx, g->D, g->Pt, g->nct, (int)c->use_glds,
-                            ctop, (double *)cand, (int *)cnt, (double *)th, (double *)sl, efin);
+                            c->d_exptab, ctop, (double *)cand, (int *)cnt, (double *)th, (double *)sl, efin);
         c->t_end();
         if (krc) break;
         c->t_begin("k_topc_rank", c0 == 0);
@@ -182,7 +183,7 @@
     for (int64_t c0 = 0; c0 < T; c0 += Tc) {
         const int64_t n = (T - c0) < Tc ? (T - c0) : Tc;
         const TopOut oc = o.at(c0);
-        if ((rc = llk_z_run(c, g, xv, dt, c0, n, lse, z, c0 == 0))) return rc;
+        if ((rc = llk_z_run(c, g, xv, dt, c0, n, lse, z, c0 == 0, LLK_COUNT_NONE))) return rc;
         c->t_begin("k_topc_from_z", c0 == 0);
         GCHK(gmmk_topc_from_z(c->stream, dt == GMMIV_F64, gmmiv_x_at(xv, dt, c0), n, xv.ldx, g->D, g->C, g->nct, z, g->mean, g->iv, g->lwc, g->w,
                               o.ctop, complete, min_llk, max_llk, oc.idx, oc.lk, oc.nlk, oc.nllk, oc.nw, oc.llk, (int *)flg));
@@ -216,9 +217,8 @@
     if (T < 0) { gmmiv_set_error("llk: T < 0"); return GMMIV_ERR_ARG; }
     XView xv;
     if ((rc = xv.init(c, x, dt, T, ldx, g->D))) return rc;
-    if ((rc = count_unusable(c, xv, dt, T, g->D))) return rc;
     double *lse;
-    if ((rc = run_lse(c, g, xv, dt, T, &lse))) return rc;
+    if ((rc = run_lse(c, g, xv, dt, T, &lse, true))) return rc;
     DevOut<double> o_llk, o_sum;
     if ((rc = o_llk.init(c, WS_T0, llk_out, (size_t)T, false))) return rc;
     if ((rc = o_sum.init(c, WS_T1, sums, 2, true))) return rc;
@@ -410,7 +410,6 @@
     if ((rc = xv.init(c, x, dt, T, ldx, g->D))) return rc;
     DevOut<double> o;
     if ((rc = o.init(c, WS_T0, gamma, (size_t)T * g->C, false))) return rc;
-    if ((rc = count_unusable(c, xv, dt, T, g->D))) return rc;
     const int64_t Tcz = c->topc_z ? z_chunk_frames(c, g) : 0;
     if (Tcz > 0 && T > 0) {
         gmmk_zview z;
@@ -418,8 +417,7 @@
         if ((rc = gmmiv_z_reserve(c, g->nct, T < Tcz ? T : Tcz, true, &z, &lz))) return rc;
         for (int64_t c0 = 0; c0 < T; c0 += Tcz) {
             const int64_t n = (T - c0) < Tcz ? (T - c0) : Tcz;
-            if ((rc = llk_z_run(c, g, xv, dt, c0, n, lz, z, c0 == 0))) return rc;
-            GCHK(count_dead(c, lz, n));
+            if ((rc = llk_z_run(c, g, xv, dt, c0, n, lz, z, c0 == 0, LLK_COUNT_BOTH))) return rc;
             c->t_begin("k_post_from_z", c0 == 0);
             GCHK(gmmk_post_from_z(c->stream, n, g->C, g->nct, z, o.d + (size_t)c0 * g->C));
             c->t_end();
@@ -427,7 +425,7 @@
         return o.finish();
     }
     double *lse;
-    if ((rc = run_lse(c, g, xv, dt, T, &lse))) return rc;
+    if ((rc = run_lse(c, g, xv, dt, T, &lse, true))) return rc;
     c->t_begin("k_posteriors");
     GCHK(gmmk_posteriors(c->stream, dt == GMMIV_F64, xv.d, T, xv.ldx, g->D, g->C, g->Cp64, g->meanT, g->ivT, g->lwc, lse, o.d));
     c->t_end();
@@ -474,8 +472,7 @@
     if ((rc = c->scratch(WS_PART, (size_t)nseg * Cp * 2 * RL * sizeof(double), &part))) return rc;
     for (int64_t k = 0; k < nchunk; ++k) {
         const int64_t c0 = k * Tc, n = (k == nchunk - 1) ? lastn : Tc;
-        if ((rc = llk_z_run(c, g, xv, dt, c0, n, lse + c0, z, k == 0))) return rc;
-        GCHK(count_dead(c, lse + c0, n));
+        if ((rc = llk_z_run(c, g, xv, dt, c0, n, lse + c0, z, k == 0, LLK_COUNT_BOTH))) return rc;
         c->t_begin("k_stats_z", k == 0);
         GCHK(gmmk_stats_z(c->stream, g->KS, 1, dt == GMMIV_F64, gmmiv_x_at(xv, dt, c0), xv.ldx, g->D, g->C, g->nct, z, weight,
                           (const long *)seg + (k == nchunk - 1 ? nseg + 1 : 0), nseg, (double *)part, nullptr, 0, k > 0, c->prune_thr()));
@@ -498,7 +495,6 @@
     if (T == 0) return o.finish();
     XView xv;
     if ((rc = xv.init(c, x, dt, T, ldx, g->D))) return rc;
-    if ((rc = count_unusable(c, xv, dt, T, g->D))) return rc;
     const int64_t Tc = z_chunk_frames(c, g);
     if (Tc > 0) {
         void *lsew, *small, *part;
@@ -512,7 +508,7 @@
         return o.finish();
     }
     double *lse;
-    if ((rc = run_lse(c, g, xv, dt, T, &lse))) return rc;
+    if ((rc = run_lse(c, g, xv, dt, T, &lse, true))) return rc;
     void *small;
     if ((rc = c->scratch(WS_SMALL, 3 * 256 * sizeof(double), &small))) return rc;
     GCHK(gmmk_llk_finalize(c->stream, lse, T, -INFINITY, INFINITY, nullptr, (double *)small, 0.0, weight, nullptr,
@@ -647,7 +643,6 @@
     if (U > 0x7fffffff / 64) { gmmiv_set_error("tv_stats: too many utterances in one call"); return GMMIV_ERR_UNSUPPORTED; }
     XView xv;
     if ((rc = xv.init(c, x, dt, T, ldx, g->D))) return rc;
-    if ((rc = count_unusable(c, xv, dt, T, g->D))) return rc;
     std::vector<long> h(utt_begin, utt_begin + U + 1);
     void *seg;
     if ((rc = c->scratch(WS_SEG, (U + 1) * sizeof(long), &seg))) return rc;
@@ -682,10 +677,15 @@
             GCHK(hipMemcpyAsync(prb, rbh.data(), rbh.size() * sizeof(int), hipMemcpyHostToDevice, c->stream));
             GCHK(hipStreamSynchronize(c->stream));
         }
+        if ((rc = count_unusable(c, xv, dt, utt_begin[0], g->D))) return rc;
+        {
+            XView tail = xv;
+            tail.d = gmmiv_x_at(xv, dt, utt_begin[U]);
+            if ((rc = count_unusable(c, tail, dt, T - utt_begin[U], g->D))) return rc;
+        }
         for (size_t k = 0; k + 1 < cu.size(); ++k) {
             const int64_t u0 = cu[k], u1 = cu[k + 1], c0 = utt_begin[u0], n = utt_begin[u1] - c0;
-            if ((rc = llk_z_run(c, g, xv, dt, c0, n, lsew, z, k == 0))) return rc;
-            GCHK(count_dead(c, lsew, n));
+            if ((rc = llk_z_run(c, g, xv, dt, c0, n, lsew, z, k == 0, LLK_COUNT_BOTH))) return rc;
             c->t_begin("k_stats_z", k == 0);
             GCHK(gmmk_stats_z(c->stream, g->KS, 0, dt == GMMIV_F64, gmmiv_x_at(xv, dt, c0), xv.ldx, g->D, g->C, g->nct, z, 1.0,
                               split ? (const long *)pseg : (const long *)seg + u0 + k, split ? np : (int)(u1 - u0), (double *)tn + (size_t)u0 * g->C,
@@ -700,7 +700,7 @@
         return o_f.finish();
     }
     double *lse;
-    if ((rc = run_lse(c, g, xv, dt, T, &lse))) return rc;
+    if ((rc = run_lse(c, g, xv, dt, T, &lse, true))) return rc;
     if (g->KS == GMMK_KS_GENERIC) {
         const int NC = g->D + 2 - (g->D & 1);
         void *S;
diff --git a/lia_ral_amd/csrc/capi_gmm_util.h b/lia_ral_amd/csrc/capi_gmm_util.h
--- a/lia_ral_amd/csrc/capi_gmm_util.h
+++ b/lia_ral_amd/csrc/capi_gmm_util.h
@@ -101,11 +101,16 @@
     return tc >= 4096 ? tc : 0;
 }
 
-static inline int llk_z_run(gmmiv_ctx *c, const gmmiv_gmm *g, const XView &xv, int dt, int64_t c0, int64_t n, double *lse, const gmmk_zview &z, bool first)
+enum { LLK_COUNT_NONE = 0, LLK_COUNT_UNUSABLE = 1, LLK_COUNT_DEAD = 2, LLK_COUNT_BOTH = 3 };
+static inline unsigned long long *llk_unusable_counter(const gmmiv_ctx *c, int counts) { return (counts & LLK_COUNT_UNUSABLE) && !c->assume_finite ? c->d_screened : nullptr; }
+static inline unsigned long long *llk_dead_counter(const gmmiv_ctx *c, int counts) { return (counts & LLK_COUNT_DEAD) ? c->d_zero_llk : nullptr; }
+
+static inline int llk_z_run(gmmiv_ctx *c, const gmmiv_gmm *g, const XView &xv, int dt, int64_t c0, int64_t n, double *lse, const gmmk_zview &z, bool first,
+                            int counts)
 {
     c->t_begin("k_llk_mfma", first);
     GCHK(gmmk_llk_z(c->stream, g->KS, dt == GMMIV_F64, gmmiv_x_at(xv, dt, c0), n, xv.ldx, g->D, g->Pt, g->nct, lse,
-                    (int)(c->use_glds | ((c->dbg & 15) << 8)), z));
+                    (int)(c->use_glds | ((c->dbg & 15) << 8)), c->d_exptab, z, llk_unusable_counter(c, counts), llk_dead_counter(c, counts)));
     c->t_end();
     return GMMIV_OK;
 }
@@ -114,7 +119,7 @@
 
 #pragma GCC visibility push(hidden)
 int count_unusable(gmmiv_ctx *c, const XView &xv, int dt, int64_t T, int D);
-int run_lse(gmmiv_ctx *c, const gmmiv_gmm *g, const XView &xv, int dt, int64_t T, double **lse_out);
+int run_lse(gmmiv_ctx *c, const gmmiv_gmm *g, const XView &xv, int dt, int64_t T, double **lse_out, bool screen);
 int generic_gamma_gemm(gmmiv_ctx *c, const gmmiv_gmm *g, const XView &xv, int dt, int64_t t0, int64_t n, const double *lse, bool sq, int NC,
                        double *S);
 extern "C" int gmmiv_feat_check_args(const char *who, const void *x, int xdt, int64_t T, int64_t ldx, const void *out, int odt, int64_t ldo, int D);
diff --git a/lia_ral_amd/csrc/capi_models.hip b/lia_ral_amd/csrc/capi_models.hip
--- a/lia_ral_amd/csrc/capi_models.hip
+++ b/lia_ral_amd/csrc/capi_models.hip
@@ -342,10 +342,10 @@
     c->t_begin("k_llk_mfma", first);
     if (z)
         GCHK(gmmk_llk_z_models(c->stream, b->KS, dt == GMMIV_F64, xb, xv.ldx, b->D, pt, (long)b->packed_doubles(), b->nct, p.d_tiles + ck.tile_off,
-                               (long)ck.ntiles, lse, (int)(c->use_glds & 1), *z));
+                               (long)ck.ntiles, lse, (int)(c->use_glds & 1), c->d_exptab, *z));
     else
         GCHK(gmmk_llk_models(c->stream, b->KS, dt == GMMIV_F64, xb, xv.ldx, b->D, pt, (long)b->packed_doubles(), b->nct, p.d_tiles + ck.tile_off,
-                             (long)ck.ntiles, lse, (int)(c->use_glds & 1)));
+                             (long)ck.ntiles, lse, (int)(c->use_glds & 1), c->d_exptab));
     c->t_end();
     GCHK(gmmk_count_dead(c->stream, lse + (f0 - ck.base), (long)n, c->d_zero_llk));
     return GMMIV_OK;
@@ -372,7 +372,7 @@
     if ((rc = om.set(c, b, m))) return rc;
     sub->d = gmmiv_x_at(xv, dt, f0); sub->ldx = xv.ldx;
     if ((rc = count_unusable(c, *sub, dt, n, b->D))) return rc;
-    if ((rc = run_lse(c, om.g, *sub, dt, n, lse))) return rc;
+    if ((rc = run_lse(c, om.g, *sub, dt, n, lse, false))) return rc;
     void *p;
     if ((rc = c->scratch(WS_MB_SEG, 2 * sizeof(long), &p))) return rc;
     GCHK(gmmk_fill_chunks(c->stream, (long *)p, 1, (long)n, (long)n));
diff --git a/lia_ral_amd/csrc/ctx.h b/lia_ral_amd/csrc/ctx.h
--- a/lia_ral_amd/csrc/ctx.h
+++ b/lia_ral_amd/csrc/ctx.h
@@ -61,6 +61,7 @@
     long topc_fused = 1;
     long assume_finite = 0;
     unsigned long long *d_zero_llk = nullptr, *d_screened = nullptr;
+    double *d_exptab = nullptr;
     long topc_fallbacks = 0;
     long topc_z = 1;
     long tv_acc_mb = 8192;
diff --git a/lia_ral_amd/csrc/devutil.h b/lia_ral_amd/csrc/devutil.h
--- a/lia_ral_amd/csrc/devutil.h
+++ b/lia_ral_amd/csrc/devutil.h
@@ -96,6 +96,11 @@
 __device__ __forceinline__ void gexp_tab_init(double *tab, int tid, int nthreads)
 {
     for (int j = tid; j < GEXP_TAB_N; j += nthreads) tab[j] = exp2((double)j * (1.0 / GEXP_TAB_N));
+}
+__device__ __forceinline__ void gexp_tab_init(double *tab, int tid, int nthreads, const double *__restrict__ src)
+{
+    typedef double d2 __attribute__((ext_vector_type(2)));
+    for (int j = tid; j < GEXP_TAB_N / 2; j += nthreads) ((d2 *)tab)[j] = ((const d2 *)src)[j];
 }
 __device__ __forceinline__ double gexp_tab_poly(double r)
 {
@@ -273,12 +278,16 @@
 __device__ __forceinline__ float feat_sane(float v) { return v; }
 __device__ __forceinline__ double feat_sane(double v) { return v; }
 #endif
+__device__ __forceinline__ bool feat_unusable(float v) { return !(__builtin_fabsf(v) <= (float)GMMIV_UNUSABLE_BOUND); }
+__device__ __forceinline__ bool feat_unusable(double v) { return !(__builtin_fabs(v) <= GMMIV_UNUSABLE_BOUND); }
 template <typename T> struct feat_load;
 template <> struct feat_load<float> {
     static __device__ __forceinline__ double get(const void *p, long i) { return (double)feat_sane(((const float *)p)[i]); }
+    static __device__ __forceinline__ double get(const void *p, long i, bool &unusable) { const float v = ((const float *)p)[i]; unusable |= feat_unusable(v); return (double)feat_sane(v); }
     static __device__ __forceinline__ double raw(const void *p, long i) { return (double)((const float *)p)[i]; }
 };
 template <> struct feat_load<double> {
     static __device__ __forceinline__ double get(const void *p, long i) { return feat_sane(((const double *)p)[i]); }
+    static __device__ __forceinline__ double get(const void *p, long i, bool &unusable) { const double v = ((const double *)p)[i]; unusable |= feat_unusable(v); return feat_sane(v); }
     static __device__ __forceinline__ double raw(const void *p, long i) { return ((const double *)p)[i]; }
 };
diff --git a/lia_ral_amd/csrc/gmm_kernels.h b/lia_ral_amd/csrc/gmm_kernels.h
--- a/lia_ral_amd/csrc/gmm_kernels.h
+++ b/lia_ral_amd/csrc/gmm_kernels.h
@@ -11,7 +11,9 @@
 int gmmk_pack_model(hipStream_t st, int C, int D, int KS, int nct, int Cp64, const double *w, const double *mean,
                     const double *iv, double *a, double *lwc, double *Pt, double *meanT, double *ivT);
 int gmmk_llk(hipStream_t st, int KS, int x_f64, const void *x, long T, long ldx, int D, const double *Pt, int nct,
-             double *lse, int use_glds, int wg_waves);
+             double *lse, int use_glds, const double *exptab, int wg_waves, unsigned long long *n_unusable, unsigned long long *n_dead);
+size_t gmmk_exp_table_doubles(void);
+int gmmk_exp_table(hipStream_t st, double *tab);
 int gmmk_llk_finalize(hipStream_t st, const double *lse, long T, double lo, double hi, double *llk_out,
                       double *partial , double scale_c, double scale_r, double *dst_clamped,
                       double *dst_raw, double scale_n = 0.0, double *dst_count = nullptr);
@@ -66,11 +68,11 @@
     int *efin;
 };
 int gmmk_llk_z(hipStream_t st, int KS, int x_f64, const void *x, long T, long ldx, int D, const double *Pt, int nct,
-               double *lse, int use_glds, const gmmk_zview &z);
+               double *lse, int use_glds, const double *exptab, const gmmk_zview &z, unsigned long long *n_unusable, unsigned long long *n_dead);
 int gmmk_llk_models(hipStream_t st, int KS, int x_f64, const void *x, long ldx, int D, const double *Pt, long pt_stride, int nct,
-                    const gmmiv_model_tile *tiles, long ntiles, double *lse, int use_glds);
+                    const gmmiv_model_tile *tiles, long ntiles, double *lse, int use_glds, const double *exptab);
 int gmmk_llk_z_models(hipStream_t st, int KS, int x_f64, const void *x, long ldx, int D, const double *Pt, long pt_stride, int nct,
-                      const gmmiv_model_tile *tiles, long ntiles, double *lse, int use_glds, const gmmk_zview &z);
+                      const gmmiv_model_tile *tiles, long ntiles, double *lse, int use_glds, const double *exptab, const gmmk_zview &z);
 int gmmk_const_models(hipStream_t st, int G, int C, int Cp, int D, const double *w, long sw, const double *mean, long sm, const double *iv,
                       long si, double *a, double *lwc);
 int gmmk_pack_models(hipStream_t st, int n, const int *ids, int C, int Cp, int D, int KS, int nct, const double *mean, long sm,
@@ -90,7 +92,7 @@
 int gmmk_acc_to_rows(hipStream_t st, int C, int D, const double *acc, double *Nrow, double *Frow, double *Srow);
 int gmmk_topc_cap(void);
 int gmmk_llk_topc(hipStream_t st, int KS, int x_f64, const void *x, long T, long ldx, int D, const double *Pt, int nct, int use_glds,
-                  int ctop, double *cand, int *cnt, double *theta, double *slow, int *efin);
+                  const double *exptab, int ctop, double *cand, int *cnt, double *theta, double *slow, int *efin);
 int gmmk_topc_rank(hipStream_t st, int x_f64, const void *x, long n, long ldx, int D, int C, const double *cand, const int *cnt,
                    const double *theta, const double *slow, const int *efin, const double *mean, const double *iv, const double *lwc,
                    const double *w, int ctop, int complete, double lo, double hi, int *idx, double *lk, double *nlk, double *nllk,
diff --git a/lia_ral_amd/csrc/gmm_kernels.hip b/lia_ral_amd/csrc/gmm_kernels.hip
--- a/lia_ral_amd/csrc/gmm_kernels.hip
+++ b/lia_ral_amd/csrc/gmm_kernels.hip
@@ -100,15 +100,18 @@
 #ifndef K1_PLAIN_SHARED
 #define K1_PLAIN_SHARED 1
 #endif
-template <int KS, typename XT, int NW, int MODE, bool MM = false>
+template <int KS, typename XT, int NW, int MODE, bool MM = false, bool GLDS = true>
 __global__ __launch_bounds__(NW * 64, 2) void k_llk_mfma(const void *__restrict__ x, long T, long ldx, int D,
                                                   const double *__restrict__ Pt, int nct,
-                                                  double *__restrict__ lse_out, int use_glds, int dbg,
+                                                  double *__restrict__ lse_out, int dbg,
                                                   double *__restrict__ zbuf, long nfb, int *__restrict__ eit,
                                                   double *__restrict__ inv_out, int *__restrict__ efin_out,
-                                                  const gmmiv_model_tile *__restrict__ tiles, long pt_stride)
+                                                  const gmmiv_model_tile *__restrict__ tiles, long pt_stride,
+                                                  unsigned long long *__restrict__ n_unusable, unsigned long long *__restrict__ n_dead,
+                                                  const double *__restrict__ exptab)
 {
     constexpr bool WZ = MODE == 1, TC = MODE == 2;
+    constexpr bool COUNT = !MM && !TC;
     static_assert(!MM || (MODE != 2 && NW == 8), "a model per segment: plain and stored-likelihood modes, 8 waves");
     constexpr int NR = 2 * KS + 2;
     constexpr int GT = 2;
@@ -130,11 +133,12 @@
         Pt += (size_t)me.model * pt_stride;
     }
     const long tb = tb0 + wave * 32;
-    gexp_tab_init(etab, tid, NW * 64);
+    gexp_tab_init(etab, tid, NW * 64, exptab);
     if (TC) ccnt[tid >> 1] = 0;
 
     constexpr int NA = TC ? KS : 2 * KS;
     double A[2][NA];
+    bool bad[2] = {false, false};
 #pragma unroll
     for (int h = 0; h < 2; ++h) {
         const long t = tb + h * 16 + i16;
@@ -142,16 +146,30 @@
         for (int s = 0; s < KS; ++s) {
             const int k = 4 * s + q;
             double v = 0.0;
-            if ((MM ? (t >= wlo && t < whi) : t < T) && k < D) v = feat_load<XT>::get(x, t * ldx + k);
+            if ((MM ? (t >= wlo && t < whi) : t < T) && k < D) {
+                if constexpr (COUNT) v = feat_load<XT>::get(x, t * ldx + k, bad[h]);
+                else v = feat_load<XT>::get(x, t * ldx + k);
+            }
             A[h][s] = v;
             if (!TC) A[h][NA - KS + s] = v * v;
+        }
+    }
+    if constexpr (COUNT) {
+        if (n_unusable) {
+            unsigned nbad = 0;
+#pragma unroll
+            for (int h = 0; h < 2; ++h) {
+                const unsigned long long m = __builtin_amdgcn_ballot_w64(bad[h]);
+                nbad += __builtin_popcount((unsigned)((m | (m >> 16) | (m >> 32) | (m >> 48)) & 0xffffu));
+            }
+            if (nbad != 0 && lane == 0) atomicAdd(n_unusable, (unsigned long long)nbad);
         }
     }
 
     const int ntiles = nct / GT;
     auto stage = [&](double *dst, int tile) {
         const char *src = (const char *)(Pt + (size_t)tile * TILE_D);
-        if (use_glds) {
+        if constexpr (GLDS) {
             if (PIECES % NW == 0) {
 #pragma unroll
                 for (int j = 0; j < PIECES / NW; ++j) {
@@ -475,6 +493,7 @@
         if (ntiles > 0) step(ntiles - 1, false, true, ntiles == 1);
     }
     if (late && ntiles > 0) epi_phase(ntiles - 1);
+    unsigned ndead = 0;
 #pragma unroll
     for (int h = 0; h < 2; ++h)
 #pragma unroll
@@ -492,12 +511,19 @@
                 if (i16 == 0 && t < T) { lse_out[t] = (double)thf[h][r]; inv_out[t] = sv; efin_out[t] = Em; }
                 continue;
             }
+            bool dead = false;
             if (i16 == 0 && (MM ? (t >= wlo && t < whi) : t < T)) {
                 const bool ok = sv > 0.0 && sv < __builtin_inf() && Em > GMMIV_MIN_FRAME_EXP;
-                lse_out[t] = ok ? log(sv) + (double)Em * 0.693147180559945309417 : -__builtin_inf();
+                const double l = ok ? log(sv) + (double)Em * 0.693147180559945309417 : -__builtin_inf();
+                lse_out[t] = l;
                 if (WZ) { inv_out[t] = ok ? 1.0 / sv : 0.0; efin_out[t] = ok ? Em : 0; }
-            }
-        }
+                dead = !(l > -__builtin_inf() && l < __builtin_inf());
+            }
+            if constexpr (COUNT) ndead += __builtin_popcountll(__builtin_amdgcn_ballot_w64(dead));
+        }
+    if constexpr (COUNT) {
+        if (n_dead && ndead != 0 && lane == 0) atomicAdd(n_dead, (unsigned long long)ndead);
+    }
     if (TC) {
         __syncthreads();
         const long t = (long)blockIdx.x * (NW * 32) + tid;
@@ -1144,6 +1170,14 @@
         if (_e != hipSuccess) return (int)_e;                             \
     } while (0)
 
+__global__ __launch_bounds__(256) void k_exp_table(double *__restrict__ tab) { gexp_tab_init(tab, blockIdx.x * 256 + threadIdx.x, gridDim.x * 256); }
+size_t gmmk_exp_table_doubles(void) { return GEXP_TAB_N; }
+int gmmk_exp_table(hipStream_t st, double *tab)
+{
+    k_exp_table<<<GEXP_TAB_N / 256, 256, 0, st>>>(tab);
+    return (int)hipGetLastError();
+}
+
 int gmmk_ks_for_dim(int D)
 {
     if (D <= 16) return 4;
@@ -1168,32 +1202,43 @@
 
 template <int KS, typename XT, int NW, int MODE>
 static int launch_llk(hipStream_t st, const void *x, long T, long ldx, int D, const double *Pt, int nct,
-                      double *lse, int use_glds, const gmmk_zview &z = gmmk_zview{})
+                      double *lse, int use_glds, const double *exptab, const gmmk_zview &z = gmmk_zview{},
+                      unsigned long long *n_unusable = nullptr, unsigned long long *n_dead = nullptr)
 {
     constexpr int NR = 2 * KS + 2;
     const size_t lds = 2 * 2 * NR * 64 * sizeof(double) + GEXP_TAB_N * sizeof(double) + (MODE == 2 ? NW * 32 * sizeof(int) : 0);
-    HIPCHK((gmmiv_lds_attr<k_llk_mfma<KS, XT, NW, MODE>>(lds)));
     const unsigned grid = (unsigned)((T + NW * 32 - 1) / (NW * 32));
-    k_llk_mfma<KS, XT, NW, MODE><<<grid, NW * 64, lds, st>>>(x, T, ldx, D, Pt, nct, lse, use_glds & 1, use_glds >> 8, z.zbuf, z.nfb, z.eit, z.inv, z.efin, nullptr, 0);
+    if (use_glds & 1) {
+        HIPCHK((gmmiv_lds_attr<k_llk_mfma<KS, XT, NW, MODE, false, true>>(lds)));
+        k_llk_mfma<KS, XT, NW, MODE, false, true><<<grid, NW * 64, lds, st>>>(x, T, ldx, D, Pt, nct, lse, use_glds >> 8, z.zbuf, z.nfb, z.eit, z.inv, z.efin, nullptr, 0, n_unusable, n_dead, exptab);
+    } else {
+        HIPCHK((gmmiv_lds_attr<k_llk_mfma<KS, XT, NW, MODE, false, false>>(lds)));
+        k_llk_mfma<KS, XT, NW, MODE, false, false><<<grid, NW * 64, lds, st>>>(x, T, ldx, D, Pt, nct, lse, use_glds >> 8, z.zbuf, z.nfb, z.eit, z.inv, z.efin, nullptr, 0, n_unusable, n_dead, exptab);
+    }
     return (int)hipGetLastError();
 }
 
 template <int KS, typename XT, int MODE>
 static int launch_llk_models(hipStream_t st, const void *x, long ldx, int D, const double *Pt, long pt_stride, int nct, const gmmiv_model_tile *tiles,
-                             long ntiles, double *lse, int use_glds, const gmmk_zview &z)
+                             long ntiles, double *lse, int use_glds, const double *exptab, const gmmk_zview &z)
 {
     constexpr int NR = 2 * KS + 2;
     const size_t lds = 2 * 2 * NR * 64 * sizeof(double) + GEXP_TAB_N * sizeof(double);
-    HIPCHK((gmmiv_lds_attr<k_llk_mfma<KS, XT, 8, MODE, true>>(lds)));
-    k_llk_mfma<KS, XT, 8, MODE, true><<<(unsigned)ntiles, 8 * 64, lds, st>>>(x, 0, ldx, D, Pt, nct, lse, use_glds & 1, 0, z.zbuf, z.nfb, z.eit, z.inv, z.efin, tiles, pt_stride);
+    if (use_glds & 1) {
+        HIPCHK((gmmiv_lds_attr<k_llk_mfma<KS, XT, 8, MODE, true, true>>(lds)));
+        k_llk_mfma<KS, XT, 8, MODE, true, true><<<(unsigned)ntiles, 8 * 64, lds, st>>>(x, 0, ldx, D, Pt, nct, lse, 0, z.zbuf, z.nfb, z.eit, z.inv, z.efin, tiles, pt_stride, nullptr, nullptr, exptab);
+    } else {
+        HIPCHK((gmmiv_lds_attr<k_llk_mfma<KS, XT, 8, MODE, true, false>>(lds)));
+        k_llk_mfma<KS, XT, 8, MODE, true, false><<<(unsigned)ntiles, 8 * 64, lds, st>>>(x, 0, ldx, D, Pt, nct, lse, 0, z.zbuf, z.nfb, z.eit, z.inv, z.efin, tiles, pt_stride, nullptr, nullptr, exptab);
+    }
     return (int)hipGetLastError();
 }
 #define MM_CASE(K, MODE)                                                                                                  \
     case K:                                                                                                               \
-        return x_f64 ? launch_llk_models<K, double, MODE>(st, x, ldx, D, Pt, pt_stride, nct, tiles, ntiles, lse, use_glds, z) \
-                     : launch_llk_models<K, float, MODE>(st, x, ldx, D, Pt, pt_stride, nct, tiles, ntiles, lse, use_glds, z);
+        return x_f64 ? launch_llk_models<K, double, MODE>(st, x, ldx, D, Pt, pt_stride, nct, tiles, ntiles, lse, use_glds, exptab, z) \
+                     : launch_llk_models<K, float, MODE>(st, x, ldx, D, Pt, pt_stride, nct, tiles, ntiles, lse, use_glds, exptab, z);
 int gmmk_llk_models(hipStream_t st, int KS, int x_f64, const void *x, long ldx, int D, const double *Pt, long pt_stride, int nct,
-                    const gmmiv_model_tile *tiles, long ntiles, double *lse, int use_glds)
+                    const gmmiv_model_tile *tiles, long ntiles, double *lse, int use_glds, const double *exptab)
 {
     if (ntiles <= 0) return 0;
     const gmmk_zview z = {};
@@ -1203,7 +1248,7 @@
     return -1;
 }
 int gmmk_llk_z_models(hipStream_t st, int KS, int x_f64, const void *x, long ldx, int D, const double *Pt, long pt_stride, int nct,
-                      const gmmiv_model_tile *tiles, long ntiles, double *lse, int use_glds, const gmmk_zview &z)
+                      const gmmiv_model_tile *tiles, long ntiles, double *lse, int use_glds, const double *exptab, const gmmk_zview &z)
 {
     if (ntiles <= 0) return 0;
     switch (KS) {
@@ -1463,17 +1508,17 @@
 }
 
 int gmmk_llk(hipStream_t st, int KS, int x_f64, const void *x, long T, long ldx, int D, const double *Pt, int nct,
-             double *lse, int use_glds, int wg_waves)
+             double *lse, int use_glds, const double *exptab, int wg_waves, unsigned long long *n_unusable, unsigned long long *n_dead)
 {
     if (T <= 0) return 0;
     if (T <= 32768 && gmmiv_kopts_cur().short_calls) wg_waves = 4;
 #define CASE(K)                                                                                      \
     case K:                                                                                          \
         if (wg_waves == 8)                                                                           \
-            return x_f64 ? launch_llk<K, double, 8, 0>(st, x, T, ldx, D, Pt, nct, lse, use_glds) \
-                         : launch_llk<K, float, 8, 0>(st, x, T, ldx, D, Pt, nct, lse, use_glds); \
-        return x_f64 ? launch_llk<K, double, 4, 0>(st, x, T, ldx, D, Pt, nct, lse, use_glds)     \
-                     : launch_llk<K, float, 4, 0>(st, x, T, ldx, D, Pt, nct, lse, use_glds);
+            return x_f64 ? launch_llk<K, double, 8, 0>(st, x, T, ldx, D, Pt, nct, lse, use_glds, exptab, gmmk_zview{}, n_unusable, n_dead) \
+                         : launch_llk<K, float, 8, 0>(st, x, T, ldx, D, Pt, nct, lse, use_glds, exptab, gmmk_zview{}, n_unusable, n_dead); \
+        return x_f64 ? launch_llk<K, double, 4, 0>(st, x, T, ldx, D, Pt, nct, lse, use_glds, exptab, gmmk_zview{}, n_unusable, n_dead)     \
+                     : launch_llk<K, float, 4, 0>(st, x, T, ldx, D, Pt, nct, lse, use_glds, exptab, gmmk_zview{}, n_unusable, n_dead);
     switch (KS) {
         CASE(4) CASE(8) CASE(15) CASE(20)
     }
@@ -1482,17 +1527,17 @@
 }
 
 int gmmk_llk_z(hipStream_t st, int KS, int x_f64, const void *x, long T, long ldx, int D, const double *Pt, int nct,
-               double *lse, int use_glds, const gmmk_zview &z)
+               double *lse, int use_glds, const double *exptab, const gmmk_zview &z, unsigned long long *n_unusable, unsigned long long *n_dead)
 {
     if (T <= 0) return 0;
     const bool small = T <= 32768 && gmmiv_kopts_cur().short_calls;
 #define CASE(K)                                                                                   \
     case K:                                                                                       \
         if (small)                                                                                \
-            return x_f64 ? launch_llk<K, double, 4, 1>(st, x, T, ldx, D, Pt, nct, lse, use_glds, z) \
-                         : launch_llk<K, float, 4, 1>(st, x, T, ldx, D, Pt, nct, lse, use_glds, z); \
-        return x_f64 ? launch_llk<K, double, 8, 1>(st, x, T, ldx, D, Pt, nct, lse, use_glds, z)   \
-                     : launch_llk<K, float, 8, 1>(st, x, T, ldx, D, Pt, nct, lse, use_glds, z);
+            return x_f64 ? launch_llk<K, double, 4, 1>(st, x, T, ldx, D, Pt, nct, lse, use_glds, exptab, z, n_unusable, n_dead) \
+                         : launch_llk<K, float, 4, 1>(st, x, T, ldx, D, Pt, nct, lse, use_glds, exptab, z, n_unusable, n_dead); \
+        return x_f64 ? launch_llk<K, double, 8, 1>(st, x, T, ldx, D, Pt, nct, lse, use_glds, exptab, z, n_unusable, n_dead)   \
+                     : launch_llk<K, float, 8, 1>(st, x, T, ldx, D, Pt, nct, lse, use_glds, exptab, z, n_unusable, n_dead);
     switch (KS) {
         CASE(4) CASE(8) CASE(15)
     }
@@ -1502,7 +1547,7 @@
 
 int gmmk_topc_cap(void) { return TOPC_CAP; }
 int gmmk_llk_topc(hipStream_t st, int KS, int x_f64, const void *x, long T, long ldx, int D, const double *Pt, int nct, int use_glds,
-                  int ctop, double *cand, int *cnt, double *theta, double *slow, int *efin)
+                  const double *exptab, int ctop, double *cand, int *cnt, double *theta, double *slow, int *efin)
 {
     if (T <= 0) return 0;
     if (ctop < 1 || ctop > 16) return -1;
@@ -1512,10 +1557,10 @@
 #define CASE(K)                                                                                                                    \
     case K:                                                                                                                        \
         if (small)                                                                                                                 \
-            return x_f64 ? launch_llk<K, double, 4, 2>(st, x, T, ldx, D, Pt, nct, theta, use_glds, tc)        \
-                         : launch_llk<K, float, 4, 2>(st, x, T, ldx, D, Pt, nct, theta, use_glds, tc);        \
-        return x_f64 ? launch_llk<K, double, 8, 2>(st, x, T, ldx, D, Pt, nct, theta, use_glds, tc)            \
-                     : launch_llk<K, float, 8, 2>(st, x, T, ldx, D, Pt, nct, theta, use_glds, tc);
+            return x_f64 ? launch_llk<K, double, 4, 2>(st, x, T, ldx, D, Pt, nct, theta, use_glds, exptab, tc)        \
+                         : launch_llk<K, float, 4, 2>(st, x, T, ldx, D, Pt, nct, theta, use_glds, exptab, tc);        \
+        return x_f64 ? launch_llk<K, double, 8, 2>(st, x, T, ldx, D, Pt, nct, theta, use_glds, exptab, tc)            \
+                     : launch_llk<K, float, 8, 2>(st, x, T, ldx, D, Pt, nct, theta, use_glds, exptab, tc);
     switch (KS) {
         CASE(4) CASE(8) CASE(15)
     }
```

Result: no change. 129.2 Gframe-Gaussian/s (median of 6 runs) (+0.7%).
